# vibevoice-community/VibeVoice

Measured on AMD Instinct MI355X. Metric: audio-sec/wall-sec, higher is better.
Workload: dtype bf16

## Files before the change

### vibevoice_amd/csrc/engine.hip

```cpp
#include "engine_ctx.h"
#include "vv_w13.h"

thread_local char g_err[512] = "";
std::shared_mutex g_dev_mu;
std::mutex g_family_mu;

int fail(vv_ctx* ctx, const char* fmt, ...) {
    va_list ap; va_start(ap, fmt);
    char* dst = ctx ? ctx->err : g_err;
    vsnprintf(dst, 512, fmt, ap);
    va_end(ap);
    if (ctx) snprintf(g_err, 512, "%s", ctx->err);
    return -1;
}

int ring_acquire(vv_ctx* ctx) {
    const int slot = ctx->ring_i;
    ctx->ring_i = (ctx->ring_i + 1) % vv_ctx::RING;
    if (ctx->ring_used[slot]) hipEventSynchronize(ctx->ring_ev[slot]);
    ctx->ring_used[slot] = true;
    return slot;
}

void* dalloc(vv_ctx* ctx, size_t bytes, bool zero) {
// ... 102 lines not shown
                char prev[200]; snprintf(prev, sizeof(prev), "%s", ctx->err);
                return fail(ctx, "%s; the eager re-run failed as well (%s).  If another host thread called a device-wide synchronize "
                                 "(torch.cuda.synchronize()) during the capture, the stream is lost: synchronize streams or events instead", ctx->last_capture_issue, prev);
            }
            return 0;
        }
        if (ctx->graphs.size() >= ctx->graph_cap) {
            std::vector<std::pair<uint64_t, std::string>> order;
            for (auto& g : ctx->graphs) order.push_back({g.second.last_use, g.first});
            std::sort(order.begin(), order.end());
            std::unique_lock<std::shared_mutex> lk(g_dev_mu);
            HIPCHK(ctx, hipDeviceSynchronize());
            for (size_t i = 0; i < order.size() / 4 + 1; ++i) {
                auto v = ctx->graphs.find(order[i].second);
                hipGraphExecDestroy(v->second.exec);
                ctx->graphs.erase(v);
            }
        }
        it = ctx->graphs.emplace(key, ge).first;
    }
    it->second.last_use = ++ctx->graph_tick;
    VV_SHARED;
    HIPCHK(ctx, hipGraphLaunch(it->second.exec, st));
    return 0;
}

int drop_graphs(vv_ctx* ctx, std::initializer_list<const char*> prefixes) {
    auto hit = [&](const std::string& key) {
        for (const char* p : prefixes) if (key.rfind(p, 0) == 0) return true;
        return false;
    };
    bool any = false;
    for (auto& g : ctx->graphs) if (hit(g.first)) { any = true; break; }
    if (!any) return 0;
    HIPCHK(ctx, hipDeviceSynchronize());
    for (auto it = ctx->graphs.begin(); it != ctx->graphs.end();) {
        if (hit(it->first)) { hipGraphExecDestroy(it->second.exec); it = ctx->graphs.erase(it); } else ++it;
    }
    return 0;
}

extern "C" const char* vv_last_error(vv_ctx* ctx) { return ctx ? ctx->err : g_err; }

#ifndef VV_BUILD_ID
#define VV_BUILD_ID "unknown"
#endif
extern "C" const char* vv_build_id() { return "VVHIP_BUILD_ID=" VV_BUILD_ID; }

static int create_impl(const vv_config* cfg, vv_ctx* parent, vv_ctx** out) {
    VV_SHARED;
    vv_ctx* ctx = new vv_ctx();
    ctx->c = *cfg; ctx->err[0] = 0;
    ctx->parent = parent; ctx->creating = true;
    vv_config& c = ctx->c;
    if (c.max_rows < 1 || c.max_rows > 16384) { delete ctx; return fail(nullptr, "max_rows must be in [1,16384]"); }
    if (c.lm_head_dim != 64 && c.lm_head_dim != 128) { delete ctx; return fail(nullptr, "head_dim must be 64 or 128"); }
    if (c.lm_kv_heads < 1 || c.lm_heads % c.lm_kv_heads != 0 || c.lm_heads / c.lm_kv_heads > 16) {
        const int hq = c.lm_heads, hkv = c.lm_kv_heads;
        delete ctx;
        return fail(nullptr, "lm_heads=%d / lm_kv_heads=%d: the GQA group size must be an integer <= 16", hq, hkv);
    }
    if (c.xsplit < 1 || c.xsplit > 3) c.xsplit = 2;
    if (c.attn_splits < 1) c.attn_splits = 128;
    if (c.enc_frames < 1) c.enc_frames = 1;
    if (getenv("VVHIP_GRAPH_CAP")) ctx->graph_cap = (size_t)std::max(4, atoi(getenv("VVHIP_GRAPH_CAP")));
    c.max_ctx = (c.max_ctx + 127) & ~127;
    const int H = ctx->H = c.lm_hidden, D = ctx->D = c.lm_head_dim, Hq = ctx->Hq = c.lm_heads, Hkv = ctx->Hkv = c.lm_kv_heads;
    const int I = ctx->I = c.lm_inter;
    const int QKV = ctx->QKV = (Hq + 2 * Hkv) * D;
    const int R = c.max_rows;
    ctx->embed = walloc(ctx, (size_t)c.lm_vocab * H * 2);
    { int i = add_w(ctx, "lm.embed_tokens.weight", W_TABLE, (int64_t)c.lm_vocab * H); ctx->w[i].dev = ctx->embed; }
    { int i = add_w(ctx, "lm_head.weight", W_TABLE, (int64_t)c.lm_vocab * H, true); ctx->w[i].dev = nullptr; }
    ctx->inv_freq = add_vec(ctx, "lm.rope.inv_freq", D / 2);
    ctx->lm_norm = add_vec(ctx, "lm.norm.weight", H);
    if (c.tts_layers > 0) {
        if (c.tts_layers >= c.lm_layers) { delete ctx; return fail(nullptr, "tts_layers must be < lm_layers"); }
        ctx->tts_types = add_vec(ctx, "tts_input_types.weight", 2 * (int64_t)H);
        ctx->eos_w1 = alloc_packed(ctx, H, H); add_mat(ctx, "eos.fc1.weight", H, H, ctx->eos_w1, 0);
        ctx->eos_b1 = add_vec(ctx, "eos.fc1.bias", H);
        ctx->eos_w2 = alloc_packed(ctx, 1, H); add_mat(ctx, "eos.fc2.weight", 1, H, ctx->eos_w2, 0);
        ctx->eos_b2 = add_vec(ctx, "eos.fc2.bias", 1);
    }
    ctx->layers.resize(c.lm_layers);
    for (int l = 0; l < c.lm_layers; ++l) {
        auto& L = ctx->layers[l];
        char nm[128]; snprintf(nm, 128, "lm.layers.%d.", l);
        std::string p(nm);
        L.ln1 = add_vec(ctx, p + "input_layernorm.weight", H);
        L.ln2 = add_vec(ctx, p + "post_attention_layernorm.weight", H);
        L.wqkv = alloc_packed(ctx, QKV, H);
        L.bqkv = (float*)walloc(ctx, (size_t)QKV * 4);
        add_mat(ctx, p + "self_attn.q_proj.weight", Hq * D, H, L.wqkv, 0);
        add_mat(ctx, p + "self_attn.k_proj.weight", Hkv * D, H, L.wqkv, Hq * D / 16);
        add_mat(ctx, p + "self_attn.v_proj.weight", Hkv * D, H, L.wqkv, (Hq + Hkv) * D / 16);
        add_vec(ctx, p + "self_attn.q_proj.bias", Hq * D, L.bqkv);
        add_vec(ctx, p + "self_attn.k_proj.bias", Hkv * D, L.bqkv + Hq * D);
        add_vec(ctx, p + "self_attn.v_proj.bias", Hkv * D, L.bqkv + (Hq + Hkv) * D);
        L.wo = alloc_packed(ctx, H, Hq * D); add_mat(ctx, p + "self_attn.o_proj.weight", H, Hq * D, L.wo, 0);
        L.wg = alloc_packed(ctx, I, H); add_mat(ctx, p + "mlp.gate_proj.weight", I, H, L.wg, 0);
        L.wu = alloc_packed(ctx, I, H); add_mat(ctx, p + "mlp.up_proj.weight", I, H, L.wu, 0);
        L.wd = alloc_packed(ctx, H, I); add_mat(ctx, p + "mlp.down_proj.weight", H, I, L.wd, 0);
    }
    const int n_caches = 2 * c.n_slots;
    ctx->head_stride = (int64_t)c.max_ctx * D;
    ctx->layer_stride = ctx->head_stride * Hkv;
    ctx->cache_stride = ctx->layer_stride * c.lm_layers;
    ctx->kc = dalloc(ctx, (size_t)ctx->cache_stride * n_caches * 2);
    ctx->vc = dalloc(ctx, (size_t)ctx->cache_stride * n_caches * 2);
    ctx->rows_cap = std::max(2048, c.max_rows);
    ctx->rows_dev = (VVRow*)dalloc(ctx, sizeof(VVRow) * ctx->rows_cap);
    hipHostMalloc((void**)&ctx->rows_pin, sizeof(VVRow) * (size_t)ctx->rows_cap * vv_ctx::RING);
    for (int i = 0; i < vv_ctx::RING; ++i) hipEventCreateWithFlags(&ctx->ring_ev[i], hipEventDisableTiming);
    ctx->ids_cap = std::max(64, c.max_rows);
    ctx->ids_dev = (int*)dalloc(ctx, sizeof(int) * ctx->ids_cap);
    hipHostMalloc((void**)&ctx->ids_pin, sizeof(int) * (size_t)ctx->ids_cap * vv_ctx::RING);
    ctx->h = (float*)dalloc(ctx, (size_t)R * H * 4);
    ctx->h_parts = (float*)dalloc(ctx, (size_t)2 * R * H * 4);
    ctx->qkv = (float*)dalloc(ctx, (size_t)R * QKV * 4);
    ctx->qrot = (float*)dalloc(ctx, (size_t)R * Hq * D * 4);
    ctx->attn = (float*)dalloc(ctx, (size_t)R * Hq * D * 4);
    ctx->act = (float*)dalloc(ctx, (size_t)R * I * 4);
    if (R >= 64 && (H % 8) == 0 && ((Hq * D) % 8) == 0 && (I % 8) == 0) {
        ctx->xp = dalloc(ctx, (size_t)vv_packed_elems(R, std::max(H, Hq * D)) * 2);
        ctx->actp = dalloc(ctx, (size_t)vv_packed_elems(R, I) * 2);
        ctx->tile3_ok = c.xsplit == 1;
        if (ctx->tile3_ok) {
            ctx->gws.g3_bytes = (size_t)8 * std::min(R, 1024) * std::max(ctx->QKV, H) * 4;
            ctx->gws.g3_partials = (float*)dalloc(ctx, ctx->gws.g3_bytes, false);
            if (!ctx->gws.g3_partials) ctx->gws.g3_bytes = 0;
        }
        const char* no_ks = getenv("VVHIP_NO_KSPLIT");
        if (ctx->tile3_ok && R >= 1024 && !(no_ks && no_ks[0] == '1')) {
            ctx->gws.partials = (float*)dalloc(ctx, (size_t)256 * 32 * 512 * 16, false);
            ctx->gws.flags = (unsigned*)dalloc(ctx, 256 * sizeof(unsigned));
            if (hipHostMalloc((void**)&ctx->gws.err, sizeof(unsigned), hipHostMallocMapped) == hipSuccess && ctx->gws.err) *ctx->gws.err = 0u;
            else ctx->gws.err = nullptr;
        }
    }
    ctx->attn2_ok = c.xsplit == 1;
    if (c.xsplit == 1 && R > 4 && (H % 32) == 0 && ((Hq * D) % 32) == 0 && (I % 32) == 0) {
        const int kx = std::max(H, Hq * D), ka = std::max(I, c.head_ffn);
        ctx->p16_x = dalloc(ctx, (size_t)vv_packed_elems(16, kx) * 2);
        ctx->p16_act = dalloc(ctx, (size_t)vv_packed_elems(16, ka + 32) * 2);
        ctx->p16_y = dalloc(ctx, (size_t)vv_packed_elems(16, kx) * 2);
        ctx->ssq_a = (float*)dalloc(ctx, (size_t)(H / 16) * 16 * 4);
        ctx->ssq_b = (float*)dalloc(ctx, (size_t)(H / 16) * 16 * 4);
        ctx->p16_ok = ctx->p16_x && ctx->p16_act && ctx->p16_y && ctx->ssq_a && ctx->ssq_b;
    }
    ctx->rope_tab = dalloc(ctx, (size_t)c.max_ctx * (D / 2) * 8, false);
    ctx->ws_rows = std::min(R, 64);
    const size_t np = (size_t)ctx->ws_rows * Hkv * c.attn_splits * 16;
    ctx->pm = (float*)dalloc(ctx, np * 4); ctx->pl = (float*)dalloc(ctx, np * 4); ctx->po = (float*)dalloc(ctx, np * D * 4);
    const int L = c.latent_dim, HL = c.head_layers, HF = ctx->HF = c.head_ffn;
    const int MODW = ctx->MODW = HL * 3 * H + 2 * H;
    ctx->h_in = alloc_packed(ctx, H, L); add_mat(ctx, "head.noisy_images_proj.weight", H, L, ctx->h_in, 0);
    ctx->h_cond = alloc_packed(ctx, H, H); add_mat(ctx, "head.cond_proj.weight", H, H, ctx->h_cond, 0);
    ctx->h_t0 = alloc_packed(ctx, H, 256); add_mat(ctx, "head.t_embedder.mlp.0.weight", H, 256, ctx->h_t0, 0);
    ctx->h_t2 = alloc_packed(ctx, H, H); add_mat(ctx, "head.t_embedder.mlp.2.weight", H, H, ctx->h_t2, 0);
    ctx->h_ada = alloc_packed(ctx, MODW, H);
    ctx->hl.resize(HL);
    {
        const char* e = getenv("VVHIP_W13");
        ctx->w13_on = parent ? parent->w13_on : !(e && e[0] == '0') && c.xsplit == 1 && vv_w13_shape_ok(HF, H) && vv_w13_shape_ok(H, HF);
    }
    auto twin = [&](int N, int K) {
        if (ctx->w13_on) ctx->w.back().w13 = walloc(ctx, (size_t)vv_w13_bytes(N, K));
        return (int)ctx->w.size() - 1;
    };
    for (int l = 0; l < HL; ++l) {
        char nm[128]; snprintf(nm, 128, "head.layers.%d.", l);
        std::string p(nm);
        ctx->hl[l].norm = add_vec(ctx, p + "norm.weight", H);
        add_mat(ctx, p + "adaLN_modulation.1.weight", 3 * H, H, ctx->h_ada, l * 3 * H / 16);
        ctx->hl[l].wg = alloc_packed(ctx, HF, H); add_mat(ctx, p + "ffn.gate_proj.weight", HF, H, ctx->hl[l].wg, 0); ctx->hl[l].ig = twin(HF, H);
        ctx->hl[l].wu = alloc_packed(ctx, HF, H); add_mat(ctx, p + "ffn.up_proj.weight", HF, H, ctx->hl[l].wu, 0); ctx->hl[l].iu = twin(HF, H);
        ctx->hl[l].wd = alloc_packed(ctx, H, HF); add_mat(ctx, p + "ffn.down_proj.weight", H, HF, ctx->hl[l].wd, 0); ctx->hl[l].id = twin(H, HF);
    }
    add_mat(ctx, "head.final_layer.adaLN_modulation.1.weight", 2 * H, H, ctx->h_ada, HL * 3 * H / 16);
    ctx->h_out = alloc_packed(ctx, L, H); add_mat(ctx, "head.final_layer.linear.weight", L, H, ctx->h_out, 0);
    const int R2 = 16;
    ctx->cproj = (float*)dalloc(ctx, (size_t)R2 * H * 4);
    ctx->mod = (float*)dalloc(ctx, (size_t)R2 * MODW * 4);
    for (HeadGen& g : ctx->hg) {
        g.zz = (float*)dalloc(ctx, (size_t)R2 * L * 4);
        g.x0p = (float*)dalloc(ctx, (size_t)R2 * L * 4);
        g.xh = (float*)dalloc(ctx, (size_t)R2 * H * 4);
    }
    ctx->head_tail = c.xsplit == 1 && L == 64 && (H % 32) == 0 && vv_head_tail_init() == 0;
    if (const char* e = getenv("VVHIP_SOLVER_FUSE"); e && e[0] == '0') ctx->solver_fuse = false;
    if (const char* e = getenv("VVHIP_NAN_PROBE"); e && e[0] == '1') {
        ctx->probe_rec = (unsigned*)dalloc(ctx, PROBE_MAX * 16);
        ctx->probe_on = ctx->probe_rec != nullptr;
    }
    ctx->xh_parts = (float*)dalloc(ctx, (size_t)4 * R2 * H * 4);
    ctx->hact = (float*)dalloc(ctx, (size_t)R2 * HF * 4);
    ctx->eps = (float*)dalloc(ctx, (size_t)R2 * L * 4);
    ctx->tmp1 = (float*)dalloc(ctx, (size_t)64 * H * 4);
    ctx->tmp2 = (float*)dalloc(ctx, (size_t)64 * 256 * 4);
    auto mk_conn = [&](vv_ctx::Conn& cn, const std::string& p, int din) {
        cn.fc1 = alloc_packed(ctx, H, din); add_mat(ctx, p + "fc1.weight", H, din, cn.fc1, 0);
        cn.b1 = add_vec(ctx, p + "fc1.bias", H);
        cn.norm = add_vec(ctx, p + "norm.weight", H);
        cn.fc2 = alloc_packed(ctx, H, H); add_mat(ctx, p + "fc2.weight", H, H, cn.fc2, 0);
        cn.b2 = add_vec(ctx, p + "fc2.bias", H);
    };
    mk_conn(ctx->ac_conn, "ac_conn.", L);
    if (c.sem_dim > 0) mk_conn(ctx->sem_conn, "sem_conn.", c.sem_dim);
    ctx->ct1 = (float*)dalloc(ctx, (size_t)256 * H * 4);
    if (build_codec(ctx, ctx->dec, "dec.", true, L, 1, c.n_slots)) { *out = ctx; return -1; }
    if (c.sem_dim > 0 && build_codec(ctx, ctx->senc, "senc.", false, c.sem_dim, 1, c.n_slots)) { *out = ctx; return -1; }
    if (c.has_acoustic_encoder && build_codec(ctx, ctx->aenc, "aenc.", false, L, c.enc_frames, 1)) { *out = ctx; return -1; }
    if (hipDeviceSynchronize() != hipSuccess || ctx->err[0]) { *out = ctx; return fail(ctx, "vv_create: allocation failed: %s", ctx->err); }
    ctx->creating = false;
    if (parent) {
        if (ctx->wshare_i != parent->wallocs.size() || ctx->w.size() != parent->w.size()) {
            *out = ctx;
            return fail(ctx, "vv_create_shared: the child registered %zu weight buffers / %zu parameters, the parent %zu / %zu -- different model configuration",
                        ctx->wshare_i, ctx->w.size(), parent->wallocs.size(), parent->w.size());
        }
        for (size_t i = 0; i < ctx->w.size(); ++i) {
            if (ctx->w[i].name != parent->w[i].name || ctx->w[i].nelem != parent->w[i].nelem) { *out = ctx; return fail(ctx, "vv_create_shared: parameter table differs at '%s'", ctx->w[i].name.c_str()); }
            ctx->w[i].loaded = parent->w[i].loaded;
            ctx->w[i].w13_ok = parent->w[i].w13_ok;
            if (ctx->w[i].name == "lm_head.weight") ctx->w[i].dev = parent->w[i].dev;
        }
        ctx->lm_head = parent->lm_head; ctx->lm_head_loaded = parent->lm_head_loaded;
        ctx->scaling = parent->scaling; ctx->bias = parent->bias;
        { std::lock_guard<std::mutex> fl(g_family_mu); parent->n_children++; }
    }
    *out = ctx;
    return 0;
}

extern "C" int vv_create(const vv_config* cfg, vv_ctx** out) { return create_impl(cfg, nullptr, out); }

extern "C" int vv_create_shared(const vv_config* cfg, vv_ctx* parent, vv_ctx** out) {
    if (!parent) return fail(nullptr, "vv_create_shared: no parent context");
    if (parent->parent) return fail(nullptr, "vv_create_shared: the parent is itself a shared context; share from the owner of the weights");
    for (auto& w : parent->w)
        if (!w.loaded && !w.optional) return fail(nullptr, "vv_create_shared: parent parameter '%s' is not uploaded yet", w.name.c_str());
    vv_config a = *cfg, b = parent->c;
    a.n_slots = b.n_slots; a.max_ctx = b.max_ctx; a.max_rows = b.max_rows; a.attn_splits = b.attn_splits; a.use_graph = b.use_graph;
    if (a.xsplit < 1 || a.xsplit > 3) a.xsplit = 2;
    if (a.enc_frames < 1) a.enc_frames = 1;
    if (memcmp(&a, &b, sizeof(vv_config)) != 0) return fail(nullptr, "vv_create_shared: the model fields of the configuration differ from the parent's");
    int r = create_impl(cfg, parent, out);
    if (r != 0 && *out) { vv_ctx* c = *out; c->parent = nullptr; }
    return r;
}

static void destroy_impl(vv_ctx* ctx) {
    if (!ctx) return;
    hipDeviceSynchronize();
    {
        std::lock_guard<std::mutex> fl(g_family_mu);
        if (ctx->n_children > 0) { ctx->zombie = true; return; }
    }
    vv_ctx* par = ctx->parent;
    for (auto& g : ctx->graphs) hipGraphExecDestroy(g.second.exec);
    if (ctx->side_ready) {
        for (int j = 0; j < 8; ++j) { hipStreamDestroy(ctx->side[j]); hipEventDestroy(ctx->ev_join[j]); }
        hipEventDestroy(ctx->ev_fork);
    }
    for (void* p : ctx->allocs) hipFree(p);
    ctx->allocs.clear();
    if (ctx->stage) hipFree(ctx->stage);
    hipHostFree(ctx->rows_pin); hipHostFree(ctx->ids_pin);
    if (ctx->gws.err) hipHostFree(ctx->gws.err);
    for (int i = 0; i < vv_ctx::RING; ++i) if (ctx->ring_ev[i]) hipEventDestroy(ctx->ring_ev[i]);
    delete ctx;
    bool last_child = false;
    if (par) { std::lock_guard<std::mutex> fl(g_family_mu); last_child = (--par->n_children == 0 && par->zombie); }
    if (last_child) destroy_impl(par);
}
extern "C" void vv_destroy(vv_ctx* ctx) {
    VV_SHARED;
    destroy_impl(ctx);
}

extern "C" int vv_num_weights(vv_ctx* ctx) { return (int)ctx->w.size(); }
extern "C" int vv_weight_info(vv_ctx* ctx, int idx, char* name, int cap, int64_t* nelem, int* loaded) {
    if (idx < 0 || idx >= (int)ctx->w.size()) return fail(ctx, "weight index out of range");
    const Weight& w = ctx->w[idx];
    snprintf(name, cap, "%s", w.name.c_str());
    if (nelem) *nelem = w.nelem;
    if (loaded) *loaded = (w.loaded || w.optional) ? 1 : 0;
    return 0;
}

extern "C" int vv_upload(vv_ctx* ctx, const char* name, const void* src, int src_dtype, int64_t nelem) {
    VV_SHARED;
    auto it = ctx->widx.find(name);
    if (it == ctx->widx.end()) return fail(ctx, "unknown parameter '%s'", name);
    Weight& w = ctx->w[it->second];
    if (ctx->parent) return fail(ctx, "parameter '%s': this context shares its parent's weights -- upload through the parent", name);
    {
        std::lock_guard<std::mutex> fl(g_family_mu);
        if (ctx->n_children > 0)
            return fail(ctx, "parameter '%s': %d shared context(s) were created from this one and hold snapshots derived from its parameters -- "
                             "destroy them (model.close_lanes()), upload / merge, then fork again", name, ctx->n_children);
    }
    if (nelem != w.nelem) return fail(ctx, "parameter '%s': expected %lld elements, got %lld", name, (long long)w.nelem, (long long)nelem);
    const size_t esz = src_dtype ? 2 : 4;
    hipPointerAttribute_t attr;
    bool on_dev = (hipPointerGetAttributes(&attr, src) == hipSuccess) && (attr.type == hipMemoryTypeDevice);
    (void)hipGetLastError();
    const void* dsrc = src;
    if (!on_dev) {
        const size_t need = (size_t)nelem * esz;
        if (need > ctx->stage_bytes) {
            if (ctx->stage) hipFree(ctx->stage);
            ctx->stage = nullptr; ctx->stage_bytes = 0;
            HIPCHK(ctx, hipMalloc(&ctx->stage, need));
            ctx->stage_bytes = need;
        }
        HIPCHK(ctx, hipMemcpy(ctx->stage, src, need, hipMemcpyHostToDevice));
        dsrc = ctx->stage;
    }
    hipStream_t st = 0;
    if (w.kind == W_TABLE) {
        if (w.name == "lm_head.weight" && !ctx->lm_head_loaded) {
            ctx->lm_head = dalloc(ctx, (size_t)nelem * 2, false);
            if (!ctx->lm_head) return -1;
            ctx->lm_head_loaded = true; w.dev = ctx->lm_head;
        }
        if (src_dtype) HIPCHK(ctx, hipMemcpy(w.dev, dsrc, (size_t)nelem * 2, hipMemcpyDeviceToDevice));
        else VVCHK(vv_cvt_launch(dsrc, w.dev, nelem, 1, st));
    } else if (w.kind == W_MAT) {
        VVCHK(vv_pack_launch(dsrc, src_dtype, w.dev, w.N, w.K, w.pk, w.Cin, w.Cout, w.ksz, w.stride, st));
        VVTRY(lora_rebase(ctx, it->second, st));
        VVTRY(w13_repack(ctx, it->second, st));
    } else {
        const float* f32 = (const float*)dsrc;
        float* tmp = nullptr;
        if (src_dtype) {
            tmp = (float*)dalloc(ctx, (size_t)nelem * 4, false);
            if (!tmp) return -1;
            VVCHK(vv_cvt_launch(dsrc, tmp, nelem, 0, st));
            f32 = tmp;
        }
        if (w.kind == W_DW) {
            VVCHK(vv_dw_transpose_launch(f32, (float*)w.dev, (int)(nelem / 7), st));
        } else if (w.kind == W_BIAS_REP) {
            for (int r = 0; r < w.rep; ++r)
                HIPCHK(ctx, hipMemcpyAsync((float*)w.dev + (size_t)r * nelem, f32, (size_t)nelem * 4, hipMemcpyDeviceToDevice, st));
        } else {
            HIPCHK(ctx, hipMemcpyAsync(w.dev, f32, (size_t)nelem * 4, hipMemcpyDeviceToDevice, st));
        }
        HIPCHK(ctx, hipStreamSynchronize(st));
        dfree(ctx, tmp);
    }
    HIPCHK(ctx, hipStreamSynchronize(st));
    w.loaded = true;
    ctx->rope_ready = false;
    return 0;
}

int w13_repack(vv_ctx* ctx, int widx, hipStream_t st) {
    Weight& w = ctx->w[widx];
    if (!w.w13) return 0;
    VVCHK(vv_w13_pack_launch(w.dev, w.w13, w.N, w.K, st));
    HIPCHK(ctx, hipStreamSynchronize(st));
    unsigned ok = 0;
    HIPCHK(ctx, hipMemcpy(&ok, (const char*)w.w13 + vv_w13_plane_bytes(w.N, w.K) + (size_t)2 * (w.N / 16) * 4, 4, hipMemcpyDeviceToHost));
    const bool now = ok == 1;
    if (now == w.w13_ok) return 0;
    w.w13_ok = now;
    return drop_graphs(ctx, {"samp:", "sde:", "rows:", "gen:"});
}

extern "C" int vv_set_speech_factors(vv_ctx* ctx, float scaling, float bias) {
    VV_SHARED;
    ctx->scaling = scaling; ctx->bias = bias;
    return drop_graphs(ctx, {"dec:1:", "chain:1:"});
}

extern "C" int vv_set_valid_tokens(vv_ctx* ctx, const int* ids, int n) {
    VV_SHARED;
    if (n < 1 || n > 16) return fail(ctx, "n_valid must be in [1,16]");
    const int H = ctx->H;
    const void* table = ctx->lm_head_loaded ? ctx->lm_head : ctx->embed;
    void* rows = dalloc(ctx, (size_t)n * H * 2, false);
    if (!rows) return -1;
    for (int i = 0; i < n; ++i) {
        if (ids[i] < 0 || ids[i] >= ctx->c.lm_vocab) return fail(ctx, "token id %d out of range", ids[i]);
        HIPCHK(ctx, hipMemcpy((char*)rows + (size_t)i * H * 2, (const char*)table + (size_t)ids[i] * H * 2, (size_t)H * 2, hipMemcpyDeviceToDevice));
    }
    if (!ctx->valid_w) ctx->valid_w = alloc_packed(ctx, 16, H);
    VVCHK(vv_pack_launch(rows, 1, ctx->valid_w, n, H, 0, 0, 0, 0, 0, 0));
    HIPCHK(ctx, hipDeviceSynchronize());
    dfree(ctx, rows);
    ctx->n_valid = n;
    for (int i = 0; i < n; ++i) ctx->valid_ids[i] = ids[i];
    return 0;
}
extern "C" int vv_check(vv_ctx* ctx, void* stream) {
    if (!ctx) return -1;
    return ksplit_check(ctx, (hipStream_t)stream);
}
extern "C" int vv_audio_to_pcm16(vv_ctx* ctx, void* stream, int n, int samples, const float* audio_dev, int16_t* pcm_out_dev) {
    VV_SHARED;
    hipStream_t st = (hipStream_t)stream;
    if (n < 1 || samples < 1) return fail(ctx, "vv_audio_to_pcm16: n and samples must be positive");
    VVCHK(vv_pcm16_launch(audio_dev, (short*)pcm_out_dev, n, samples, st));
    return 0;
}
extern "C" int vv_connect(vv_ctx* ctx, void* stream, int n, const float* latent_dev, const float* sem_dev, float* out_dev) {
    VV_SHARED;
    hipStream_t st = (hipStream_t)stream;
    const int H = ctx->H, L = ctx->c.latent_dim;
    for (int i0 = 0; i0 < n; i0 += 16) {
        const int nn = std::min(16, n - i0);
        float* out = out_dev + (size_t)i0 * H;
        VVGemm a1 = mk_gemm(ctx->ac_conn.fc1, latent_dev + (size_t)i0 * L, ctx->ct1, nn, H, L, L, H);
        a1.epi = VV_EPI_BIAS; a1.bias = ctx->ac_conn.b1; GEMM(a1);
        VVGemm a2 = mk_gemm(ctx->ac_conn.fc2, ctx->ct1, out, nn, H, H, H, H);
        a2.pro = VV_PRO_RMS; a2.nw = ctx->ac_conn.norm; a2.eps = 1e-6f; a2.epi = VV_EPI_BIAS; a2.bias = ctx->ac_conn.b2; GEMM(a2);
        if (sem_dev) {
            const int S = ctx->c.sem_dim;
            VVGemm s1 = mk_gemm(ctx->sem_conn.fc1, sem_dev + (size_t)i0 * S, ctx->ct1, nn, H, S, S, H);
            s1.epi = VV_EPI_BIAS; s1.bias = ctx->sem_conn.b1; GEMM(s1);
            VVGemm s2 = mk_gemm(ctx->sem_conn.fc2, ctx->ct1, out, nn, H, H, H, H);
            s2.pro = VV_PRO_RMS; s2.nw = ctx->sem_conn.norm; s2.eps = 1e-6f; s2.epi = VV_EPI_RESID; s2.bias = ctx->sem_conn.b2; GEMM(s2);
        }
    }
    return 0;
}

extern "C" int64_t vv_packed_bytes(int N, int K) { return vv_packed_elems(N, K) * 2; }
extern "C" int vv_pack_matrix(void* stream, const float* src_dev, void* dst_dev, int N, int K) {
    return vv_pack_launch(src_dev, 0, dst_dev, N, K, 0, 0, 0, 0, 0, (hipStream_t)stream);
}
extern "C" int64_t vv_stat(vv_ctx* ctx, int what) {
    switch (what) {
        case 0: return ctx->launches;
        case 2: return ctx->prof_raw_ns;
        case 3: return ctx->prof_ev_over_ns;
        case 5: return ctx->foreign_nodes;
        case 4: return ctx->capture_fallbacks;
        case 6: return ctx->seam_launches;
        case 8: return ctx->solver_fused;
        case 7: return ctx->lora_base_bytes;
        case 9: {
            int64_t n = 0;
            for (const auto& l : ctx->hl) {
                if (ctx->w[l.ig].w13_ok && ctx->w[l.iu].w13_ok) n += 2;
                if (ctx->w[l.id].w13_ok) n += 1;
            }
            return n;
        }
        default: return (int64_t)ctx->graphs.size();
    }
}
```

### vibevoice_amd/csrc/engine_ctx.h

```cpp
#pragma once
#include <algorithm>
#include <cmath>
#include <cstdarg>
#include <cstdio>
#include <cstdlib>
#include <cstring>
#include <functional>
#include <initializer_list>
#include <map>
#include <mutex>
#include <set>
#include <shared_mutex>
#include <string>
#include <vector>
#include "../../include/vvhip.h"
#include "vv_common.h"
#include "vv_launch.h"

namespace vv_engine {
struct VVShiftH { float* buf; int T, hist, C; };
enum WKind { W_MAT = 0, W_VEC = 1, W_DW = 2, W_TABLE = 3, W_BIAS_REP = 4 };

struct Weight {
    std::string name;
    int kind = W_VEC;
    int64_t nelem = 0;
    void* dev = nullptr;
    int N = 0, K = 0, pk = 0, Cin = 0, Cout = 0, ksz = 0, stride = 0;
    int rep = 1;
    bool loaded = false;
    bool optional = false;
    void* w13 = nullptr;
    bool w13_ok = false;
};

struct Block {
    int C;
    float *norm_w, *ffn_norm_w, *gamma, *ffn_gamma, *dw_w, *dw_b, *b1, *b2;
    void *w1, *w2;
    float* nb;
    float* nst;
    int64_t nb_stride;
};

struct ConvG {
    void* w; float* bias;
    int K, N, ldx;
    int rows_per_frame;
};

struct Stage {
    int C, Tpf;
    int hist;
    float* xs;
    float* xs2;
    float* xfinal;
    bool fused;
    bool pp;
    int64_t sl_stride;
    std::vector<Block> blocks;
    ConvG in;
};

struct CodecNet {
    bool decoder = false;
    int Fmax = 1, in_dim = 1, out_dim = 1, in_hist = 6, in_Tpf = 1;
    std::vector<float*> in_buf;
    std::vector<std::vector<Stage>> st;
    ConvG head;
    std::vector<float*> u;
    std::map<std::pair<uint64_t, int>, std::pair<void*, int>> shift_tab;
    int maxC = 1;
    int kd = 0, ke = 1 << 30;
    bool head_batch = false;
    int64_t in_stride = 0, u_stride = 0;
};

struct GraphEntry { hipGraphExec_t exec; uint64_t last_use; };

struct HeadGen { float *xh = nullptr, *zz = nullptr, *x0p = nullptr, *m2 = nullptr; };

}
using namespace vv_engine;

constexpr int PROBE_MAX = 1024;

struct vv_ctx {
    vv_config c;
    char err[512];
    std::vector<Weight> w;
    std::map<std::string, int> widx;
    int H, D, Hq, Hkv, I, QKV;
    struct Layer { float *ln1, *ln2, *bqkv; void *wqkv, *wo, *wg, *wu, *wd; };
    std::vector<Layer> layers;
    float *lm_norm = nullptr, *inv_freq = nullptr;
    int ws_rows = 0;
    void* rope_tab = nullptr; bool rope_ready = false;
    float *tts_types = nullptr, *eos_b1 = nullptr, *eos_b2 = nullptr; void *eos_w1 = nullptr, *eos_w2 = nullptr;
    void *embed = nullptr, *lm_head = nullptr;
    bool lm_head_loaded = false;
    void* valid_w = nullptr; int n_valid = 0;
    int valid_ids[16] = {0};
    void *kc = nullptr, *vc = nullptr;
    int64_t cache_stride = 0, head_stride = 0, layer_stride = 0;
    VVRow* rows_dev = nullptr; VVRow* rows_pin = nullptr; int rows_cap = 2048;
    int* ids_dev = nullptr; int* ids_pin = nullptr; int ids_cap = 64;
    static constexpr int RING = 32;
    hipEvent_t ring_ev[RING] = {}; bool ring_used[RING] = {}; int ring_i = 0;
    float *h = nullptr, *qkv = nullptr, *qrot = nullptr, *attn = nullptr, *act = nullptr;
    float *h_parts = nullptr, *xh_parts = nullptr;
    void *xp = nullptr, *actp = nullptr;
    bool tile3_ok = false, attn2_ok = false;
    VVGemmWs gws = {nullptr, nullptr, nullptr, nullptr, 0};
    void *p16_x = nullptr, *p16_act = nullptr, *p16_y = nullptr, *p16_shift = nullptr; float *ssq_a = nullptr, *ssq_b = nullptr; bool p16_ok = false;
    size_t p16_shift_tile = 0;
    float *pm = nullptr, *pl = nullptr, *po = nullptr;
    int HF = 0, MODW = 0;
    struct HLayer { float* norm; void *wg, *wu, *wd; int ig, iu, id; };
    bool w13_on = false;
    std::vector<HLayer> hl;
    void *h_in = nullptr, *h_cond = nullptr, *h_t0 = nullptr, *h_t2 = nullptr, *h_ada = nullptr, *h_out = nullptr;
    int n_steps = 0;
    float *temb = nullptr, *coef = nullptr, *tvals = nullptr;
    bool sde_on = false;
    bool general_on = false;
    float* mod_all = nullptr; size_t mod_all_bytes = 0;
    float* ada_in = nullptr;
    void* ada_p = nullptr;
    float *cproj = nullptr, *mod = nullptr, *hact = nullptr, *eps = nullptr;
    HeadGen hg[2];
    bool head_tail = false;
    bool solver_fuse = true;
    float *tmp1 = nullptr, *tmp2 = nullptr;
    struct Conn { void *fc1, *fc2; float *b1, *b2, *norm; } ac_conn, sem_conn;
    float *ct1 = nullptr;
    CodecNet dec, aenc, senc;
    int enc_pass = 0;
    hipStream_t side[8] = {}; hipEvent_t ev_fork = nullptr, ev_join[8] = {}; bool side_ready = false;
    float scaling = 1.f, bias = 0.f;
    int hop = 3200;
    void* stage = nullptr; size_t stage_bytes = 0;
    std::map<std::string, GraphEntry> graphs;
    uint64_t graph_tick = 0; size_t graph_cap = 512;
    std::set<std::string> seen;
    std::set<void*> allocs;
    vv_ctx* parent = nullptr; int n_children = 0; bool zombie = false, creating = false;
    unsigned* probe_rec = nullptr; std::vector<std::string> probe_names; bool probe_on = false; int probe_calls = 0;
    int64_t foreign_nodes = 0;
    int64_t capture_fallbacks = 0; char last_capture_issue[256] = "";
    std::vector<std::pair<void*, size_t>> wallocs; size_t wshare_i = 0;
    struct LoraBase { void* snap; size_t bytes; bool merged; };
    std::map<int, LoraBase> lora_base;
    int64_t lora_base_bytes = 0;
    struct RowStage { int n_streams = 0; std::vector<int64_t> total; std::vector<char> flushed; };
    struct Resampler : RowStage { int L = 0, M = 0, T = 0; float* coef = nullptr; float* hist = nullptr; };
    static constexpr int N_RESAMPLERS = 4;
    Resampler rs[N_RESAMPLERS];
    struct Tempo : RowStage { float* window = nullptr; float* hist = nullptr; int* dstate = nullptr; std::vector<int> P, Q; };
    static constexpr int N_TEMPOS = 4;
    Tempo tp[N_TEMPOS];
    struct Level : RowStage { int A = 0, H = 0; float c = 0.f; float* hist = nullptr; std::vector<float> gain; };
    static constexpr int N_LEVELS = 4;
    Level lv[N_LEVELS];
    int64_t launches = 0;
    int64_t solver_fused = 0;
    int64_t seam_launches = 0;
    bool prof_on = false;
    std::vector<hipEvent_t> prof_ev;
    int prof_n = 0;
    double prof_bytes = 0.0;
    struct ProfRec { int T, N, K, pro, epi, dual; double bytes; int gemv; };
    std::vector<ProfRec> prof_rec;
    std::vector<VVGemm> prof_gemv;
    double prof_gemv_bytes = 0.0;
    struct ProfLaunch { int family; double bytes; std::function<int(hipStream_t)> fn; };
    std::vector<ProfLaunch> prof_other;
    int64_t prof_raw_ns = 0, prof_ev_over_ns = 0;
    hipStream_t prof_stream = nullptr;
#ifdef VV_GEMM_TIMING
    unsigned long long* tl_base = nullptr; int tl_idx = 0;
    struct TlRec { int T, N, K, pro, epi; };
    std::vector<TlRec> tl_rec;
#endif
};

extern thread_local char g_err[512];
extern std::shared_mutex g_dev_mu;
#define VV_SHARED std::shared_lock<std::shared_mutex> _vv_dev_lk(g_dev_mu)
extern std::mutex g_family_mu;
int fail(vv_ctx* ctx, const char* fmt, ...);
#define HIPCHK(ctx, e) do { hipError_t _e = (e); if (_e != hipSuccess) return fail(ctx, "%s:%d hip error %s", __FILE__, __LINE__, hipGetErrorString(_e)); } while (0)
#define VVCHK(e) do { int _r = (e); if (_r != 0) return _r < 0 ? fail(ctx, "%s:%d launch failed (%d): hip error %d (%s)", __FILE__, __LINE__, _r, g_vv_launch_err, hipGetErrorString((hipError_t)g_vv_launch_err)) : _r; } while (0)
#define VVTRY(e) do { if (int _r = (e)) return _r; } while (0)

void* dalloc(vv_ctx* ctx, size_t bytes, bool zero = true);
void dfree(vv_ctx* ctx, void* p);
void* walloc(vv_ctx* ctx, size_t bytes, bool zero = true);
void* alloc_packed(vv_ctx* ctx, int N, int K);
int add_w(vv_ctx* ctx, const std::string& name, int kind, int64_t nelem, bool optional = false);
void add_mat(vv_ctx* ctx, const std::string& name, int N, int K, void* base, int ntile_off, int pk = 0, int Cin = 0, int Cout = 0,
             int ksz = 0, int stride = 0, int64_t src_nelem = -1);
float* add_vec(vv_ctx* ctx, const std::string& name, int64_t n, float* dst = nullptr, int kind = W_VEC, int rep = 1);
// ... 27 lines not shown
```

### vibevoice_amd/csrc/engine_head.hip

```cpp
#include "engine_ctx.h"
#include "pass_plan.h"

static int set_schedule(vv_ctx* ctx, int n_steps, const float* t, const float* coef, int width, void* stream, bool stochastic = false) {
    VV_SHARED;
    hipStream_t st = (hipStream_t)stream;
    if (n_steps < 1 || n_steps > 64) return fail(ctx, "n_steps must be in [1,64]");
    const int H = ctx->H;
    if (!ctx->temb) {
        ctx->temb = (float*)dalloc(ctx, (size_t)64 * H * 4);
        ctx->coef = (float*)dalloc(ctx, 64 * 8 * 4);
        ctx->tvals = (float*)dalloc(ctx, 64 * 4);
    }
    const bool general = width == 8;
    if (general && !ctx->hg[0].m2) {
        for (HeadGen& g : ctx->hg) g.m2 = (float*)dalloc(ctx, (size_t)8 * ctx->c.latent_dim * 4);
        if (!ctx->hg[0].m2 || !ctx->hg[1].m2) return fail(ctx, "vv_set_schedule_general: out of device memory");
    }
    float rows[64 * 8] = {};
    for (int i = 0; i < n_steps; ++i)
        for (int j = 0; j < width; ++j) rows[i * 8 + j] = coef[i * width + j];
    ctx->sde_on = general ? stochastic : (width == 6);
    ctx->general_on = general;
    HIPCHK(ctx, hipStreamSynchronize(st));
    HIPCHK(ctx, hipMemcpy(ctx->coef, rows, (size_t)n_steps * 8 * 4, hipMemcpyHostToDevice));
    HIPCHK(ctx, hipMemcpy(ctx->tvals, t, (size_t)n_steps * 4, hipMemcpyHostToDevice));
    VVCHK(vv_tfreq_launch(ctx->tvals, ctx->tmp2, n_steps, st));
    for (int i0 = 0; i0 < n_steps; i0 += 16) {
        const int nn = std::min(16, n_steps - i0);
        VVGemm g = mk_gemm(ctx->h_t0, ctx->tmp2 + (size_t)i0 * 256, ctx->tmp1 + (size_t)i0 * H, nn, H, 256, 256, H);
        GEMM(g);
    }
    VVCHK(vv_silu_launch(ctx->tmp1, n_steps * H, st));
    for (int i0 = 0; i0 < n_steps; i0 += 16) {
        const int nn = std::min(16, n_steps - i0);
        VVGemm g = mk_gemm(ctx->h_t2, ctx->tmp1 + (size_t)i0 * H, ctx->temb + (size_t)i0 * H, nn, H, H, H, H);
        GEMM(g);
    }
    HIPCHK(ctx, hipStreamSynchronize(st));
    ctx->n_steps = n_steps;
    {
        const size_t need = (size_t)n_steps * 16 * ctx->MODW * 4;
        if (need > ctx->mod_all_bytes) {
            dfree(ctx, ctx->mod_all);
            dfree(ctx, ctx->ada_in);
            ctx->mod_all = (float*)dalloc(ctx, need, false);
            ctx->ada_in = (float*)dalloc(ctx, (size_t)n_steps * 16 * ctx->H * 4, false);
            dfree(ctx, ctx->ada_p);
            ctx->ada_p = (ctx->c.xsplit == 1 && (ctx->H & 7) == 0) ? dalloc(ctx, (size_t)vv_packed_elems(n_steps * 16, ctx->H) * 2, false) : nullptr;
            ctx->mod_all_bytes = (ctx->mod_all && ctx->ada_in) ? need : 0;
            dfree(ctx, ctx->p16_shift); ctx->p16_shift = nullptr;
            if (ctx->p16_ok) {
                ctx->p16_shift_tile = (size_t)vv_packed_elems(16, ctx->H) * 2;
                ctx->p16_shift = dalloc(ctx, (size_t)n_steps * (ctx->c.head_layers + 1) * ctx->p16_shift_tile);
            }
        }
    }
    return drop_graphs(ctx, {"samp:", "sde:", "rows:", "gen:"});
}
extern "C" int vv_set_schedule(vv_ctx* ctx, int n_steps, const float* t, const float* coef, void* stream) {
    return set_schedule(ctx, n_steps, t, coef, 5, stream);
}
extern "C" int vv_set_schedule_sde(vv_ctx* ctx, int n_steps, const float* t, const float* coef6, void* stream) {
    return set_schedule(ctx, n_steps, t, coef6, 6, stream);
}

extern "C" int vv_set_schedule_general(vv_ctx* ctx, int n_steps, const float* t, const float* coef, int stochastic, void* stream) {
    return set_schedule(ctx, n_steps, t, coef, 8, stream, stochastic != 0);
}

static VVHeadPlan head_plan(const vv_ctx* ctx, int rows, int n_steps, bool has_coef) {
    return vv_head_plan(rows, n_steps, ctx->HF, ctx->c.head_layers, ctx->MODW,
                        {ctx->p16_ok, ctx->p16_shift != nullptr, ctx->ada_p != nullptr, ctx->mod_all_bytes != 0, ctx->head_tail, ctx->w13_on}, has_coef,
                        has_coef && ctx->general_on);
}

struct StepEnd { const float* coef; float cfg; const float *cfg_rows, *noise; };
struct HeadStep {
    int step;
    const float *z, *temb, *mod;
    const unsigned char* sh_tiles;
    float* eps_out;
    const HeadGen &cur, &nxt;
    bool have_x;
    const StepEnd* end;
};

static int head_eval(vv_ctx* ctx, hipStream_t st, const VVHeadPlan& p, const HeadStep& s) {
    const vv_config& c = ctx->c;
    const int rows = p.rows, final_stage = vv_head_final(p, s.step);
    const int H = ctx->H, L = c.latent_dim, HL = c.head_layers, HF = ctx->HF, MODW = ctx->MODW;
    const float* mod = s.mod ? s.mod : ctx->mod;
    const StepEnd end = s.end ? *s.end : StepEnd{};
    auto put_end = [&](auto& a) { a.coef = end.coef; a.cfg = end.cfg; a.n_cfg = rows / 2; a.sde_noise = end.noise; a.cfg_rows = end.cfg_rows; };
    float* const xh = s.cur.xh;
    if (!s.mod) {
        VVGemm ga = mk_gemm(ctx->h_ada, ctx->cproj, ctx->mod, rows, MODW, H, H, MODW);
        ga.pro = VV_PRO_ADD_SILU; ga.addvec = s.temb; ga.nt = 1;
        GEMM(ga);
    }
    if (!s.have_x) {
        VVGemm gi = mk_gemm(ctx->h_in, s.z, xh, rows, H, L, L, H);
        GEMM(gi);
        nan_probe(ctx, st, "in-proj xh", xh, (size_t)rows * H);
    }
    int xp = 0;
    const int xps = 16 * H;
    for (int l = 0; l < HL; ++l) {
        const float* base = mod + (size_t)l * 3 * H;
        if (p.layers == VV_HEAD_P16) {
            ctx->launches += 3;
            VVCHK(vv_pack16_launch(xh, H, 2, ctx->hl[l].norm, c.head_eps, base + H, base, MODW, ctx->p16_x, rows, H, st));
            VVCHK(p16_gemv(ctx, st, ctx->hl[l].wg, ctx->hl[l].wu, ctx->p16_x, nullptr, ctx->p16_act, nullptr, nullptr, rows, HF, H, 0, 0, VV_EPI_SWIGLU));
            if (l + 1 == HL && final_stage == VV_FINAL_P16_CFG) {
                VVGemv16p ad = p16_args(ctx->hl[l].wd, nullptr, ctx->p16_act, xh, ctx->p16_x, rows, H, HF, H);
                ad.gate = base + 2 * H; ad.ld_gate = MODW; ad.ssq_out = ctx->ssq_a;
                ad.pk_nw = nullptr; ad.pk_sc = mod + (size_t)HL * 3 * H + H; ad.ld_pk = MODW;
                VVCHK(p16_go(ctx, st, ad, VV_EPI_GATED_RESID, 4));
            } else
            VVCHK(p16_gemv(ctx, st, ctx->hl[l].wd, nullptr, ctx->p16_act, xh, nullptr, nullptr, base + 2 * H, rows, H, HF, H, MODW, VV_EPI_GATED_RESID));
            continue;
        }
        VVGemm g1 = mk_gemm(ctx->hl[l].wg, xh, ctx->hact, rows, HF, H, H, HF);
        g1.W2 = (const u32x4*)ctx->hl[l].wu; g1.pro = VV_PRO_RMS_MOD; g1.nw = ctx->hl[l].norm; g1.eps = c.head_eps;
        g1.mod_shift = base; g1.mod_scale = base + H; g1.ld_mod = MODW; g1.epi = VV_EPI_SWIGLU; g1.nt = 1;
        float* cur = ctx->xh_parts + (size_t)(l & 1) * 2 * xps;
        float* nxt = ctx->xh_parts + (size_t)((l + 1) & 1) * 2 * xps;
        g1.xa = cur; g1.n_xa = xp; g1.part_stride = xps;
        const Weight &mg = ctx->w[ctx->hl[l].ig], &mu = ctx->w[ctx->hl[l].iu], &md = ctx->w[ctx->hl[l].id];
        if (p.w13 && mg.w13_ok && mu.w13_ok && vv_gemv_w13_form(&g1, c.xsplit) >= 0) { g1.w13 = mg.w13; g1.w13_2 = mu.w13; }
        GEMM(g1);
        VVGemm g2 = mk_gemm(ctx->hl[l].wd, ctx->hact, xh, rows, H, HF, HF, H);
        g2.epi = VV_EPI_GATED_RESID; g2.gate = base + 2 * H; g2.ld_gate = MODW; g2.nt = 1;
        g2.ya = cur; g2.n_ya = xp; g2.part_stride = xps;
        xp = ksplit_parts(ctx, g2, nxt, xps);
        if (p.w13 && md.w13_ok && vv_gemv_w13_form(&g2, c.xsplit) >= 0) g2.w13 = md.w13;
        if (ctx->probe_on) { char nm[64]; snprintf(nm, 64, "layer %d hact (parts in %d)", l, g1.n_xa); nan_probe(ctx, st, nm, ctx->hact, (size_t)rows * HF); }
        GEMM(g2);
        if (ctx->probe_on) {
            char nm[64]; snprintf(nm, 64, "layer %d xh", l); nan_probe(ctx, st, nm, xh, (size_t)rows * H);
            for (int q = 0; q < xp; ++q) { snprintf(nm, 64, "layer %d part %d", l, q); nan_probe(ctx, st, nm, nxt + (size_t)q * xps, (size_t)rows * H); }
        }
    }
    const float* fb = mod + (size_t)HL * 3 * H;
    if (final_stage == VV_FINAL_P16_CFG) {
        ctx->launches += 1;
        VVGemv16p af = p16_args(ctx->h_out, nullptr, ctx->p16_x, nullptr, nullptr, rows, L, H, L);
        af.ssq_in = ctx->ssq_a; af.ssq_tiles = H / 16; af.eps = c.head_eps;
        af.Xs = (const u32x4*)(s.sh_tiles + (size_t)HL * ctx->p16_shift_tile);
        af.z = s.cur.zz; af.x0p = s.cur.x0p; put_end(af);
        VVCHK(p16_go(ctx, st, af, VV_EPI_CFG_DPM, 3));
        return 0;
    }
    if (final_stage == VV_FINAL_SEAM) {
        VVTail t{};
        t.Wout = (const u32x4*)ctx->h_out; t.Win = (const u32x4*)ctx->h_in; t.bin = nullptr;
        t.X = xh; t.xa = ctx->xh_parts + (size_t)(HL & 1) * 2 * xps; t.n_xa = xp; t.part_stride = xps;
        t.sc = fb + H; t.sh = fb; t.ld_mod = MODW;
        t.Xout = s.nxt.xh;
        t.z_in = s.cur.zz; t.x0p_in = s.cur.x0p; t.z_out = s.nxt.zz; t.x0p_out = s.nxt.x0p; put_end(t);
        t.T = rows; t.H = H; t.L = L; t.eps = c.head_eps;
        if (vv_head_tail_ok(&t)) {
            ctx->launches++;
            ctx->seam_launches++;
            if (ctx->prof_on) {
                const VVTail tc = t;
                ctx->prof_other.push_back({3, (double)vv_packed_elems(L, H) * 2.0 + (double)vv_packed_elems(H, L) * 2.0 + (double)rows * H * 8.0,
                                           [=](hipStream_t s2) { return vv_head_tail_launch(&tc, s2); }});
            }
            VVCHK(vv_head_tail_launch(&t, st));
            return 1;
        }
    }
    VVGemm gf = mk_gemm(ctx->h_out, xh, s.eps_out, rows, L, H, H, L);
    gf.pro = VV_PRO_RMS_MOD; gf.nw = nullptr; gf.eps = c.head_eps; gf.mod_shift = fb; gf.mod_scale = fb + H; gf.ld_mod = MODW;
    gf.xa = ctx->xh_parts + (size_t)(HL & 1) * 2 * xps; gf.n_xa = xp; gf.part_stride = xps;
    if (final_stage != VV_FINAL_GEMM) {
        gf.epi = VV_EPI_CFG_DPM; gf.z = s.cur.zz; gf.x0p = s.cur.x0p; put_end(gf);
    }
    GEMM(gf);
    return 0;
}

struct SampleReq { int n; const float *cond, *noise, *step_noise; float cfg; const float* cfg_rows; float* out; };
struct StepDone { int rc; bool flipped; };

static StepDone step_shipped(vv_ctx* ctx, hipStream_t st, const VVHeadPlan& p, const SampleReq& r, HeadStep s) {
    const StepEnd end{ctx->coef + s.step * 8, r.cfg, r.cfg_rows,
                      r.step_noise ? r.step_noise + (size_t)s.step * r.n * ctx->c.latent_dim : nullptr};
    s.end = &end;
    const int hr = head_eval(ctx, st, p, s);
    return {hr, hr == 1};
}

static StepDone step_general(vv_ctx* ctx, hipStream_t st, const VVHeadPlan& p, const SampleReq& r, const HeadStep& s) {
    const int L = ctx->c.latent_dim;
    if (head_eval(ctx, st, p, s) < 0) return {-1, false};
    VVSolverStep v{};
    v.eps = s.eps_out; v.coef = ctx->coef + s.step * 8; v.cfg = r.cfg; v.cfg_rows = r.cfg_rows; v.n = r.n; v.L = L;
    v.noise = r.step_noise ? r.step_noise + (size_t)s.step * r.n * L : nullptr;
    v.z_in = s.cur.zz; v.m1_in = s.cur.x0p; v.m2_in = s.cur.m2;
    v.z_out = s.nxt.zz; v.m1_out = s.nxt.x0p; v.m2_out = s.nxt.m2;
    if (s.step + 1 < p.n_steps && ctx->solver_fuse) { v.Win = (const u32x4*)ctx->h_in; v.Xout = s.nxt.xh; v.H = ctx->H; v.xs = ctx->c.xsplit; }
    ctx->launches++;
    const int sr = vv_solver_step_launch(&v, st);
    if (sr == VV_RC_NO_FORM) return {fail(ctx, "vv_diffusion_sample_general: solver.hip has no form for n = %d, latent_dim = %d", r.n, L), false};
    if (sr < 0) return {fail(ctx, "%s:%d launch failed (%d): hip error %d (%s)", __FILE__, __LINE__, sr, g_vv_launch_err, hipGetErrorString((hipError_t)g_vv_launch_err)), false};
    if (sr == 1) ctx->solver_fused++;
    return {sr == 1, true};
}

static int sample_body(vv_ctx* ctx, hipStream_t st, const SampleReq& r) {
    const int H = ctx->H, L = ctx->c.latent_dim, HL = ctx->c.head_layers;
    const int n = r.n, rows = 2 * n;
    ctx->seam_launches = ctx->solver_fused = 0;
    ctx->probe_names.clear();
    nan_probe(ctx, st, "cond (input)", r.cond, (size_t)rows * H);
    nan_probe(ctx, st, "noise (input)", r.noise, (size_t)n * L);
    VVCHK(vv_sampler_init_launch(r.noise, ctx->hg[0].zz, ctx->hg[0].x0p, n * L, st));
    VVGemm gc = mk_gemm(ctx->h_cond, r.cond, ctx->cproj, rows, H, H, H, H);
    gc.nt = 1;
    GEMM(gc);
    const int MODW = ctx->MODW;
    const VVHeadPlan p = head_plan(ctx, rows, ctx->n_steps, true);
    const bool batch_ada = p.ada != VV_ADA_PER_STEP;
    if (batch_ada) {
        const int total = rows * ctx->n_steps;
        if (p.ada == VV_ADA_TILE) {
            ctx->launches += 2;
            VVCHK(vv_ada_pack_launch(ctx->cproj, ctx->temb, ctx->ada_p, rows, ctx->n_steps, H, st));
            VVCHK(vv_gemm3_launch(ctx->h_ada, nullptr, ctx->ada_p, ctx->mod_all, nullptr, nullptr, total, MODW, H, MODW, VV_EPI_STORE, nullptr, st));
        } else {
        VVCHK(vv_ada_in_launch(ctx->cproj, ctx->temb, ctx->ada_in, rows, ctx->n_steps, H, st));
        ctx->launches++;
        for (int t0 = 0; t0 < total; t0 += 16) {
            const int T = std::min(16, total - t0);
            VVGemm ga = mk_gemm(ctx->h_ada, ctx->ada_in + (size_t)t0 * H, ctx->mod_all + (size_t)t0 * MODW, T, MODW, H, H, MODW);
            GEMM(ga);
        }
        }
    }
    nan_probe(ctx, st, "cproj", ctx->cproj, (size_t)rows * H);
    if (batch_ada) nan_probe(ctx, st, "mod_all", ctx->mod_all, (size_t)rows * ctx->n_steps * MODW);
    if (p.sh_tiles) {
        ctx->launches++;
        VVCHK(vv_pack16_tiles_launch(ctx->mod_all, MODW, (int64_t)rows * MODW, HL + 1, (int64_t)3 * H, ctx->p16_shift,
                                     (int64_t)ctx->p16_shift_tile, rows, H, ctx->n_steps * (HL + 1), st));
    }
    int gen = 0; bool have_x = false;
    for (int i = 0; i < ctx->n_steps; ++i) {
        const HeadGen& cur = ctx->hg[gen];
        const HeadStep s{.step = i, .z = cur.zz, .temb = ctx->temb + (size_t)i * H,
                         .mod = batch_ada ? ctx->mod_all + (size_t)i * rows * MODW : nullptr,
                         .sh_tiles = p.sh_tiles ? (const unsigned char*)ctx->p16_shift + (size_t)i * (HL + 1) * ctx->p16_shift_tile : nullptr,
                         .eps_out = ctx->eps, .cur = cur, .nxt = ctx->hg[gen ^ 1], .have_x = have_x, .end = nullptr};
        const StepDone d = p.solver_step ? step_general(ctx, st, p, r, s) : step_shipped(ctx, st, p, r, s);
        if (d.rc < 0) return -1;
        have_x = d.rc == 1;
        gen ^= d.flipped;
        if (ctx->probe_on) {
            const HeadGen& now = ctx->hg[gen];
            char nm[64];
            snprintf(nm, 64, "step %d z%s", i, p.solver_step ? " (general)" : have_x ? " (seam, next gen)" : ""); nan_probe(ctx, st, nm, now.zz, (size_t)rows * L);
            if (!p.solver_step) { snprintf(nm, 64, "step %d x0p", i); nan_probe(ctx, st, nm, now.x0p, (size_t)n * L); }
            if (!p.solver_step && have_x) { snprintf(nm, 64, "step %d next xh", i); nan_probe(ctx, st, nm, now.xh, (size_t)rows * H); }
        }
    }
    VVCHK(vv_copy_launch(r.out, ctx->hg[gen].zz, (size_t)n * L * 4, st));
    return 0;
}

static int run_sampler(vv_ctx* ctx, hipStream_t st, const char* key, const SampleReq& r) {
    ctx->launches = 0;
    const int rc = graphed(ctx, key, st, [&]() { return sample_body(ctx, st, r); });
    nan_probe_report(ctx, st, key);
    return rc;
}

extern "C" int vv_diffusion_sample(vv_ctx* ctx, void* stream, int n, const float* cond_dev, const float* noise_dev, float cfg_scale, float* latent_out_dev) {
    if (ctx->n_steps < 1) return fail(ctx, "vv_set_schedule has not been called");
    if (n < 1 || n > 8) return fail(ctx, "vv_diffusion_sample: n must be in [1,8]");
    if (ctx->general_on) return fail(ctx, "the installed table is a general one (vv_set_schedule_general): sample with vv_diffusion_sample_general");
    if (ctx->sde_on) return fail(ctx, "the schedule is stochastic (vv_set_schedule_sde): sample with vv_diffusion_sample_sde and its per-step noise");
    char key[128]; snprintf(key, 128, "samp:%d:%p:%p:%p:%a", n, (const void*)cond_dev, (const void*)noise_dev, (void*)latent_out_dev, cfg_scale);
    return run_sampler(ctx, (hipStream_t)stream, key, {n, cond_dev, noise_dev, nullptr, cfg_scale, nullptr, latent_out_dev});
}

extern "C" int vv_diffusion_sample_sde(vv_ctx* ctx, void* stream, int n, const float* cond_dev, const float* noise_dev,
                                       const float* step_noise_dev, float cfg_scale, float* latent_out_dev) {
    if (ctx->n_steps < 1) return fail(ctx, "vv_set_schedule_sde has not been called");
    if (n < 1 || n > 8) return fail(ctx, "vv_diffusion_sample_sde: n must be in [1,8]");
    if (ctx->general_on) return fail(ctx, "the installed table is a general one (vv_set_schedule_general): sample with vv_diffusion_sample_general");
    if (!ctx->sde_on) return fail(ctx, "the schedule is deterministic (vv_set_schedule): sample with vv_diffusion_sample");
    if (!step_noise_dev) return fail(ctx, "vv_diffusion_sample_sde: step_noise is null");
    char key[160]; snprintf(key, 160, "sde:%d:%p:%p:%p:%p:%a", n, (const void*)cond_dev, (const void*)noise_dev, (const void*)step_noise_dev,
                            (void*)latent_out_dev, cfg_scale);
    return run_sampler(ctx, (hipStream_t)stream, key, {n, cond_dev, noise_dev, step_noise_dev, cfg_scale, nullptr, latent_out_dev});
}

extern "C" int vv_diffusion_sample_rows(vv_ctx* ctx, void* stream, int n, const float* cond_dev, const float* noise_dev,
                                        const float* step_noise_dev, const float* cfg_rows_dev, float* latent_out_dev) {
    if (ctx->n_steps < 1) return fail(ctx, "vv_set_schedule / vv_set_schedule_sde has not been called");
    if (n < 1 || n > 8) return fail(ctx, "vv_diffusion_sample_rows: n must be in [1,8]");
    if (ctx->general_on) return fail(ctx, "the installed table is a general one (vv_set_schedule_general): sample with vv_diffusion_sample_general");
    if (!cfg_rows_dev) return fail(ctx, "vv_diffusion_sample_rows: cfg_rows is null");
    if (ctx->sde_on && !step_noise_dev) return fail(ctx, "the schedule is stochastic (vv_set_schedule_sde): vv_diffusion_sample_rows needs its per-step noise");
    if (!ctx->sde_on && step_noise_dev) return fail(ctx, "the schedule is deterministic (vv_set_schedule): vv_diffusion_sample_rows takes no step noise");
    char key[192]; snprintf(key, 192, "rows:%d:%p:%p:%p:%p:%p", n, (const void*)cond_dev, (const void*)noise_dev, (const void*)step_noise_dev,
                            (const void*)cfg_rows_dev, (void*)latent_out_dev);
    return run_sampler(ctx, (hipStream_t)stream, key, {n, cond_dev, noise_dev, step_noise_dev, 0.f, cfg_rows_dev, latent_out_dev});
}

extern "C" int vv_diffusion_sample_general(vv_ctx* ctx, void* stream, int n, const float* cond_dev, const float* noise_dev,
                                           const float* step_noise_dev, float cfg_scale, const float* cfg_rows_dev, float* latent_out_dev) {
    if (ctx->n_steps < 1) return fail(ctx, "vv_set_schedule_general has not been called");
    if (n < 1 || n > 8) return fail(ctx, "vv_diffusion_sample_general: n must be in [1,8]");
    if (!ctx->general_on) return fail(ctx, "the installed table is a shipped one (vv_set_schedule / vv_set_schedule_sde): sample with vv_diffusion_sample, _sde or _rows");
    if (ctx->sde_on && !step_noise_dev) return fail(ctx, "the general table is stochastic: vv_diffusion_sample_general needs its per-step noise");
    if (!ctx->sde_on && step_noise_dev) return fail(ctx, "the general table is deterministic: vv_diffusion_sample_general takes no step noise");
    char key[224]; snprintf(key, 224, "gen:%d:%p:%p:%p:%p:%p:%a", n, (const void*)cond_dev, (const void*)noise_dev, (const void*)step_noise_dev,
                            (const void*)cfg_rows_dev, (void*)latent_out_dev, cfg_rows_dev ? 0.f : cfg_scale);
    return run_sampler(ctx, (hipStream_t)stream, key, {n, cond_dev, noise_dev, step_noise_dev, cfg_scale, cfg_rows_dev, latent_out_dev});
}

extern "C" int vv_head_forward(vv_ctx* ctx, void* stream, int n, const float* noisy_dev, const float* t_host, const float* cond_dev, float* out_dev) {
    VV_SHARED;
    hipStream_t st = (hipStream_t)stream;
    if (n < 1 || n > 16) return fail(ctx, "vv_head_forward: n must be in [1,16]");
    const int H = ctx->H;
    for (int i = 1; i < n; ++i) if (t_host[i] != t_host[0]) return fail(ctx, "vv_head_forward: all rows must share one timestep");
    float* tdev = ctx->tmp2 + 63 * 256;
    HIPCHK(ctx, hipStreamSynchronize(st));
    HIPCHK(ctx, hipMemcpy(tdev + 128, t_host, 4, hipMemcpyHostToDevice));
    VVCHK(vv_tfreq_launch(tdev + 128, ctx->tmp2, 1, st));
    VVGemm g = mk_gemm(ctx->h_t0, ctx->tmp2, ctx->tmp1, 1, H, 256, 256, H); GEMM(g);
    VVCHK(vv_silu_launch(ctx->tmp1, H, st));
    VVGemm g2 = mk_gemm(ctx->h_t2, ctx->tmp1, ctx->tmp1 + H, 1, H, H, H, H); GEMM(g2);
    VVGemm gc = mk_gemm(ctx->h_cond, cond_dev, ctx->cproj, n, H, H, H, H); GEMM(gc);
    const HeadStep s{.step = 0, .z = noisy_dev, .temb = ctx->tmp1 + H, .mod = nullptr, .sh_tiles = nullptr, .eps_out = out_dev,
                     .cur = ctx->hg[0], .nxt = ctx->hg[1], .have_x = false, .end = nullptr};
    if (head_eval(ctx, st, head_plan(ctx, n, 1, false), s)) return -1;
    HIPCHK(ctx, hipStreamSynchronize(st));
    return 0;
}
```

### vibevoice_amd/csrc/engine_lm.hip

```cpp
#include "engine_ctx.h"
#include "pass_plan.h"

int p16_gemv(vv_ctx* ctx, hipStream_t st, const void* W, const void* W2, const void* Xp, float* Y, void* Yp, const float* bias,
                    const float* gate, int T, int N, int K, int ldy, int ld_gate, int epi) {
    if (ctx->prof_on) {
        const double by = (double)vv_packed_elems(N, K) * 2.0 * (W2 ? 2.0 : 1.0) + (double)vv_packed_elems(16, K) * 2.0 +
                          (Yp ? (double)T * N * 2.0 : (double)T * N * 4.0 * (epi == VV_EPI_RESID || epi == VV_EPI_GATED_RESID ? 2.0 : 1.0));
        ctx->prof_other.push_back({1, by, [=](hipStream_t s) { return vv_gemv16p_launch(W, W2, Xp, Y, Yp, bias, gate, T, N, K, ldy, ld_gate, epi, s); }});
    }
    return vv_gemv16p_launch(W, W2, Xp, Y, Yp, bias, gate, T, N, K, ldy, ld_gate, epi, st);
}

int p16_go(vv_ctx* ctx, hipStream_t st, const VVGemv16p& a, int epi, int flags) {
    if (ctx->prof_on) {
        const double by = (double)vv_packed_elems(a.N, a.K) * 2.0 * (a.W2 ? 2.0 : 1.0) + (double)vv_packed_elems(16, a.K) * 2.0 * ((flags & 2) ? 2.0 : 1.0) +
                          ((epi == VV_EPI_SWIGLU) ? (double)a.T * a.N * 2.0 : (double)a.T * a.N * 4.0 * (epi == VV_EPI_RESID || epi == VV_EPI_GATED_RESID ? 2.0 : 1.0)) +
                          ((flags & 4) ? (double)a.T * a.N * 2.0 : 0.0);
        const VVGemv16p ac = a;
        ctx->prof_other.push_back({1, by, [=](hipStream_t s) { return vv_gemv16p_launch2(&ac, epi, flags, s); }});
    }
    return vv_gemv16p_launch2(&a, epi, flags, st);
}
VVGemv16p p16_args(const void* W, const void* W2, const void* Xp, float* Y, void* Yp, int T, int N, int K, int ldy) {
    VVGemv16p a{};
// ... 21 lines not shown
    const vv_config& c = ctx->c;
    const int H = ctx->H, D = ctx->D, Hq = ctx->Hq, Hkv = ctx->Hkv, I = ctx->I, QKV = ctx->QKV;
    for (int l = l0; l < l1; ++l) {
        auto& L = ctx->layers[l];
        char *kl = lm_kc(ctx, l), *vl = lm_vc(ctx, l);
        ctx->launches += 9;
        VVCHK(vv_pack_rows_launch(ctx->h, H, L.ln1, c.lm_eps, ctx->xp, R, H, st));
        const int fq = vv_gemm_qkv_rope_launch(L.wqkv, ctx->xp, L.bqkv, R, H, D, Hq, Hkv, ctx->rows_dev, ctx->rope_tab, ctx->qrot, kl, vl,
                                               ctx->cache_stride, ctx->head_stride, &ctx->gws, st);
        if (fq < 0) return fail(ctx, "vv_gemm_qkv_rope_launch failed (%d)", fq);
        if (fq == 0) {
            VVCHK(vv_gemm3_launch(L.wqkv, nullptr, ctx->xp, ctx->qkv, nullptr, L.bqkv, R, QKV, H, QKV, VV_EPI_BIAS, &ctx->gws, st));
            VVCHK(vv_rope_append_launch(D, ctx->qkv, ctx->rows_dev, ctx->inv_freq, ctx->qrot, kl, vl,
                                        R, Hq, Hkv, ctx->cache_stride, ctx->head_stride, st));
        }
        const bool apk = ((Hq * D) & 31) == 0;
        VVCHK(vv_attn_prefill4_launch(D, ctx->qrot, ctx->rows_dev, kl, vl, R, Hq, Hkv, ctx->cache_stride, ctx->head_stride, ctx->attn,
                                      apk ? ctx->xp : nullptr, st));
        if (!apk) VVCHK(vv_pack_rows_launch(ctx->attn, Hq * D, nullptr, 0.f, ctx->xp, R, Hq * D, st));
        VVCHK(vv_gemm3_launch(L.wo, nullptr, ctx->xp, ctx->h, nullptr, nullptr, R, H, Hq * D, H, VV_EPI_RESID, &ctx->gws, st));
        VVCHK(vv_pack_rows_launch(ctx->h, H, L.ln2, c.lm_eps, ctx->xp, R, H, st));
        VVCHK(vv_gemm3_launch(L.wg, L.wu, ctx->xp, nullptr, ctx->actp, nullptr, R, I, H, 0, VV_EPI_SWIGLU, &ctx->gws, st));
        VVCHK(vv_gemm3_launch(L.wd, nullptr, ctx->actp, ctx->h, nullptr, nullptr, R, H, I, H, VV_EPI_RESID, &ctx->gws, st));
    }
    return lm_finish(ctx, st, R, hidden_out, final_norm);
}

static int lm_decode_attn(vv_ctx* ctx, hipStream_t st, int R, int l, const VVLmPlan& p, void* out_packed) {
    const vv_config& c = ctx->c;
    const int D = ctx->D, Hq = ctx->Hq, Hkv = ctx->Hkv;
    char *kl = lm_kc(ctx, l), *vl = lm_vc(ctx, l);
    const int attn_S = p.attn_S;
    ctx->launches += (attn_S > 1) ? 2 : 1;
    if (ctx->prof_on) {
        const double by = (double)p.kv_positions * Hkv * D * 2.0 * 2.0 + (double)R * (ctx->QKV + Hq * D) * 4.0;
        const int xs = c.xsplit; vv_ctx* cx = ctx;
        ctx->prof_other.push_back({2, by, [=](hipStream_t s) {
            return vv_attn_fused_launch(D, xs, cx->qkv, cx->rows_dev, cx->rope_tab, kl, vl, R, Hq, Hkv, cx->cache_stride,
                                        cx->head_stride, attn_S, cx->pm, cx->pl, cx->po, cx->attn, out_packed, s); }});
    }
    VVCHK(vv_attn_fused_launch(D, c.xsplit, ctx->qkv, ctx->rows_dev, ctx->rope_tab, kl, vl, R, Hq, Hkv, ctx->cache_stride,
                               ctx->head_stride, attn_S, ctx->pm, ctx->pl, ctx->po, ctx->attn, out_packed, st));
    return 0;
}

static int lm_p16_layer(vv_ctx* ctx, hipStream_t st, int R, int l, int l0, int l1, const VVLmPlan& p) {
    const vv_config& c = ctx->c;
    const int H = ctx->H, Hq = ctx->Hq, D = ctx->D, I = ctx->I, QKV = ctx->QKV;
    auto& L = ctx->layers[l];
    if (l > l0) {
        ctx->launches += 1;
        VVGemv16p a = p16_args(L.wqkv, nullptr, ctx->p16_x, ctx->qkv, nullptr, R, QKV, H, QKV);
        a.bias = L.bqkv; a.ssq_in = ctx->ssq_b; a.ssq_tiles = H / 16; a.eps = c.lm_eps;
        VVCHK(p16_go(ctx, st, a, VV_EPI_BIAS, 1));
    } else {
        ctx->launches += 2;
        VVCHK(vv_pack16_launch(ctx->h, H, 1, L.ln1, c.lm_eps, nullptr, nullptr, 0, ctx->p16_x, R, H, st));
        VVCHK(p16_gemv(ctx, st, L.wqkv, nullptr, ctx->p16_x, ctx->qkv, nullptr, L.bqkv, nullptr, R, QKV, H, QKV, 0, VV_EPI_BIAS));
    }
    VVTRY(lm_decode_attn(ctx, st, R, l, p, ctx->p16_y));
    ctx->launches += 3;
    VVGemv16p ao = p16_args(L.wo, nullptr, ctx->p16_y, ctx->h, ctx->p16_x, R, H, Hq * D, H);
    ao.pk_nw = L.ln2; ao.ssq_out = ctx->ssq_a;
    VVCHK(p16_go(ctx, st, ao, VV_EPI_RESID, 4));
    VVGemv16p ag = p16_args(L.wg, L.wu, ctx->p16_x, nullptr, ctx->p16_act, R, I, H, 0);
    ag.ssq_in = ctx->ssq_a; ag.ssq_tiles = H / 16; ag.eps = c.lm_eps;
    VVCHK(p16_go(ctx, st, ag, VV_EPI_SWIGLU, 1));
    VVGemv16p ad = p16_args(L.wd, nullptr, ctx->p16_act, ctx->h, nullptr, R, H, I, H);
    if (l + 1 < l1) {
        ad.Yp = (unsigned char*)ctx->p16_x; ad.pk_nw = ctx->layers[l + 1].ln1; ad.ssq_out = ctx->ssq_b;
        VVCHK(p16_go(ctx, st, ad, VV_EPI_RESID, 4));
    } else VVCHK(p16_go(ctx, st, ad, VV_EPI_RESID, 0));
    return 0;
}

static int lm_gemv_layer(vv_ctx* ctx, hipStream_t st, int R, int l, int l1, const VVLmPlan& p, int& hp) {
    const vv_config& c = ctx->c;
    const int H = ctx->H, D = ctx->D, Hq = ctx->Hq, Hkv = ctx->Hkv, I = ctx->I, QKV = ctx->QKV;
    const int hps = ctx->c.max_rows * H;
    auto& L = ctx->layers[l];
    VVGemm g = mk_gemm(L.wqkv, ctx->h, ctx->qkv, R, QKV, H, H, QKV);
    g.pro = VV_PRO_RMS; g.nw = L.ln1; g.eps = c.lm_eps; g.epi = VV_EPI_BIAS; g.bias = L.bqkv; g.nt = 1;
    g.xa = ctx->h_parts; g.n_xa = hp; g.part_stride = hps;
    GEMM(g);
    if (p.attn == VV_ATTN_FUSED) {
        VVTRY(lm_decode_attn(ctx, st, R, l, p, nullptr));
    } else {
        char *kl = lm_kc(ctx, l), *vl = lm_vc(ctx, l);
        ctx->launches += 3;
        VVCHK(vv_rope_append_launch(D, ctx->qkv, ctx->rows_dev, ctx->inv_freq, ctx->qrot, kl, vl,
                                    R, Hq, Hkv, ctx->cache_stride, ctx->head_stride, st));
        if (p.attn == VV_ATTN_PREFILL4)
            VVCHK(vv_attn_prefill4_launch(D, ctx->qrot, ctx->rows_dev, kl, vl, R, Hq, Hkv, ctx->cache_stride, ctx->head_stride, ctx->attn, nullptr, st));
        else {
            for (int k = 0; k < p.attn_groups; ++k) {
                const int g0 = k * ctx->ws_rows, ng = std::min(ctx->ws_rows, R - g0);
                if (g0) ctx->launches += 2;
                VVCHK(vv_attn_launch(D, c.xsplit, ctx->qrot + (size_t)g0 * Hq * D, ctx->rows_dev + g0, kl, vl, ng, Hq, Hkv, ctx->cache_stride,
                                     ctx->head_stride, p.attn_S, ctx->pm, ctx->pl, ctx->po, ctx->attn + (size_t)g0 * Hq * D, st));
            }
        }
    }
    VVGemm go = mk_gemm(L.wo, ctx->attn, ctx->h, R, H, Hq * D, Hq * D, H);
    go.epi = VV_EPI_RESID; go.nt = 1;
    go.ya = ctx->h_parts; go.n_ya = hp; go.part_stride = hps;
    GEMM(go);
    hp = 0;
    VVGemm gm = mk_gemm(L.wg, ctx->h, ctx->act, R, I, H, H, I);
    gm.W2 = (const u32x4*)L.wu; gm.pro = VV_PRO_RMS; gm.nw = L.ln2; gm.eps = c.lm_eps; gm.epi = VV_EPI_SWIGLU; gm.nt = 1;
    GEMM(gm);
    VVGemm gd = mk_gemm(L.wd, ctx->act, ctx->h, R, H, I, I, H);
    gd.epi = VV_EPI_RESID; gd.nt = 1;
    if (l + 1 < l1) hp = ksplit_parts(ctx, gd, ctx->h_parts, hps);
    GEMM(gd);
    return 0;
}

static int lm_body(vv_ctx* ctx, hipStream_t st, int R, const float* x_in, float* hidden_out, int l0, int l1, int final_norm, const VVLmPlan& p) {
    VVCHK(vv_copy_launch(ctx->h, x_in, (size_t)R * ctx->H * 4, st));
    if (p.zero_v_tail) VVTRY(lm_zero_v_tail(ctx, st, R, l0, l1));
    if (p.route == VV_LM_PREFILL) return lm_prefill_layers(ctx, st, R, hidden_out, l0, l1, final_norm);
    int hp = 0;
    for (int l = l0; l < l1; ++l)
        VVTRY(p.route == VV_LM_P16 ? lm_p16_layer(ctx, st, R, l, l0, l1, p) : lm_gemv_layer(ctx, st, R, l, l1, p, hp));
    return lm_finish(ctx, st, R, hidden_out, final_norm);
}

int ksplit_check(vv_ctx* ctx, hipStream_t st) {
    if (!(ctx->gws.err && *ctx->gws.err)) return 0;
    {
        VV_SHARED;
        hipStreamSynchronize(st);
        if (ctx->gws.flags) { hipMemsetAsync(ctx->gws.flags, 0, 256 * sizeof(unsigned), st); hipStreamSynchronize(st); }
    }
    *ctx->gws.err = 0u;
    return fail(ctx, "prefill GEMM: a K-split hand-off timed out (lost producer workgroup); the prompt pass that was in flight is invalid -- "
                     "the arrival words were re-armed, retry the pass (VVHIP_NO_KSPLIT=1 disables the split)");
}
extern "C" int vv_lm_forward(vv_ctx* ctx, void* stream, int n_rows, const vv_row* rows, const float* x_in_dev, float* hidden_out_dev) {
    return vv_lm_forward_range(ctx, stream, n_rows, rows, x_in_dev, hidden_out_dev, 0, ctx->c.lm_layers, 1);
}
extern "C" int vv_lm_forward_range(vv_ctx* ctx, void* stream, int n_rows, const vv_row* rows, const float* x_in_dev,
                                   float* hidden_out_dev, int l0, int l1, int final_norm) {
    hipStream_t st = (hipStream_t)stream;
    if (l0 < 0 || l1 > ctx->c.lm_layers || l0 >= l1) return fail(ctx, "layer range [%d,%d) invalid", l0, l1);
    if (n_rows < 1 || n_rows > ctx->c.max_rows) return fail(ctx, "n_rows %d out of range [1,%d]", n_rows, ctx->c.max_rows);
    if (ksplit_check(ctx, st)) return -1;
    (void)hipGetLastError();
    for (int i = 0; i < n_rows; ++i) {
        if (rows[i].cache < 0 || rows[i].cache >= 2 * ctx->c.n_slots) return fail(ctx, "row %d: cache id %d out of range", i, rows[i].cache);
        if (rows[i].pos < 0 || rows[i].pos >= ctx->c.max_ctx) return fail(ctx, "row %d: position %d exceeds max_ctx %d", i, rows[i].pos, ctx->c.max_ctx);
    }
    const int slot = ring_acquire(ctx);
    VVRow* pin = ctx->rows_pin + (size_t)slot * ctx->rows_cap;
    for (int i = 0; i < n_rows; ++i) { pin[i].cache = rows[i].cache; pin[i].pos = rows[i].pos; }
    HIPCHK(ctx, hipMemcpyAsync(ctx->rows_dev, pin, sizeof(VVRow) * n_rows, hipMemcpyHostToDevice, st));
    HIPCHK(ctx, hipEventRecord(ctx->ring_ev[slot], st));
    ctx->launches = 0;
    if (!ctx->rope_ready) {
        VVCHK(vv_rope_table_launch(ctx->inv_freq, ctx->rope_tab, ctx->c.max_ctx, ctx->D / 2, st));
        ctx->rope_ready = true;
    }
    VVLmPlan plan;
    if (vv_lm_pass_plan(pin, n_rows, {ctx->ws_rows, ctx->c.attn_splits, ctx->Hkv, ctx->tile3_ok, ctx->attn2_ok, ctx->p16_ok}, &plan))
        return fail(ctx, "a launch of %d rows must be consecutive positions of one cache (decode / ragged launches take <= %d rows)", n_rows, ctx->ws_rows);
    char key[160]; snprintf(key, 160, "lm:%d:%p:%p:%d:%d:%d:%d:%d", n_rows, (const void*)x_in_dev, (void*)hidden_out_dev, l0, l1, final_norm,
                            plan.key_mode, plan.key_split);
    return graphed(ctx, key, st, [&]() { return lm_body(ctx, st, n_rows, x_in_dev, hidden_out_dev, l0, l1, final_norm, plan); });
}

extern "C" int vv_kv_import_at(vv_ctx* ctx, void* stream, int cache, int layer, int pos0, int n_pos, const void* k_dev, const void* v_dev, int src_dtype) {
    VV_SHARED;
    hipStream_t st = (hipStream_t)stream;
    if (cache < 0 || cache >= 2 * ctx->c.n_slots) return fail(ctx, "cache id %d out of range", cache);
    if (layer < 0 || layer >= ctx->c.lm_layers) return fail(ctx, "layer %d out of range", layer);
    if (pos0 < 0 || n_pos < 0 || (int64_t)pos0 + n_pos > ctx->c.max_ctx) return fail(ctx, "positions [%d, %d) exceed max_ctx %d", pos0, pos0 + n_pos, ctx->c.max_ctx);
    if (n_pos == 0) return 0;
    const size_t off = ((size_t)cache * ctx->cache_stride + (size_t)layer * ctx->layer_stride) * 2;
    VVCHK(vv_kv_import_launch(k_dev, v_dev, src_dtype, (char*)ctx->kc + off, (char*)ctx->vc + off, n_pos, ctx->Hkv, ctx->D, ctx->head_stride, pos0, st));
    return 0;
}
extern "C" int vv_kv_move(vv_ctx* ctx, void* stream, int cache, int src_pos, int dst_pos) {
    VV_SHARED;
    hipStream_t st = (hipStream_t)stream;
    if (cache < 0 || cache >= 2 * ctx->c.n_slots) return fail(ctx, "cache id %d out of range", cache);
    if (src_pos < 0 || dst_pos < 0 || src_pos >= ctx->c.max_ctx || dst_pos >= ctx->c.max_ctx)
        return fail(ctx, "vv_kv_move: positions %d -> %d outside [0, %d)", src_pos, dst_pos, ctx->c.max_ctx);
    if (src_pos == dst_pos) return 0;
    const size_t off = (size_t)cache * ctx->cache_stride * 2;
    ctx->launches++;
    VVCHK(vv_kv_move_launch((char*)ctx->kc + off, (char*)ctx->vc + off, ctx->c.lm_layers, ctx->Hkv, ctx->D, ctx->layer_stride, ctx->head_stride,
                            src_pos, dst_pos, st));
    return 0;
}
extern "C" int vv_kv_import(vv_ctx* ctx, void* stream, int cache, int layer, int n_pos, const void* k_dev, const void* v_dev, int src_dtype) {
    return vv_kv_import_at(ctx, stream, cache, layer, 0, n_pos, k_dev, v_dev, src_dtype);
}
extern "C" int vv_kv_export(vv_ctx* ctx, void* stream, int cache, int layer, int pos0, int n_pos, void* k_out_dev, void* v_out_dev, int dst_dtype) {
    VV_SHARED;
    hipStream_t st = (hipStream_t)stream;
    if (cache < 0 || cache >= 2 * ctx->c.n_slots) return fail(ctx, "cache id %d out of range", cache);
    if (layer < 0 || layer >= ctx->c.lm_layers) return fail(ctx, "layer %d out of range", layer);
    if (pos0 < 0 || n_pos < 0 || (int64_t)pos0 + n_pos > ctx->c.max_ctx)
        return fail(ctx, "vv_kv_export: positions [%d, %lld) exceed max_ctx %d", pos0, (long long)pos0 + n_pos, ctx->c.max_ctx);
    if (dst_dtype != 0 && dst_dtype != 1) return fail(ctx, "vv_kv_export: dst_dtype %d (0 = fp32, 1 = bf16)", dst_dtype);
    if (n_pos == 0) return 0;
    if (!k_out_dev || !v_out_dev) return fail(ctx, "vv_kv_export: null output");
    if (((uintptr_t)k_out_dev | (uintptr_t)v_out_dev) & 15) return fail(ctx, "vv_kv_export: outputs must be 16-byte aligned");
    const size_t off = ((size_t)cache * ctx->cache_stride + (size_t)layer * ctx->layer_stride) * 2;
    VVCHK(vv_kv_export_launch((char*)ctx->kc + off, (char*)ctx->vc + off, k_out_dev, v_out_dev, dst_dtype, n_pos, ctx->Hkv, ctx->D, ctx->head_stride, pos0, st));
    return 0;
}
extern "C" int64_t vv_kv_snapshot_bytes(vv_ctx* ctx, int n_pos) {
    if (n_pos < 0 || n_pos > ctx->c.max_ctx) return fail(ctx, "vv_kv_snapshot_bytes: %d positions outside [0, max_ctx %d]", n_pos, ctx->c.max_ctx);
    return (int64_t)ctx->c.lm_layers * ctx->Hkv * ((n_pos + 31) & ~31) * ctx->D * 2;
}
static int kv_span_copy(vv_ctx* ctx, void* stream, const char* who, int cache, int n_pos, void* k_dev, void* v_dev, int to_cache) {
    VV_SHARED;
    hipStream_t st = (hipStream_t)stream;
    if (cache < 0 || cache >= 2 * ctx->c.n_slots) return fail(ctx, "%s: cache id %d out of range", who, cache);
    if (n_pos < 0 || n_pos > ctx->c.max_ctx) return fail(ctx, "%s: %d positions outside [0, max_ctx %d]", who, n_pos, ctx->c.max_ctx);
    if (n_pos == 0) return 0;
    if (!k_dev || !v_dev) return fail(ctx, "%s: null snapshot buffer", who);
    if (((uintptr_t)k_dev | (uintptr_t)v_dev) & 15) return fail(ctx, "%s: snapshot buffers must be 16-byte aligned", who);
    const size_t off = (size_t)cache * ctx->cache_stride * 2;
    VVCHK(vv_kv_span_copy_launch((char*)ctx->kc + off, (char*)ctx->vc + off, k_dev, v_dev, to_cache, ctx->c.lm_layers, ctx->Hkv, ctx->D,
                                 ctx->layer_stride, ctx->head_stride, n_pos, st));
    return 0;
}
extern "C" int vv_kv_snapshot(vv_ctx* ctx, void* stream, int cache, int n_pos, void* k_out_dev, void* v_out_dev) {
    return kv_span_copy(ctx, stream, "vv_kv_snapshot", cache, n_pos, k_out_dev, v_out_dev, 0);
}
extern "C" int vv_kv_restore(vv_ctx* ctx, void* stream, int cache, int n_pos, const void* k_dev, const void* v_dev) {
    return kv_span_copy(ctx, stream, "vv_kv_restore", cache, n_pos, (void*)k_dev, (void*)v_dev, 1);
}
extern "C" int vv_add_type_embedding(vv_ctx* ctx, void* stream, int n, const float* x_dev, int type, float* out_dev) {
    VV_SHARED;
    hipStream_t st = (hipStream_t)stream;
    if (!ctx->tts_types) return fail(ctx, "engine was not configured with tts_layers");
    if (type < 0 || type > 1) return fail(ctx, "type must be 0 (speech) or 1 (text)");
    VVCHK(vv_add_rows_launch(x_dev, ctx->tts_types + (size_t)type * ctx->H, out_dev, n, ctx->H, st));
    return 0;
}

extern "C" int vv_eos_logit(vv_ctx* ctx, void* stream, int n, const float* hidden_dev, float* out_dev) {
    VV_SHARED;
    hipStream_t st = (hipStream_t)stream;
// ... 78 lines not shown
```

### vibevoice_amd/csrc/gemv.hip

```cpp
#include <array>
#include <utility>
#include "vv_common.h"
#include "vv_device.h"
#include "vv_launch.h"
#include "vv_w13.h"

#ifdef VV_GEMM_TIMING
#define VV_STAMP(i) do { if (a.dbg && blockIdx.x == 0 && threadIdx.x == 0) a.dbg[i] = __builtin_amdgcn_s_memtime(); } while (0)
#define VV_BSTAMP(i) do { if (a.dbg && threadIdx.x == 0 && blockIdx.y * gridDim.x + blockIdx.x < 3200) a.dbg[16 + 2 * (blockIdx.y * gridDim.x + blockIdx.x) + (i)] = __builtin_amdgcn_s_memrealtime(); } while (0)
#else
#define VV_BSTAMP(i) do { } while (0)
#define VV_STAMP(i) do { } while (0)
#endif

namespace {

constexpr int U = 8;


template <int XS, int PRO, int EPI, int MR, int WPB, int PARTS = 0, int SL = 0, int WF = 0>
__global__ __launch_bounds__(WPB * 64) void vv_gemv_kernel(const u32x4* __restrict__ pW, const u32x4* __restrict__ pW2,
                                                           const float* __restrict__ pX, float* __restrict__ pY,
                                                           const float* __restrict__ pnw, int pT, int pN, int pK, int pldx,
                                                           int pldy, const VVGemm a) {
    constexpr bool DUAL = (EPI == VV_EPI_SWIGLU);
    constexpr int NM = DUAL ? 2 : 1;
    constexpr bool FOLD = (PRO == VV_PRO_RMS_MOD) && MR <= 4;
    constexpr int NOP = (PRO == VV_PRO_RMS_MOD && !FOLD) ? 2 : 1;
    constexpr int MRS = FOLD ? 2 * MR : MR;
    static_assert(WF == 0 || (XS == 1 && NOP == 1 && MR <= 4 && PARTS == 0 && SL == 0), "W13 forms: bf16 mode, decode rows, one operand");
    constexpr int GSB = MRS * 16 + (MR == 16 ? 16 : 0);
    __shared__ __attribute__((aligned(16))) unsigned char stg_all[WPB * NOP * XS * U * 4 * GSB];
    __shared__ f32x4 red[WPB][NM * NOP][64];
    __shared__ float ssq_sh[WPB][MR];
    __shared__ float ssq1_sh[PRO == VV_PRO_NORMDW ? WPB : 1];
    asm volatile("" ::"s"(a.mod_scale), "s"(a.mod_shift), "s"(a.addvec), "s"(a.bias), "s"(a.nscale), "s"(a.gate));
    asm volatile("" ::"s"(a.ld_mod), "s"(a.ld_gate), "s"(a.x_row_mod), "s"(a.add_rows_per_vec),
                 "s"(a.eps), "s"(a.z), "s"(a.x0p), "s"(a.coef), "s"(a.cfg), "s"(a.n_cfg));
    asm volatile("" ::"s"(a.yparts), "s"(a.xa), "s"(a.ya), "s"(a.n_xa), "s"(a.n_ya), "s"(a.part_stride));
    if constexpr (EPI == VV_EPI_CFG_DPM) asm volatile("" ::"s"(a.sde_noise), "s"(a.cfg_rows));
    VV_STAMP(0);
    VV_BSTAMP(0);
    const int lane = threadIdx.x & 63;
    const int wave = __builtin_amdgcn_readfirstlane((int)(threadIdx.x >> 6));
    const int t_base = (MR == 16) ? (int)blockIdx.y * 16 : 0;
    const int T = min(MR, pT - t_base);
    const unsigned tile = blockIdx.x;
    const unsigned k_tiles = (unsigned)(pK + 31) >> 5;
    const unsigned KSB = (MR <= 4) ? gridDim.y : 1u;
    const unsigned ksb = (MR <= 4) ? blockIdx.y : 0u;
    const unsigned kchunk = (k_tiles + KSB - 1) / KSB;
    const unsigned kb0 = min(k_tiles, ksb * kchunk), kb1 = min(k_tiles, kb0 + kchunk);
    const unsigned kper = (kb1 - kb0 + WPB - 1) / WPB;
    const unsigned kt0 = kb0 + wave * kper;
    const unsigned kt1 = min(kb1, kt0 + kper);
    const bool has_k = kt0 < kt1;
    const int frow = lane & 15, fq = lane >> 4;
    unsigned char* stg = stg_all + (size_t)wave * (NOP * XS * U * 4 * GSB);
    const unsigned kk = lane * 4;
    const unsigned st_off = ((kk >> 5) * 4 + ((kk & 31) >> 3)) * GSB + (kk & 7) * 2;

    const u32x4* wbase = pW + (size_t)tile * k_tiles * 64 + lane;
    const u32x4* wbase2 = DUAL ? pW2 + (size_t)tile * k_tiles * 64 + lane : nullptr;
    const unsigned char* gbase = reinterpret_cast<const unsigned char*>(pW) + (size_t)tile * (k_tiles >> 2) * VV_W13_GROUP;
    const unsigned char* gbase2 = reinterpret_cast<const unsigned char*>(pW2) + (size_t)tile * (k_tiles >> 2) * VV_W13_GROUP;
    constexpr int RG = WF ? (DUAL ? 2 : 3) : 1;
    const unsigned g_lo = kt0 >> 2, g_hi = (kt1 + 3) >> 2, ph = kt0 & 3;
    VVW13Raw raw[RG][NM];
    auto g_load = [&](unsigned g, VVW13Raw (&dst)[NM]) {
        g = min(g, g_hi - 1);
        dst[0] = vv_w13_load(gbase + g * VV_W13_GROUP, lane);
        if constexpr (DUAL) dst[1] = vv_w13_load(gbase2 + g * VV_W13_GROUP, lane);
    };

    unsigned xoff_sl[SL ? MR : 1];
    if constexpr (SL) {
#pragma unroll
        for (int r = 0; r < MR; ++r) {
            const int rg = t_base + r;
            const int j = rg / a.sl_T, tt = rg - j * a.sl_T;
            xoff_sl[r] = (r < T) ? (a.sl_x ? (unsigned)(vv_slot_id(a.sl_id, j) * a.sl_x + tt * pldx) : (unsigned)(rg * pldx)) : 0u;
        }
    }
    constexpr int MODR = (PRO == VV_PRO_RMS_MOD) ? MR : 1;
    constexpr int ADDR = (PRO == VV_PRO_ADD_SILU) ? MR : 1;
    constexpr int PR = (PARTS == 1) ? MR : 1;
    constexpr int DWH = (PRO == VV_PRO_NORMDW) ? 6 : 1, DWT = (PRO == VV_PRO_NORMDW) ? 7 : 1;
    struct XR { float4 x[MR]; float4 p0[PR]; float4 p1[PR]; float4 sc[MODR]; float4 sh[MODR]; float4 addv[ADDR]; float4 nwv;
                float4 dh[DWH]; float4 dt[DWT]; float4 db, dg, dn; };
    auto x_load = [&](unsigned ktb, XR& R) {
        unsigned k = ktb * 32 + kk;
        const bool kin = k < min(kt1 * 32, (unsigned)pK);
        if (!kin) k = 0;
        R.nwv = pnw ? *reinterpret_cast<const float4*>(pnw + k) : float4{1.f, 1.f, 1.f, 1.f};
        if constexpr (PRO == VV_PRO_NORMDW) {
#pragma unroll
            for (int j = 0; j < 6; ++j) R.dh[j] = *reinterpret_cast<const float4*>(a.dw_hist + (unsigned)(j * pK) + k);
#pragma unroll
            for (int j = 0; j < 7; ++j) R.dt[j] = *reinterpret_cast<const float4*>(a.dw_w + (unsigned)(j * pK) + k);
            R.db = *reinterpret_cast<const float4*>(a.dw_b + k);
            R.dg = *reinterpret_cast<const float4*>(a.dw_gamma + k);
            R.dn = *reinterpret_cast<const float4*>(a.dw_nw + k);
        }
#pragma unroll
        for (int r = 0; r < MR; ++r) {
            if (r < T) {
                const int rg = t_base + r;
                const int xr_idx = a.x_row_mod > 0 ? rg % a.x_row_mod : rg;
                if constexpr (SL) R.x[r] = *reinterpret_cast<const float4*>(pX + xoff_sl[r] + k);
                else R.x[r] = *reinterpret_cast<const float4*>(pX + (unsigned)(xr_idx * pldx) + k);
                if constexpr (PARTS == 1) {
                    R.p0[r] = *reinterpret_cast<const float4*>(a.xa + (unsigned)(xr_idx * pldx) + k);
                    R.p1[r] = *reinterpret_cast<const float4*>(a.xa + (unsigned)(a.part_stride + xr_idx * pldx) + k);
                }
                if constexpr (PRO == VV_PRO_ADD_SILU) {
                    const int av = a.add_rows_per_vec > 0 ? rg / a.add_rows_per_vec : 0;
                    R.addv[r] = *reinterpret_cast<const float4*>(a.addvec + (unsigned)(av * pK) + k);
                }
                if constexpr (PRO == VV_PRO_RMS_MOD) {
                    R.sc[r] = *reinterpret_cast<const float4*>(a.mod_scale + (unsigned)(rg * a.ld_mod) + k);
                    R.sh[r] = *reinterpret_cast<const float4*>(a.mod_shift + (unsigned)(rg * a.ld_mod) + k);
                }
            }
        }
    };
    auto w_load = [&](unsigned ktb, u32x4 (&dst)[U][NM]) {
#pragma unroll
        for (int u = 0; u < U; ++u) {
            const unsigned kt = min(ktb + u, kt1 - 1);
            dst[u][0] = __builtin_nontemporal_load(wbase + kt * 64);
            if constexpr (DUAL) dst[u][1] = __builtin_nontemporal_load(wbase2 + kt * 64);
        }
    };
    XR R;
    u32x4 wA[WF ? 1 : U][NM], wB[WF ? 1 : U][NM];
    if constexpr (WF) {
        if (has_k) {
            x_load(kt0, R);
#pragma unroll
            for (int q = 0; q < RG; ++q) g_load(g_lo + q, raw[q]);
        }
    } else
    if (has_k) { x_load(kt0, R); w_load(kt0, wA); }
    __builtin_amdgcn_sched_barrier(0);
    VV_STAMP(1);
    float rs1 = 1.0f;
    if constexpr (PRO == VV_PRO_NORMDW) {
        float s1 = 0.f;
        for (unsigned ktb = kt0; ktb < kt1; ktb += U) {
            const unsigned k = ktb * 32 + kk;
            if (k < min(kt1 * 32, (unsigned)pK)) {
                const float4 v = *reinterpret_cast<const float4*>(pX + k);
                s1 += v.x * v.x + v.y * v.y + v.z * v.z + v.w * v.w;
            }
        }
        s1 = vv_wave_sum_dpp(s1);
        if (lane == 0) ssq1_sh[wave] = s1;
        __syncthreads();
        float tot = 0.f;
#pragma unroll
        for (int w = 0; w < WPB; ++w) tot += ssq1_sh[w];
        rs1 = rsqrtf(tot / (float)pK + a.eps);
    }

    const int n0 = tile * 16 + fq * 4;
    const bool epi_lane = (wave == 0) && frow < T && n0 < pN;
    float4 pre_y = {0.f, 0.f, 0.f, 0.f}, pre_b = {0.f, 0.f, 0.f, 0.f}, pre_g = {1.f, 1.f, 1.f, 1.f};
    float4 pre_y0 = {0.f, 0.f, 0.f, 0.f}, pre_y1 = {0.f, 0.f, 0.f, 0.f};
    unsigned yrow_off = (unsigned)((t_base + frow) * pldy);
    if constexpr (SL) {
        const int rg = min(t_base + frow, pT - 1);
        const int j = rg / a.sl_T, tt = rg - j * a.sl_T;
        yrow_off = a.sl_y ? (unsigned)(vv_slot_id(a.sl_id, j) * a.sl_y + tt * pldy) : (unsigned)(rg * pldy);
    }
    if (epi_lane) {
        if constexpr (EPI == VV_EPI_BIAS || EPI == VV_EPI_BIAS_GELU || EPI == VV_EPI_RESID) {
            if (a.bias) pre_b = *reinterpret_cast<const float4*>(a.bias + n0);
        }
        if constexpr (EPI == VV_EPI_RESID || EPI == VV_EPI_GATED_RESID) {
            pre_y = *reinterpret_cast<const float4*>(pY + (yrow_off + (unsigned)n0));
            if constexpr (PARTS == 2) {
                const float* yp0 = a.ya + (unsigned)((t_base + frow) * pldy + n0);
                pre_y0 = *reinterpret_cast<const float4*>(yp0);
                pre_y1 = *reinterpret_cast<const float4*>(yp0 + a.part_stride);
            }
            if constexpr (EPI == VV_EPI_GATED_RESID) pre_g = *reinterpret_cast<const float4*>(a.gate + (unsigned)((t_base + frow) * a.ld_gate + n0));
            else if (a.nscale) pre_g = *reinterpret_cast<const float4*>(a.nscale + n0);
        }
    }

    f32x4 acc[NM * NOP];
#pragma unroll
    for (int i = 0; i < NM * NOP; ++i) acc[i] = f32x4{0.f, 0.f, 0.f, 0.f};
    float ssq[MR];
#pragma unroll
    for (int r = 0; r < MR; ++r) ssq[r] = 0.f;

    auto x_stage = [&](unsigned ktb, const XR& R) {
        const unsigned k = ktb * 32 + kk;
        const float msk = (k < min(kt1 * 32, (unsigned)pK)) ? 1.f : 0.f;
#pragma unroll
        for (int r = 0; r < MR; ++r) {
            if (r < T) {
                float v[4] = {R.x[r].x, R.x[r].y, R.x[r].z, R.x[r].w};
                if constexpr (PARTS == 1) {
                    v[0] = (v[0] + R.p0[r].x) + R.p1[r].x; v[1] = (v[1] + R.p0[r].y) + R.p1[r].y;
                    v[2] = (v[2] + R.p0[r].z) + R.p1[r].z; v[3] = (v[3] + R.p0[r].w) + R.p1[r].w;
                }
                v[0] *= msk; v[1] *= msk; v[2] *= msk; v[3] *= msk;
                if constexpr (PRO == VV_PRO_RMS) {
                    ssq[r] += v[0] * v[0] + v[1] * v[1] + v[2] * v[2] + v[3] * v[3];
                    v[0] *= R.nwv.x; v[1] *= R.nwv.y; v[2] *= R.nwv.z; v[3] *= R.nwv.w;
                } else if constexpr (PRO == VV_PRO_NORMDW) {
                    if (r == 0) {
                        const float xn[4] = {R.dn.x, R.dn.y, R.dn.z, R.dn.w}, bb[4] = {R.db.x, R.db.y, R.db.z, R.db.w};
                        const float gg[4] = {R.dg.x, R.dg.y, R.dg.z, R.dg.w}, n2[4] = {R.nwv.x, R.nwv.y, R.nwv.z, R.nwv.w};
                        float hn[4], xo[4];
#pragma unroll
                        for (int e = 0; e < 4; ++e) {
                            hn[e] = v[e] * rs1 * xn[e];
                            float acc = bb[e];
#pragma unroll
                            for (int j = 0; j < 6; ++j) acc += reinterpret_cast<const float*>(&R.dt[j])[e] * reinterpret_cast<const float*>(&R.dh[j])[e];
                            acc += reinterpret_cast<const float*>(&R.dt[6])[e] * hn[e];
                            xo[e] = (v[e] + gg[e] * acc) * msk;
                        }
                        if (tile == 0 && msk != 0.f) {
                            *reinterpret_cast<float4*>(a.dw_xout + k) = float4{xo[0], xo[1], xo[2], xo[3]};
                            *reinterpret_cast<float4*>(a.dw_hnew + k) = float4{hn[0], hn[1], hn[2], hn[3]};
                        }
                        ssq[r] += xo[0] * xo[0] + xo[1] * xo[1] + xo[2] * xo[2] + xo[3] * xo[3];
#pragma unroll
                        for (int e = 0; e < 4; ++e) v[e] = xo[e] * n2[e];
                    }
                } else if constexpr (PRO == VV_PRO_RMS_MOD) {
                    ssq[r] += v[0] * v[0] + v[1] * v[1] + v[2] * v[2] + v[3] * v[3];
                    v[0] = (v[0] * R.nwv.x) * (1.f + R.sc[r].x); v[1] = (v[1] * R.nwv.y) * (1.f + R.sc[r].y);
                    v[2] = (v[2] * R.nwv.z) * (1.f + R.sc[r].z); v[3] = (v[3] * R.nwv.w) * (1.f + R.sc[r].w);
                    float sh4[4] = {R.sh[r].x * msk, R.sh[r].y * msk, R.sh[r].z * msk, R.sh[r].w * msk};
                    uint2 sparts[XS];
                    vv_split_bf16<XS>(sh4, sparts);
#pragma unroll
                    for (int p = 0; p < XS; ++p) {
                        if constexpr (FOLD) *reinterpret_cast<uint2*>(stg + p * (U * 4 * GSB) + st_off + (MR + r) * 16) = sparts[p];
                        else *reinterpret_cast<uint2*>(stg + (XS + p) * (U * 4 * GSB) + st_off + r * 16) = sparts[p];
                    }
                } else if constexpr (PRO == VV_PRO_ADD_SILU) {
                    v[0] = vv_silu(v[0] + R.addv[r].x) * msk; v[1] = vv_silu(v[1] + R.addv[r].y) * msk;
                    v[2] = vv_silu(v[2] + R.addv[r].z) * msk; v[3] = vv_silu(v[3] + R.addv[r].w) * msk;
                }
                uint2 parts[XS];
                vv_split_bf16<XS>(v, parts);
#pragma unroll
                for (int p = 0; p < XS; ++p)
                    *reinterpret_cast<uint2*>(stg + p * (U * 4 * GSB) + st_off + r * 16) = parts[p];
            }
        }
    };
    auto mma = [&](unsigned ktb, const u32x4 (&wb)[U][NM]) {
#pragma unroll
        for (int u = 0; u < U; ++u) {
            if (ktb + u < kt1) {
#pragma unroll
                for (int p = 0; p < XS; ++p) {
                    u32x4 f = u32x4{0u, 0u, 0u, 0u};
                    if (frow < MRS) f = *reinterpret_cast<const u32x4*>(stg + (size_t)((p * U + u) * 4 + fq) * GSB + frow * 16);
                    const bf16x8 xb = __builtin_bit_cast(bf16x8, f);
#pragma unroll
                    for (int i = 0; i < NM; ++i)
                        acc[i] = __builtin_amdgcn_mfma_f32_16x16x32_bf16(__builtin_bit_cast(bf16x8, wb[u][i]), xb, acc[i], 0, 0, 0);
                    if constexpr (NOP == 2) {
                        u32x4 f2 = u32x4{0u, 0u, 0u, 0u};
                        if (frow < MR) f2 = *reinterpret_cast<const u32x4*>(stg + (size_t)(((XS + p) * U + u) * 4 + fq) * GSB + frow * 16);
                        const bf16x8 sb = __builtin_bit_cast(bf16x8, f2);
#pragma unroll
                        for (int i = 0; i < NM; ++i)
                            acc[NM + i] = __builtin_amdgcn_mfma_f32_16x16x32_bf16(__builtin_bit_cast(bf16x8, wb[u][i]), sb, acc[NM + i], 0, 0, 0);
                    }
                }
            }
        }
    };

    if constexpr (WF) {
        float wscale[NM];
        {
            const size_t tail = (size_t)gridDim.x * (k_tiles >> 2) * VV_W13_GROUP;
            wscale[0] = vv_w13_scale(reinterpret_cast<const unsigned*>(reinterpret_cast<const unsigned char*>(pW) + tail)[tile]);
            if constexpr (DUAL) wscale[1] = vv_w13_scale(reinterpret_cast<const unsigned*>(reinterpret_cast<const unsigned char*>(pW2) + tail)[tile]);
        }
        if (has_k) {
            x_stage(kt0, R);
            VV_STAMP(2);
            const unsigned klen = kt1 - kt0;
            auto mma1 = [&](const u32x4 (&f)[NM][4], int t, unsigned slot) {
                u32x4 xf = u32x4{0u, 0u, 0u, 0u};
                if (frow < MRS) xf = *reinterpret_cast<const u32x4*>(stg + (size_t)(slot * 4 + fq) * GSB + frow * 16);
                const bf16x8 xb = __builtin_bit_cast(bf16x8, xf);
#pragma unroll
                for (int i = 0; i < NM; ++i)
                    acc[i] = __builtin_amdgcn_mfma_f32_16x16x32_bf16(__builtin_bit_cast(bf16x8, f[i][t]), xb, acc[i], 0, 0, 0);
            };
            auto wstep = [&](unsigned i, auto s0c, auto s1c) {
                constexpr int sl[2] = {decltype(s0c)::value, decltype(s1c)::value};
#pragma unroll
                for (int gi = 0; gi < 2; ++gi) {
                    u32x4 f[NM][4];
                    if (gi == 0) {
                        if (ph > 0 && i > 0) {
#pragma unroll
                            for (int m = 0; m < NM; ++m) vv_w13_unpack(raw[sl[0]][m], wscale[m], f[m]);
#pragma unroll
                            for (int t = 0; t < 3; ++t)
                                if ((unsigned)t < ph && 8 * i + t - ph < klen) mma1(f, t, 8 + t - ph);
                        }
                        if (i > 0 && 8 * i < klen) x_stage(kt0 + 8 * i, R);
                        if (8 * (i + 1) < klen) x_load(kt0 + 8 * (i + 1), R);
                    }
#pragma unroll
                    for (int m = 0; m < NM; ++m) vv_w13_unpack(raw[sl[gi]][m], wscale[m], f[m]);
                    const unsigned gn = g_lo + 2 * i + gi + RG;
                    if (gn < g_hi) g_load(gn, raw[sl[gi]]);
#pragma unroll
                    for (int t = 0; t < 4; ++t)
                        if ((unsigned)t >= (gi == 0 ? ph : 0u) && 8 * i + 4 * gi + t - ph < klen) mma1(f, t, 4 * gi + t - ph);
                }
            };
            const unsigned n_wb = (ph + klen + 7) >> 3;
            using S0 = std::integral_constant<int, 0>; using S1 = std::integral_constant<int, 1>; using S2 = std::integral_constant<int, 2>;
            if constexpr (RG == 2) {
#pragma unroll 1
                for (unsigned i = 0; i < n_wb; ++i) wstep(i, S0{}, S1{});
            } else {
#pragma unroll 1
                for (unsigned i = 0; i < n_wb; i += 3) {
                    wstep(i, S0{}, S1{});
                    if (i + 1 < n_wb) wstep(i + 1, S2{}, S0{});
                    if (i + 2 < n_wb) wstep(i + 2, S1{}, S2{});
                }
            }
        }
    } else
    if (has_k) {
        x_stage(kt0, R);
        VV_STAMP(2);
        if constexpr (DUAL) {
#pragma unroll 1
            for (unsigned ktb = kt0; ktb < kt1; ktb += U) {
                const bool n1 = ktb + U < kt1;
                if (n1) x_load(ktb + U, R);
                mma(ktb, wA);
                if (n1) { w_load(ktb + U, wA); x_stage(ktb + U, R); }
            }
        } else
#pragma unroll 1
        for (unsigned ktb = kt0; ktb < kt1; ktb += 2 * U) {
            const bool n1 = ktb + U < kt1, n2 = ktb + 2 * U < kt1;
            if (n1) { x_load(ktb + U, R); w_load(ktb + U, wB); }
            mma(ktb, wA);
            if (n1) x_stage(ktb + U, R);
            if (n2) { x_load(ktb + 2 * U, R); w_load(ktb + 2 * U, wA); }
            if (n1) mma(ktb + U, wB);
            if (n2) x_stage(ktb + 2 * U, R);
        }
    }

    VV_STAMP(3);
#pragma unroll
    for (int i = 0; i < NM * NOP; ++i) red[wave][i][lane] = acc[i];
    if constexpr (PRO == VV_PRO_RMS || PRO == VV_PRO_RMS_MOD || PRO == VV_PRO_NORMDW) {
#pragma unroll
        for (int r = 0; r < MR; ++r) {
            const float s = (r < T) ? vv_wave_sum_dpp(ssq[r]) : 0.f;
            if (lane == 0) ssq_sh[wave][r] = s;
        }
    }
    VV_STAMP(4);
    __syncthreads();
    VV_STAMP(5);
    if (wave != 0) return;
#pragma unroll
    for (int w = 1; w < WPB; ++w)
#pragma unroll
        for (int i = 0; i < NM * NOP; ++i) acc[i] += red[w][i][lane];
    f32x4 shf[FOLD ? NM : 1];
    if constexpr (FOLD) {
#pragma unroll
        for (int i = 0; i < NM; ++i)
#pragma unroll
            for (int r = 0; r < 4; ++r) {
                const float av = acc[i][r];
                const int sv = __builtin_amdgcn_update_dpp(0, __builtin_bit_cast(int, av), 0x100 + MR, 0xF, 0xF, true);
                shf[i][r] = __builtin_bit_cast(float, sv);
            }
    }
    if (!epi_lane) return;
    float rs = 1.0f;
    if constexpr (PRO == VV_PRO_RMS || PRO == VV_PRO_RMS_MOD || PRO == VV_PRO_NORMDW) {
        float s = 0.f;
#pragma unroll
        for (int w = 0; w < WPB; ++w) s += ssq_sh[w][frow];
        rs = rsqrtf(s / (float)pK + a.eps);
    }
    float o[4] = {acc[0][0] * rs, acc[0][1] * rs, acc[0][2] * rs, acc[0][3] * rs};
    float up[4] = {0.f, 0.f, 0.f, 0.f};
    if constexpr (DUAL) { up[0] = acc[1][0] * rs; up[1] = acc[1][1] * rs; up[2] = acc[1][2] * rs; up[3] = acc[1][3] * rs; }
    if constexpr (NOP == 2) {
#pragma unroll
        for (int r = 0; r < 4; ++r) { o[r] += acc[NM][r]; if constexpr (DUAL) up[r] += acc[NM + 1][r]; }
    }
    if constexpr (FOLD) {
#pragma unroll
        for (int r = 0; r < 4; ++r) { o[r] += shf[0][r]; if constexpr (DUAL) up[r] += shf[1][r]; }
    }
    const float pb[4] = {pre_b.x, pre_b.y, pre_b.z, pre_b.w};
    const float py[4] = {(pre_y.x + pre_y0.x) + pre_y1.x, (pre_y.y + pre_y0.y) + pre_y1.y, (pre_y.z + pre_y0.z) + pre_y1.z, (pre_y.w + pre_y0.w) + pre_y1.w};
    const float pg[4] = {pre_g.x, pre_g.y, pre_g.z, pre_g.w};
    if constexpr (EPI == VV_EPI_BIAS) {
#pragma unroll
        for (int r = 0; r < 4; ++r) o[r] += pb[r];
    } else if constexpr (EPI == VV_EPI_BIAS_GELU) {
#pragma unroll
        for (int r = 0; r < 4; ++r) o[r] = vv_gelu_erf(o[r] + pb[r]);
    } else if constexpr (EPI == VV_EPI_SWIGLU) {
#pragma unroll
        for (int r = 0; r < 4; ++r) o[r] = vv_silu(o[r]) * up[r];
    } else if constexpr (EPI == VV_EPI_RESID) {
#pragma unroll
        for (int r = 0; r < 4; ++r) o[r] = (ksb == 0) ? py[r] + pg[r] * (o[r] + pb[r]) : pg[r] * o[r];
    } else if constexpr (EPI == VV_EPI_GATED_RESID) {
#pragma unroll
        for (int r = 0; r < 4; ++r) o[r] = (ksb == 0) ? py[r] + pg[r] * o[r] : pg[r] * o[r];
    }
    if constexpr (EPI == VV_EPI_CFG_DPM) {
        const int nc = a.n_cfg;
        const VVSolverCoef cf = vv_solver_coef(a.coef, a.sde_noise != nullptr);
        float cfg = a.cfg;
        if (a.cfg_rows && frow < nc) cfg = a.cfg_rows[frow];
#pragma unroll
        for (int r = 0; r < 4; ++r) {
            const float vu = __shfl(o[r], lane + nc);
            const int n = n0 + r;
            if (frow < nc && n < pN) {
                const unsigned zi = (unsigned)(frow * pN + n);
                float x0, zn;
                vv_cfg_dpm_update(o[r], vu, cfg, a.z[zi], a.x0p[zi], cf, a.sde_noise != nullptr, [&] { return a.sde_noise[zi]; }, x0, zn);
                a.x0p[zi] = x0;
                a.z[zi] = zn;
                a.z[zi + (unsigned)(nc * pN)] = zn;
            }
        }
        return;
    }
    float* yp = (ksb == 0 ? pY : a.yparts + (unsigned)((ksb - 1) * a.part_stride)) + (yrow_off + (unsigned)n0);
    *reinterpret_cast<float4*>(yp) = float4{o[0], o[1], o[2], o[3]};
    VV_STAMP(6);
    VV_BSTAMP(1);
}

}

extern "C" int vv_gemv_ok(const VVGemm* a) { return vv_gemv_eligible(a); }

using GemvKernel = void (*)(const u32x4*, const u32x4*, const float*, float*, const float*, int, int, int, int, int, const VVGemm);
template <int F, int I, int XS>
static constexpr GemvKernel gemv_kernel_at() {
    constexpr const VVGemvFamily& f = vv_gemv_families[F];
    if constexpr (I < f.n && XS <= f.xs_max) return vv_gemv_kernel<XS, f.pair[I].pro, f.pair[I].epi, f.mr, f.wpb, f.parts, f.sl>;
    else return nullptr;
}
template <size_t... J>
static constexpr std::array<GemvKernel, sizeof...(J)> gemv_kernel_table(std::index_sequence<J...>) {
    return {gemv_kernel_at<J / (VV_GEMV_MAX_PAIRS * VV_GEMV_MAX_XS), J / VV_GEMV_MAX_XS % VV_GEMV_MAX_PAIRS, J % VV_GEMV_MAX_XS + 1>()...};
}
static const auto gemv_kernels = gemv_kernel_table(std::make_index_sequence<VV_GF_COUNT * VV_GEMV_MAX_PAIRS * VV_GEMV_MAX_XS>{});

template <size_t... J>
static constexpr std::array<std::array<GemvKernel, 2>, sizeof...(J)> gemv_w13_table(std::index_sequence<J...>) {
    return {{{vv_gemv_kernel<1, vv_gemv_w13_forms[J].pro, vv_gemv_w13_forms[J].epi, vv_gemv_w13_forms[J].mr, vv_gemv_w13_forms[J].wpb, 0, 0, 0>,
              vv_gemv_kernel<1, vv_gemv_w13_forms[J].pro, vv_gemv_w13_forms[J].epi, vv_gemv_w13_forms[J].mr, vv_gemv_w13_forms[J].wpb, 0, 0, 1>}...}};
}
static const auto gemv_w13_kernels = gemv_w13_table(std::make_index_sequence<VV_GEMV_W13_FORMS>{});

static GemvKernel gemv_kernel(const VVGemvForm& form, int pro, int epi) {
    for (int f = 0; f < VV_GF_COUNT; ++f) {
        const VVGemvFamily& fam = vv_gemv_families[f];
        if (fam.mr != form.mr || fam.wpb != form.wpb || fam.parts != form.parts || fam.sl != form.sl || form.xs > fam.xs_max) continue;
        for (int i = 0; i < fam.n; ++i)
            if (fam.pair[i].pro == pro && fam.pair[i].epi == epi) return gemv_kernels[(f * VV_GEMV_MAX_PAIRS + i) * VV_GEMV_MAX_XS + form.xs - 1];
    }
    return nullptr;
}

extern "C" int vv_gemv_launch(VVGemm a, int xs, hipStream_t s, int* form) {
    if (a.epi == VV_EPI_SWIGLU && !a.W2) return -1;
    VVGemvPlan p;
    if (!vv_gemv_plan(&a, xs, &p)) return VV_RC_NO_FORM;
    GemvKernel k = gemv_kernel(p.form, a.pro, a.epi);
    if (a.w13) {
        const int wi = vv_gemv_w13_form(&a, xs);
        if (wi < 0 || (a.epi == VV_EPI_SWIGLU && !a.w13_2)) return VV_RC_NO_FORM;
        k = gemv_w13_kernels[wi][1];
        a.W = (const u32x4*)a.w13; a.W2 = (const u32x4*)a.w13_2;
    }
    if (form) { form[0] = p.form.xs; form[1] = p.form.mr; form[2] = p.form.wpb; form[3] = p.form.parts; form[4] = p.form.sl; }
    hipLaunchKernelGGL(k, p.grid, dim3(p.form.wpb * 64), 0, s, a.W, a.W2, a.X, a.Y, a.nw, a.T, a.N, a.K, a.ldx, a.ldy, a);
    return vv_launch_rc(0);
}

extern "C" int vv_gemv_w13_form_launch(VVGemm a, int mr, int wpb, hipStream_t s) {
    if (a.epi == VV_EPI_SWIGLU && (!a.W2 || (a.w13 && !a.w13_2))) return -1;
    const int wi = vv_gemv_w13_find(a.pro, a.epi, mr, wpb);
    if (wi < 0 || !vv_gemv_eligible(&a) || !vv_gemv_w13_shape(&a, 1) || a.T > mr) return VV_RC_NO_FORM;
    const GemvKernel k = gemv_w13_kernels[wi][a.w13 ? 1 : 0];
    if (a.w13) { a.W = (const u32x4*)a.w13; a.W2 = (const u32x4*)a.w13_2; }
    hipLaunchKernelGGL(k, dim3(a.N / 16, 1), dim3(wpb * 64), 0, s, a.W, a.W2, a.X, a.Y, a.nw, a.T, a.N, a.K, a.ldx, a.ldy, a);
    return vv_launch_rc(0);
}
```

### vibevoice_amd/csrc/gemv_plan.h

```cpp
#pragma once
#include "vv_common.h"

struct VVGemvForm { int xs, mr, wpb, parts, sl; };
struct VVGemvPlan { VVGemvForm form; dim3 grid; };

struct VVGemvPair { int pro, epi; };
struct VVGemvFamily {
    int mr, wpb, parts, sl, xs_max, n;
    const VVGemvPair* pair;
    template <int N>
    constexpr VVGemvFamily(int mr_, int wpb_, int parts_, int sl_, int xs_max_, const VVGemvPair (&p)[N])
        : mr(mr_), wpb(wpb_), parts(parts_), sl(sl_), xs_max(xs_max_), n(N), pair(p) {}
    constexpr bool has(int pro, int epi) const {
        for (int i = 0; i < n; ++i) if (pair[i].pro == pro && pair[i].epi == epi) return true;
        return false;
    }
};
inline constexpr VVGemvPair vv_gemv_pairs[] = {
    {VV_PRO_NONE, VV_EPI_STORE}, {VV_PRO_NONE, VV_EPI_BIAS}, {VV_PRO_NONE, VV_EPI_RESID}, {VV_PRO_NONE, VV_EPI_GATED_RESID},
    {VV_PRO_RMS, VV_EPI_BIAS}, {VV_PRO_RMS, VV_EPI_BIAS_GELU}, {VV_PRO_RMS, VV_EPI_SWIGLU}, {VV_PRO_RMS, VV_EPI_RESID}, {VV_PRO_RMS, VV_EPI_STORE},
    {VV_PRO_RMS_MOD, VV_EPI_SWIGLU}, {VV_PRO_RMS_MOD, VV_EPI_CFG_DPM}, {VV_PRO_RMS_MOD, VV_EPI_STORE},
    {VV_PRO_ADD_SILU, VV_EPI_STORE}, {VV_PRO_NORMDW, VV_EPI_BIAS_GELU}};
inline constexpr VVGemvPair vv_gemv_pairs_w4[] = {
    {VV_PRO_RMS, VV_EPI_SWIGLU}, {VV_PRO_RMS_MOD, VV_EPI_SWIGLU}, {VV_PRO_RMS, VV_EPI_BIAS_GELU}, {VV_PRO_RMS, VV_EPI_BIAS},
// ... 23 lines not shown
    {4, 16, 0, 0, 1, vv_gemv_pairs_w16},
    {16, 8, 0, 0, 2, vv_gemv_pairs_wide},
    {16, 4, 0, 0, 1, vv_gemv_pairs_wide4},
    {16, 4, 0, 0, 1, vv_gemv_pairs_wide_mod},
    {4, 8, 1, 0, 3, vv_gemv_pairs_parts_x},
    {2, 4, 1, 0, 1, vv_gemv_pairs_parts_x_wide},
    {4, 4, 1, 0, 1, vv_gemv_pairs_parts_x_wide},
    {4, 8, 2, 0, 3, vv_gemv_pairs_parts_y},
    {16, 8, 0, 1, 2, vv_gemv_pairs_slots},
    {16, 4, 0, 1, 1, vv_gemv_pairs_slots}};

inline bool vv_gemv_eligible(const VVGemm* a) {
    const VVGemvFamily* const fam = vv_gemv_families;
    if (a->T < 1) return false;
    if (a->T > 4 || a->sl_n > 0) { if (!fam[VV_GF_WIDE].has(a->pro, a->epi) && !fam[VV_GF_WIDE_MOD].has(a->pro, a->epi)) return false; }
    else if (!fam[VV_GF_DEFAULT].has(a->pro, a->epi)) return false;
    if (a->sl_n > 0) {
        if (a->sl_n > 8 || a->sl_T < 1 || a->T != a->sl_n * a->sl_T || a->sl_x < 0 || a->sl_y < 0 || (a->sl_x & 3) || (a->sl_y & 3)) return false;
        if (a->kgrid > 1 || a->n_xa || a->n_ya || a->x_row_mod > 0 || a->add_rows_per_vec > 0) return false;
        if (!fam[VV_GF_SLOTS].has(a->pro, a->epi)) return false;
        for (int j = 0; j < a->sl_n; ++j)
            if (a->sl_id[j] < 0 || (int64_t)a->sl_id[j] * a->sl_x + (int64_t)a->sl_T * a->ldx >= (1LL << 30) ||
                (int64_t)a->sl_id[j] * a->sl_y + (int64_t)a->sl_T * a->ldy >= (1LL << 30)) return false;
    }
    if ((a->x_row_mod > 0 || a->add_rows_per_vec > 0) && a->pro != VV_PRO_ADD_SILU) return false;
    if (a->epi == VV_EPI_CFG_DPM && (a->n_cfg < 1 || a->T != 2 * a->n_cfg || a->T > 16 || !a->z || !a->x0p || !a->coef)) return false;
    if (a->pro == VV_PRO_NORMDW) {
        if (a->T != 1 || a->sl_n > 0 || a->kgrid > 1 || a->n_xa || a->n_ya || !a->dw_hist || !a->dw_w || !a->dw_b || !a->dw_gamma ||
            !a->dw_nw || !a->dw_xout || !a->dw_hnew || a->dw_xout == a->X) return false;
        if ((((uintptr_t)a->dw_hist) | ((uintptr_t)a->dw_w) | ((uintptr_t)a->dw_b) | ((uintptr_t)a->dw_gamma) | ((uintptr_t)a->dw_nw) |
             ((uintptr_t)a->dw_xout) | ((uintptr_t)a->dw_hnew)) & 15) return false;
        if ((int64_t)7 * a->K >= (1LL << 30)) return false;
    }
    if ((a->K & 3) || (a->ldx & 3) || (((uintptr_t)a->X) & 15)) return false;
    if (a->pro == VV_PRO_RMS_MOD && (a->ld_mod & 3)) return false;
    if (a->nw && (((uintptr_t)a->nw) & 15)) return false;
    if (a->K < 32) return false;
    if ((int64_t)a->T * a->ldy >= (1LL << 30) || (int64_t)a->T * a->ldx >= (1LL << 30)) return false;
    if ((a->N & 3) || (a->ldy & 3)) return false;
    if ((((uintptr_t)a->Y) & 15) || (a->bias && (((uintptr_t)a->bias) & 15))) return false;
    if (a->nscale && (((uintptr_t)a->nscale) & 15)) return false;
    if (a->epi == VV_EPI_GATED_RESID && ((a->ld_gate & 3) || (((uintptr_t)a->gate) & 15))) return false;
    if (a->pro == VV_PRO_RMS_MOD && ((((uintptr_t)a->mod_scale) & 15) || (((uintptr_t)a->mod_shift) & 15))) return false;
    if (a->pro == VV_PRO_ADD_SILU && (((uintptr_t)a->addvec) & 15)) return false;
    if (a->kgrid > 1 && (a->T > 4 || a->kgrid != 3 || a->pro != VV_PRO_NONE || !a->yparts || (a->part_stride & 3) ||
                         (a->epi != VV_EPI_RESID && a->epi != VV_EPI_GATED_RESID) || (((uintptr_t)a->yparts) & 15))) return false;
    if ((a->n_xa > 0 && (!a->xa || (((uintptr_t)a->xa) & 15))) || (a->n_ya > 0 && (!a->ya || (((uintptr_t)a->ya) & 15)))) return false;
    if ((a->n_xa != 0 && a->n_xa != 2) || (a->n_ya != 0 && a->n_ya != 2) || (a->n_xa && a->n_ya)) return false;
    if ((a->n_xa || a->n_ya) && ((a->part_stride & 3) || a->T > 4 || !fam[a->n_xa > 0 ? VV_GF_PARTS_X : VV_GF_PARTS_Y].has(a->pro, a->epi))) return false;
    return true;
}

constexpr int VV_GEMV_WIDE_TILES = 256;
constexpr int VV_GEMV_W16_MAX_TILES = 128, VV_GEMV_W16_MIN_KTILES = 96;
constexpr int VV_GEMV_WIDE4_WGS = 128;

inline bool vv_gemv_plan(const VVGemm* a, int xs, VVGemvPlan* out) {
    if (!vv_gemv_eligible(a)) return false;
    const VVGemvFamily* const fam = vv_gemv_families;
    const int n_tiles = (a->N + 15) / 16, k_tiles = (a->K + 31) / 32;
    const bool rows16 = a->T > 4 || a->sl_n > 0;
    const int grid_y = rows16 ? (a->T + 15) / 16 : a->kgrid > 1 ? a->kgrid : 1;
    const auto fits = [&](int f) { return xs >= 1 && xs <= fam[f].xs_max && fam[f].has(a->pro, a->epi); };
    const bool wide = n_tiles > VV_GEMV_WIDE_TILES, wide4 = (int64_t)n_tiles * grid_y > VV_GEMV_WIDE4_WGS;
    int f = VV_GF_DEFAULT;
    if (a->sl_n > 0) f = wide4 && fits(VV_GF_SLOTS4) ? VV_GF_SLOTS4 : VV_GF_SLOTS;
    else if (rows16 && wide4 && fits(VV_GF_WIDE4)) f = VV_GF_WIDE4;
    else if (rows16) f = fits(VV_GF_WIDE) ? VV_GF_WIDE : VV_GF_WIDE_MOD;
    else if (a->n_xa > 0 && wide && a->T <= 2 && fits(VV_GF_PARTS_X_ROWS2_W4)) f = VV_GF_PARTS_X_ROWS2_W4;
    else if (a->n_xa > 0) f = wide && fits(VV_GF_PARTS_X_W4) ? VV_GF_PARTS_X_W4 : VV_GF_PARTS_X;
    else if (a->n_ya > 0) f = VV_GF_PARTS_Y;
    else if (a->kgrid > 1) f = VV_GF_DEFAULT;
    else if (wide && a->T <= 2 && fits(VV_GF_ROWS2_W4)) f = VV_GF_ROWS2_W4;
    else if (wide && fits(VV_GF_ROWS4_W4)) f = VV_GF_ROWS4_W4;
    else if (n_tiles <= VV_GEMV_W16_MAX_TILES && k_tiles >= VV_GEMV_W16_MIN_KTILES && fits(VV_GF_W16)) f = VV_GF_W16;
    if (!fits(f)) return false;
    out->form = {xs, fam[f].mr, fam[f].wpb, fam[f].parts, fam[f].sl};
    out->grid = dim3(n_tiles, grid_y);
    return true;
}

struct VVGemvW13Form { int pro, epi, mr, wpb; };
inline constexpr VVGemvW13Form vv_gemv_w13_forms[] = {
    {VV_PRO_RMS_MOD, VV_EPI_SWIGLU, 2, 4}, {VV_PRO_RMS_MOD, VV_EPI_SWIGLU, 4, 8}, {VV_PRO_NONE, VV_EPI_GATED_RESID, 4, 8}};
constexpr int VV_GEMV_W13_FORMS = sizeof(vv_gemv_w13_forms) / sizeof(vv_gemv_w13_forms[0]);
inline int vv_gemv_w13_find(int pro, int epi, int mr, int wpb) {
    for (int i = 0; i < VV_GEMV_W13_FORMS; ++i) {
        const VVGemvW13Form& f = vv_gemv_w13_forms[i];
        if (f.pro == pro && f.epi == epi && f.mr == mr && f.wpb == wpb) return i;
    }
    return -1;
}
inline bool vv_gemv_w13_shape(const VVGemm* a, int xs) {
    return xs == 1 && (a->K & 127) == 0 && (a->N & 15) == 0 && a->T <= 4 && a->kgrid <= 1 && a->n_xa == 0 && a->n_ya == 0 && a->sl_n == 0;
}
inline int vv_gemv_w13_form(const VVGemm* a, int xs) {
    VVGemvPlan p;
    if (!vv_gemv_w13_shape(a, xs) || !vv_gemv_plan(a, xs, &p) || p.form.parts || p.form.sl) return -1;
    return vv_gemv_w13_find(a->pro, a->epi, p.form.mr, p.form.wpb);
}

constexpr int VV_TILE_BM = 64;
#define VV_TILE_COMBOS(X)                                                                      \
    X(VV_PRO_NONE, VV_EPI_STORE) X(VV_PRO_NONE, VV_EPI_BIAS) X(VV_PRO_NONE, VV_EPI_RESID)      \
    X(VV_PRO_RMS, VV_EPI_BIAS) X(VV_PRO_RMS, VV_EPI_BIAS_GELU) X(VV_PRO_RMS, VV_EPI_SWIGLU)    \
    X(VV_PRO_RMS, VV_EPI_STORE)

inline bool vv_tile_eligible(const VVGemm* a, int xs) {
    if (a->T < 32 || xs > 2) return false;
    {
        const int per_wg = 4 * (a->epi == VV_EPI_SWIGLU ? 1 : 2);
        const int64_t wgs = (int64_t)(((a->N + 15) / 16 + per_wg - 1) / per_wg) * ((a->T + VV_TILE_BM - 1) / VV_TILE_BM);
        const int min_wgs = a->sl_n > 0 ? 40 : 48;
        if (wgs < min_wgs) return false;
    }
    if (a->sl_n > 0) {
        if (a->sl_n > 8 || a->sl_T < 1 || a->T != a->sl_n * a->sl_T || a->sl_x < 0 || a->sl_y < 0 || (a->sl_x & 3) || (a->sl_y & 3)) return false;
    }
    if ((a->K & 3) || (a->ldx & 3) || (a->N & 3) || (a->ldy & 3)) return false;
    if ((((uintptr_t)a->X) | ((uintptr_t)a->Y)) & 15) return false;
    if ((a->nw && (((uintptr_t)a->nw) & 15)) || (a->bias && (((uintptr_t)a->bias) & 15)) || (a->nscale && (((uintptr_t)a->nscale) & 15))) return false;
    if (a->x_row_mod > 0 || a->add_rows_per_vec > 0 || a->kgrid > 1 || a->n_xa > 0 || a->n_ya > 0 || a->ksplit > 0) return false;
    if (a->K < 32) return false;
    if (a->epi == VV_EPI_SWIGLU && !a->W2) return false;
#define X(P, E) if (a->pro == P && a->epi == E) return true;
    VV_TILE_COMBOS(X)
#undef X
    return false;
}

enum { VV_ROUTE_TILE, VV_ROUTE_GEMV, VV_ROUTE_GENERAL, VV_ROUTE_NONE };
inline int vv_gemm_route(const VVGemm* a, int xs) {
    VVGemvPlan p;
    if (vv_tile_eligible(a, xs)) return VV_ROUTE_TILE;
    if (a->sl_n > 0) return xs <= 2 && vv_gemv_plan(a, xs, &p) ? VV_ROUTE_GEMV : VV_ROUTE_NONE;
    if (a->ksplit <= 0 && vv_gemv_plan(a, xs, &p)) return VV_ROUTE_GEMV;
    if (a->kgrid > 1 || a->n_xa > 0 || a->n_ya > 0) return VV_ROUTE_NONE;
    return VV_ROUTE_GENERAL;
}

struct VVGemmGeneralPlan {
    bool vec, dual;
    int wpb, maxr, nt;
    int ks, t_pad;
    dim3 grid;
    size_t lds;
};
constexpr int VV_GG_NT2_TILE_PAIRS = 4096;
constexpr int VV_GG_WAVES = 2048, VV_GG_MIN_KSTEPS = 8;
constexpr int VV_GG_FEW_TILES = 512;
inline int vv_pow2_floor(int v) { int p = 1; while (p * 2 <= v) p *= 2; return p; }

inline int vv_gemm_general_plan(const VVGemm* a, int xs, VVGemmGeneralPlan* p) {
    const int n_tiles = (a->N + 15) / 16, k_tiles = (a->K + 31) / 32, t_tiles = (a->T + 15) / 16;
    p->dual = a->epi == VV_EPI_SWIGLU;
    if (p->dual && !a->W2) return -1;
    p->vec = ((a->K & 3) == 0) && ((a->ldx & 3) == 0) && ((((uintptr_t)a->X) & 15) == 0) && (a->pro != VV_PRO_RMS_MOD || (a->ld_mod & 3) == 0);
    if (!p->vec && p->dual) return VV_RC_NO_FORM;
    p->t_pad = a->T < 16 ? a->T : 16;
    p->wpb = (p->t_pad <= 4 && p->vec) ? 8 : 4;
    p->maxr = p->wpb == 8 ? 4 : 16;
    p->nt = (!p->dual && p->vec && (long)n_tiles * t_tiles >= VV_GG_NT2_TILE_PAIRS) ? 2 : 1;
    const long work = ((long)n_tiles + p->nt - 1) / p->nt * t_tiles;
    int ks = 1;
    if (a->ksplit > 0) ks = a->ksplit;
    else {
        const int want = (int)((VV_GG_WAVES + work - 1) / work);
// ... 15 lines not shown
```

### vibevoice_amd/csrc/pass_plan.h

```cpp
#pragma once
#include "vv_common.h"

constexpr int VV_P16_MIN_ROWS = 5, VV_P16_MAX_ROWS = 16;
inline bool vv_p16_rows(int rows) { return rows >= VV_P16_MIN_ROWS && rows <= VV_P16_MAX_ROWS; }

constexpr int VV_ATTN_SPLIT_POS = 1024;
constexpr int VV_ATTN_TARGET_WGS = 256;
constexpr int VV_CHUNK_MIN_ROWS = 8;
constexpr int VV_PREFILL_MIN_ROWS = 64;

enum { VV_LM_PREFILL, VV_LM_P16, VV_LM_GEMV };
enum { VV_ATTN_FUSED, VV_ATTN_PREFILL4, VV_ATTN_SPLIT_MERGE };

struct VVLmCaps { int ws_rows, attn_splits, Hkv; bool tile3_ok, attn2_ok, p16_ok; };

struct VVLmPlan {
    bool fused;
    bool contiguous;
    int route, attn;
    int attn_S;
    int attn_groups;
    bool zero_v_tail;
    int key_mode, key_split;
    int64_t kv_positions;
};

inline int vv_lm_pass_plan(const VVRow* rows, int n_rows, const VVLmCaps& c, VVLmPlan* p) {
    bool fused = true;
    for (int i = 0; i < n_rows && fused; ++i)
        for (int j = 0; j < i; ++j) if (rows[i].cache == rows[j].cache) { fused = false; break; }
    bool contiguous = !fused && n_rows >= VV_CHUNK_MIN_ROWS;
    for (int i = 1; i < n_rows && contiguous; ++i)
        if (rows[i].cache != rows[0].cache || rows[i].pos != rows[0].pos + i) contiguous = false;
    p->fused = fused; p->contiguous = contiguous;
    if (!contiguous && n_rows > c.ws_rows) return -1;
    int max_len = 1, n_long = 0;
    int64_t kv_positions = 0;
    for (int i = 0; i < n_rows; ++i) {
        const int len = rows[i].pos + 1;
        if (len > max_len) max_len = len;
        if (len > VV_ATTN_SPLIT_POS) ++n_long;
        kv_positions += len;
    }
    const int long_wgs = (n_long > 1 ? n_long : 1) * c.Hkv;
    int S = (VV_ATTN_TARGET_WGS + long_wgs - 1) / long_wgs;
    if (S < 1) S = 1;
    if (S > c.attn_splits) S = c.attn_splits;
    const int by_len = (max_len + VV_ATTN_SPLIT_POS - 1) / VV_ATTN_SPLIT_POS;
    if (S > by_len) S = by_len;
    p->attn_S = S;
    p->kv_positions = kv_positions;
    const bool chunk_attn = contiguous && c.attn2_ok;
    if (contiguous && c.tile3_ok && n_rows >= VV_PREFILL_MIN_ROWS) { p->route = VV_LM_PREFILL; p->attn = VV_ATTN_PREFILL4; }
    else {
        p->route = vv_p16_rows(n_rows) && c.p16_ok && fused ? VV_LM_P16 : VV_LM_GEMV;
        p->attn = fused ? VV_ATTN_FUSED : chunk_attn ? VV_ATTN_PREFILL4 : VV_ATTN_SPLIT_MERGE;
    }
    p->attn_groups = p->attn == VV_ATTN_SPLIT_MERGE ? (n_rows + c.ws_rows - 1) / c.ws_rows : 0;
    p->zero_v_tail = p->route == VV_LM_PREFILL || chunk_attn;
    p->key_mode = fused ? 1 : (contiguous ? 2 : 0);
    p->key_split = chunk_attn ? 0 : S;
    return 0;
}

constexpr int VV_ADA_TILE_ABOVE_ROWS = 32;

enum { VV_ADA_PER_STEP, VV_ADA_TILE, VV_ADA_ROWS16 };
enum { VV_HEAD_P16, VV_HEAD_GEMV };
enum { VV_FINAL_P16_CFG,
       VV_FINAL_SEAM,
       VV_FINAL_GEMM_CFG,
       VV_FINAL_GEMM };

struct VVHeadCaps { bool p16_ok, p16_shift, ada_p, mod_all, head_tail, w13; };

struct VVHeadPlan {
    int rows, n_steps;
    int ada;
    bool sh_tiles;
    int layers;
    bool seam;
    int final_stage;
    bool solver_step;
    bool w13;
};

inline VVHeadPlan vv_head_plan(int rows, int n_steps, int HF, int HL, int MODW, const VVHeadCaps& c, bool has_coef, bool solver_step = false) {
    VVHeadPlan p;
    p.rows = rows; p.n_steps = n_steps;
    const bool batch_ada = has_coef && c.mod_all;
    p.ada = !batch_ada ? VV_ADA_PER_STEP : (c.ada_p && rows * n_steps > VV_ADA_TILE_ABOVE_ROWS && (MODW & 3) == 0) ? VV_ADA_TILE : VV_ADA_ROWS16;
    p.sh_tiles = batch_ada && vv_p16_rows(rows) && c.p16_shift;
    p.layers = vv_p16_rows(rows) && c.p16_ok && (HF % 32) == 0 ? VV_HEAD_P16 : VV_HEAD_GEMV;
    p.seam = has_coef && rows == 2 && c.head_tail;
    p.w13 = c.w13 && p.layers == VV_HEAD_GEMV && rows <= 2;
    p.final_stage = p.layers == VV_HEAD_P16 && p.sh_tiles && has_coef && HL > 0 ? VV_FINAL_P16_CFG : has_coef ? VV_FINAL_GEMM_CFG : VV_FINAL_GEMM;
    p.solver_step = solver_step;
    if (solver_step) { p.sh_tiles = false; p.seam = false; p.final_stage = VV_FINAL_GEMM; }
    return p;
}
inline int vv_head_final(const VVHeadPlan& p, int step) { return p.seam && step + 1 < p.n_steps ? VV_FINAL_SEAM : p.final_stage; }
```

### vibevoice_amd/csrc/vv_common.h

```cpp
#pragma once
#include <hip/hip_runtime.h>
#include <stdint.h>

typedef __attribute__((ext_vector_type(8))) __bf16 bf16x8;
typedef __attribute__((ext_vector_type(4))) __bf16 bf16x4;
typedef __attribute__((ext_vector_type(2))) __bf16 bf16x2;
typedef __attribute__((ext_vector_type(4))) float f32x4;
typedef __attribute__((ext_vector_type(2))) float f32x2;
typedef __attribute__((ext_vector_type(4))) unsigned int u32x4;

#define VV_WAVE 64

static inline __host__ __device__ int64_t vv_packed_elems(int N, int K) {
    return (int64_t)((N + 15) / 16) * ((K + 31) / 32) * 512;
}

struct VVRow {
    int cache;
    int pos;
};

struct VVGemmWs {
    float* partials;
    unsigned* flags;
    unsigned* err;
    float* g3_partials;
    size_t g3_bytes;
};

enum { VV_PRO_NONE = 0, VV_PRO_RMS = 1, VV_PRO_RMS_MOD = 2, VV_PRO_ADD_SILU = 3,
       VV_PRO_NORMDW = 4 };
enum { VV_EPI_STORE = 0, VV_EPI_BIAS = 1, VV_EPI_BIAS_GELU = 2, VV_EPI_SWIGLU = 3,
       VV_EPI_RESID = 4, VV_EPI_GATED_RESID = 5, VV_EPI_CFG_DPM = 6,
       VV_EPI_QKV_ROPE = 7 };

struct VVGemm {
    const u32x4* W;
    const u32x4* W2;
    const float* X;
    float* Y;
    const float* nw;
    const float* mod_scale;
    const float* mod_shift;
    const float* addvec;
    const float* bias;
    const float* nscale;
    const float* gate;
    int T, N, K;
    int ldx, ldy, ld_mod, ld_gate;
    int pro, epi;
    int ksplit;
    int nt;
    int t_pad;
    float* z;
    float* x0p;
    const float* coef;
    float cfg;
    int n_cfg;
    const float* cfg_rows;
    const float* sde_noise;
    unsigned long long* dbg;
    int x_row_mod, add_rows_per_vec;
    float eps;
    int kgrid;
    float* yparts;
    const float* xa;
    const float* ya;
    int n_xa, n_ya;
    int part_stride;
    int sl_n, sl_T, sl_x, sl_y;
    int sl_id[8];
    const float* dw_hist;
    const float* dw_w;
    const float* dw_b;
    const float* dw_gamma;
    const float* dw_nw;
    float* dw_xout;
    float* dw_hnew;
    const void* w13;
    const void* w13_2;
};

struct VVGemv16p {
    const u32x4* W;
    const u32x4* W2;
    const u32x4* Xp;
    float* Y;
    unsigned char* Yp;
    const float* bias;
    const float* gate;
    int T, N, K, ldy, ld_gate;
    const float* ssq_in;
    int ssq_tiles;
    float eps;
    const u32x4* Xs;
    const float* pk_nw;
    const float* pk_sc;
    int ld_pk;
    float* ssq_out;
    float* z; float* x0p; const float* coef; float cfg; int n_cfg; const float* sde_noise;
    const float* cfg_rows;
};

struct VVTail {
    const u32x4* Wout;
    const u32x4* Win;
    const float* bin;
    const float* X;
    const float* xa; int n_xa, part_stride;
    const float* sc; const float* sh; int ld_mod;
    float* Xout;
    const float* z_in; const float* x0p_in;
    float* z_out; float* x0p_out;
    const float* coef; float cfg; int n_cfg; const float* sde_noise;
    const float* cfg_rows;
    int T, H, L; float eps;
};

struct VVSlotIds { int n; int id[8]; };
static inline VVSlotIds vv_slot_ids(const int* ids, int n) {
    VVSlotIds sl; sl.n = ids ? n : 0;
    for (int i = 0; i < 8; ++i) sl.id[i] = (ids && i < n) ? ids[i] : 0;
    return sl;
}
__device__ __forceinline__ int vv_slot_id(const int (&id)[8], int j) {
    int r = id[0];
#pragma unroll
    for (int i = 1; i < 8; ++i) r = (j == i) ? id[i] : r;
    return r;
}

struct VVRsRow { int stream, n_in, n_out, p0, b0; };
struct VVRsRows { VVRsRow r[16]; };
constexpr int VV_RS_MAX_OUT = 8192;

struct VVTpRow { long long k0, base; int stream, n_in, nblk, n_out, P, Q; };
struct VVTpRows { VVTpRow r[16]; };
constexpr int VV_TP_HS = 240, VV_TP_N = 480, VV_TP_DELTA = 160;
constexpr int VV_TP_HIST = 1280;
constexpr int VV_TP_MAX_IN = 7680;
constexpr int VV_TP_PAD = 896;
constexpr int VV_TP_BUF = VV_TP_HIST + VV_TP_MAX_IN + VV_TP_PAD;
constexpr int VV_TP_MAX_BLOCKS = 96;

struct VVLvRow { int stream, n_in, n_out, b0; float gain; };
struct VVLvRows { VVLvRow r[16]; };
constexpr int VV_LV_BUF = 8128;
constexpr int VV_LV_MAX_A = 2047;

template <class... K>
static inline hipError_t vv_raise_lds_limit(int bytes, K*... kernels) {
    hipError_t rc = hipSuccess;
    for (const void* k : {reinterpret_cast<const void*>(kernels)...}) {
        const hipError_t e = hipFuncSetAttribute(k, hipFuncAttributeMaxDynamicSharedMemorySize, bytes);
        if (rc == hipSuccess) rc = e;
    }
    return rc;
}

enum { VV_RC_NO_FORM = -3, VV_RC_NO_KERNEL = -4 };

inline thread_local int g_vv_launch_err = 0;
static inline int vv_launch_rc(int rc_ok) {
// ... 7 lines not shown
```

### vibevoice_amd/csrc/vv_launch.h

```cpp
#pragma once
#include "vv_common.h"
#include "gemv_plan.h"

struct VVSolverStep {
    const float* eps;
    const float* z_in; const float* m1_in; const float* m2_in;
    float* z_out; float* m1_out; float* m2_out;
    const float* coef;
    float cfg; const float* cfg_rows;
    const float* noise;
    int n, L;
    const u32x4* Win;
    float* Xout;
    int H, xs;
};
extern "C" {
int vv_gemm_launch(VVGemm a, int xs, hipStream_t s);
int vv_pack_launch(const void* src, int src_is_bf16, void* dst, int N, int K, int kind, int Cin, int Cout, int ksz, int stride, hipStream_t s);
int vv_rope_append_launch(int D, const float* qkv, const VVRow* rows, const float* inv_freq, float* q_out, void* kc, void* vc, int R, int Hq, int Hkv,
                          int64_t cache_stride, int64_t head_stride, hipStream_t s);
int vv_rope_table_launch(const float* inv_freq, void* tab, int n_pos, int half, hipStream_t s);
int vv_attn_fused_launch(int D, int xs, const float* qkv, const VVRow* rows, const void* rope_tab, void* kc, void* vc, int R, int Hq, int Hkv,
                         int64_t cache_stride, int64_t head_stride, int S, float* pm, float* pl, float* po, float* out, void* out_packed,
                         hipStream_t s);
int vv_attn_launch(int D, int xs, const float* q, const VVRow* rows, const void* kc, const void* vc, int R, int Hq, int Hkv, int64_t cache_stride,
                   int64_t head_stride, int S, float* pm, float* pl, float* po, float* out, hipStream_t s);
int vv_embed_launch(const void* table, const int* ids, float* out, int n, int H, hipStream_t s);
int vv_logits_full_launch(const void* table, const float* hidden, float* out, int n, int V, int H, hipStream_t s);
int vv_warp_valid_launch(const float* logits, const unsigned char* seen, float* out, int* survivors, int n, int V, const int* ids, int n_valid,
                         float pen, float temp, int do_sample, int top_k, float top_p, float min_p, hipStream_t s);
int vv_noise_rows_launch(float* out, int n, const uint32_t* keys, uint32_t stream0, int n_streams, int n_t, int width, hipStream_t s);
int vv_rmsnorm_rows_launch(const float* x, int ldx, float* y, int ldy, const float* w, int T, int C, float eps, hipStream_t s);
int vv_dwconv_res_launch(const float* nb, const float* x, float* xo, const float* w, const float* b, const float* gamma, int T, int C, hipStream_t s);
int vv_normdw_sliced_ok(int T, int C);
int vv_normdw_sliced_slots_launch(const float* xin, float* xout, float* nb, const float* nw, const float* w, const float* b, const float* gamma,
                                  int T, int C, float eps, const int* ids, int n, int64_t sx, int64_t snb, hipStream_t s);
int vv_normdw_rows_slots_launch(const float* xin, float* xout, float* nb, const float* nw, const float* w, const float* b, const float* gamma, int T,
                                int C, float eps, const int* ids, int n, int64_t sx, int64_t snb, hipStream_t s);
int vv_stem_conv_slots_launch(const float* in, const void* wp, const float* bias, float* out, int T, int N, const int* ids, int n, int64_t s_in,
                              int64_t s_out, hipStream_t s);
int vv_head_conv1_slots_launch(const float* x, const void* wp, const float* bias, float* out, int T, int Cin, const int* ids, int n, int64_t s_in,
                               int64_t s_out, hipStream_t s);
int vv_block1d_slots_launch(int C, int xs, const float* xin, float* xout, float* nst, const float* norm_w, const float* ffn_norm_w,
                            const float* gamma, const float* ffn_gamma, const float* dw_w, const float* dw_b, const float* b1, const float* b2,
                            const void* w1, const void* w2, int T, float eps, const int* ids, int n, int64_t sx, int64_t snst, hipStream_t s);
int vv_affine_slots_launch(const float* x, float* y, float mul, float add, int L, const int* ids, int n, int64_t stride, hipStream_t s);
int vv_normdw_launch(float* x, float* nb, const float* nw, const float* w, const float* b, const float* gamma, int T, int C, float eps,
                     hipStream_t s);
int vv_normdw_rows_ok(int T, int C);
int vv_shift_rows_launch(const void* tab, int n_entries, int maxC, hipStream_t s);
int vv_zero_hist_launch(const void* tab, int n_entries, hipStream_t s);
int vv_affine_launch(const float* x, float* y, float mul, float add, int n, hipStream_t s);
int vv_copy_launch(void* dst, const void* src, size_t bytes, hipStream_t s);
int vv_zero_launch(void* dst, size_t bytes, hipStream_t s);
int vv_sampler_init_launch(const float* noise, float* z, float* x0p, int nL, hipStream_t s);
int vv_tfreq_launch(const float* t, float* out, int n, hipStream_t s);
int vv_silu_launch(float* x, int n, hipStream_t s);
int vv_ada_in_launch(const float* cproj, const float* temb, float* out, int rows, int n_steps, int H, hipStream_t s);
int vv_add_rows_launch(const float* x, const float* v, float* y, int n, int C, hipStream_t s);
int vv_relu_launch(float* x, int n, hipStream_t s);
int vv_kv_import_launch(const void* k, const void* v, int src_bf16, void* kc, void* vc, int L, int Hkv, int D, int64_t head_stride, int pos0,
                        hipStream_t s);
int vv_kv_move_launch(void* kc, void* vc, int layers, int Hkv, int D, int64_t layer_stride, int64_t head_stride, int src, int dst, hipStream_t s);
int vv_kv_zero_v_tail_launch(void* vc, const VVRow* rows, int R, int layers, int Hkv, int D, int64_t cache_stride, int64_t layer_stride,
                             int64_t head_stride, int max_ctx, hipStream_t s);
int vv_kv_span_copy_launch(void* kc, void* vc, void* ks, void* vs, int to_cache, int layers, int Hkv, int D, int64_t layer_stride,
                           int64_t head_stride, int n_pos, hipStream_t s);
int vv_kv_export_launch(const void* kc, const void* vc, void* k, void* v, int dst_bf16, int L, int Hkv, int D, int64_t head_stride, int pos0,
                        hipStream_t s);
int vv_pcm16_launch(const float* x, short* out, int n, int samples, hipStream_t s);
int vv_cvt_launch(const void* src, void* dst, int64_t n, int to_bf16, hipStream_t s);
int vv_dw_transpose_launch(const float* src, float* dst, int C, hipStream_t s);
int vv_pack_rows_launch(const float* x, int ldx, const float* nw, float eps, void* xp, int T, int K, hipStream_t s);
int vv_unpack_rows_launch(const void* xp, float* x, int T, int K, hipStream_t s);
int vv_pack16_launch(const float* x, int ldx, int mode, const float* nw, float eps, const float* sc, const float* sh, int ld_mod, void* xp, int T,
                     int K, hipStream_t s);
int vv_gemv16p_launch(const void* W, const void* W2, const void* Xp, float* Y, void* Yp, const float* bias, const float* gate, int T, int N, int K,
                      int ldy, int ld_gate, int epi, hipStream_t s);
int vv_gemv16p_launch2(const VVGemv16p* a, int epi, int flags, hipStream_t s);
int vv_head_tail_ok(const VVTail* a);
int vv_head_tail_init();
int vv_head_tail_launch(const VVTail* a, hipStream_t s);
int vv_solver_step_ok(const VVSolverStep* a);
int vv_solver_step_fused_ok(const VVSolverStep* a);
int vv_solver_step_launch(const VVSolverStep* a, hipStream_t s);
int vv_pack16_tiles_launch(const float* x, int ldx, int64_t stride_outer, int n_inner, int64_t stride_inner, void* xp, int64_t tile_bytes, int T,
                           int K, int n_tiles, hipStream_t s);
int vv_ada_pack_launch(const float* cproj, const float* temb, void* xp, int rows, int n_steps, int H, hipStream_t s);
int vv_gemm3_launch(const void* W, const void* W2, const void* Xp, float* Y, void* Yp, const float* bias, int T, int N, int K, int ldy, int epi,
                    const VVGemmWs* ws, hipStream_t s);
int vv_gemm_qkv_rope_launch(const void* W, const void* Xp, const float* bias, int T, int K, int D, int Hq, int Hkv, const VVRow* rows_dev,
                            const void* rope_tab, float* q_out, void* kc, void* vc, int64_t cache_stride, int64_t head_stride, const VVGemmWs* ws,
                            hipStream_t s);
int vv_attn_prefill4_launch(int D, const float* q, const VVRow* rows, const void* kc, const void* vc, int R, int Hq, int Hkv, int64_t cache_stride,
                            int64_t head_stride, float* out, void* out_packed, hipStream_t s);
int vv_block1d_supported(int C);
int vv_gemv_ok(const VVGemm* a);
int vv_gemv_launch(VVGemm a, int xs, hipStream_t s, int* form);
int vv_gemv_w13_form_launch(VVGemm a, int mr, int wpb, hipStream_t s);
int vv_w13_pack_launch(const void* packed, void* twin, int N, int K, hipStream_t s);
int vv_w13_unpack_launch(const void* twin, void* packed, int N, int K, hipStream_t s);
int vv_tile_ok(const VVGemm* a, int xs);
int vv_tile_launch(VVGemm a, int xs, hipStream_t s);
int vv_lora_merge_launch(const void* base, void* dst, int N, int K, const float* a, const float* b, int r, float scale, int delta_bf16,
                         hipStream_t s);
int vv_unpack_launch(const void* packed, float* dst, int N, int K, hipStream_t s);
int vv_resample_lds_bytes(int L, int T, int n_in);
int vv_resample_rows_launch(const VVRsRows* rows, int n, int L, int M, int T, const float* coef, float* hist, int n_streams, const float* x,
                            int ld_in, void* out, int ld_out, int pcm16, hipStream_t s);
int vv_resample_once_launch(int L, int M, int T, const float* coef, int n, int n_in, const float* x, int ld_in, float* out, int ld_out, hipStream_t s);
int vv_resample_reset_launch(float* hist, int T, int n_streams, const int* ids, int n, hipStream_t s);
int vv_tempo_rows_launch(const VVTpRows* rows, int n, const float* window, float* hist, int* dstate, int n_streams, const float* x, int ld_in,
                         void* out, int ld_out, int pcm16, int* offsets, int ld_off, hipStream_t s);
int vv_tempo_once_launch(const float* window, int P, int Q, int n, int n_in, const float* x, int ld_in, float* out, int ld_out, int* offsets,
                         int ld_off, hipStream_t s);
int vv_tempo_reset_launch(float* hist, int* dstate, int n_streams, const int* ids, int n, hipStream_t s);
int vv_level_rows_launch(const VVLvRows* rows, int n, int A, int H, float c, float* hist, int n_streams, const float* x, int ld_in, void* out,
                         int ld_out, int pcm16, hipStream_t s);
int vv_level_once_launch(int A, int H, float g, float c, int n, int n_in, const float* x, int ld_in, float* out, int ld_out, hipStream_t s);
int vv_level_reset_launch(float* hist, int nh, int n_streams, const int* ids, int n, hipStream_t s);
}
```

### vibevoice_amd/csrc/w13.hip

```cpp
#include "vv_common.h"
#include "vv_w13.h"
#include "vv_launch.h"

namespace {

constexpr int PACK_WAVES = 4;

__global__ __launch_bounds__(PACK_WAVES * 64) void vv_w13_pack_kernel(const u32x4* __restrict__ W, unsigned char* __restrict__ out, int n_tiles, int k_tiles) {
    __shared__ unsigned red[PACK_WAVES];
    const int lane = threadIdx.x & 63, wave = threadIdx.x >> 6;
    const unsigned tile = blockIdx.x;
    const int groups = k_tiles >> 2;
    const u32x4* src = W + (size_t)tile * k_tiles * 64;
    unsigned emax = 0;
    for (int i = threadIdx.x; i < k_tiles * 64; i += PACK_WAVES * 64) {
        const u32x4 v = src[i];
#pragma unroll
        for (int d = 0; d < 4; ++d) emax = max(emax, max((v[d] >> 7) & 0xffu, (v[d] >> 23) & 0xffu));
    }
#pragma unroll
    for (int o = 32; o > 0; o >>= 1) emax = max(emax, (unsigned)__shfl_xor((int)emax, o));
    if (lane == 0) red[wave] = emax;
    __syncthreads();
    emax = red[0];
#pragma unroll
    for (int w = 1; w < PACK_WAVES; ++w) emax = max(emax, red[w]);
    __syncthreads();
    const float scale = vv_w13_scale(emax);
    unsigned char* planes = out + (size_t)tile * groups * VV_W13_GROUP;
    unsigned ok = 1;
    for (int g = wave; g < groups; g += PACK_WAVES) {
        u32x4 f[4];
#pragma unroll
        for (int t = 0; t < 4; ++t) f[t] = src[(g * 4 + t) * 64 + lane];
        unsigned hi[8] = {0, 0, 0, 0, 0, 0, 0, 0}, lo[5] = {0, 0, 0, 0, 0};
#pragma unroll
        for (int j = 0; j < 16; ++j) {
            const unsigned pair = f[j >> 2][j & 3];
            unsigned x = 0;
#pragma unroll
            for (int h = 0; h < 2; ++h) {
                const unsigned b = (pair >> (16 * h)) & 0xffffu, s = b >> 15, E = (b >> 7) & 0xffu, m = b & 0x7fu;
                const bool zero = (b & 0x7fffu) == 0;
                const bool rep = zero || (E >= 1 && E + 29 >= emax && emax <= 254);
                const unsigned c = (rep && !zero) ? E + 30 - emax : 0u;
                const unsigned hb = (s << 7) | (c << 2) | ((rep && !zero) ? m >> 5 : 0u);
                const unsigned l5 = (rep && !zero) ? m & 31u : 0u;
                hi[j >> 1] |= hb << (8 * (2 * (j & 1) + h));
                x |= l5 << (5 * h);
            }
            const int d = (10 * j) >> 5, s10 = (10 * j) & 31;
            lo[d] |= x << s10;
            if (s10 + 10 > 32) lo[d + 1] |= x >> (32 - s10);
        }
        VVW13Raw r;
        r.h0 = u32x4{hi[0], hi[1], hi[2], hi[3]}; r.h1 = u32x4{hi[4], hi[5], hi[6], hi[7]};
        r.lo = u32x4{lo[0], lo[1], lo[2], lo[3]}; r.l4 = lo[4];
        vv_w13_store(planes + (size_t)g * VV_W13_GROUP, lane, r);
        u32x4 back[4];
        vv_w13_unpack(r, scale, back);
#pragma unroll
        for (int t = 0; t < 4; ++t)
#pragma unroll
            for (int d = 0; d < 4; ++d) if (back[t][d] != f[t][d]) ok = 0;
    }
    ok = __all((int)ok) ? 1u : 0u;
    if (lane == 0) red[wave] = ok;
    __syncthreads();
    if (threadIdx.x == 0) {
        unsigned all = 1;
#pragma unroll
        for (int w = 0; w < PACK_WAVES; ++w) all &= red[w];
        unsigned* tail = reinterpret_cast<unsigned*>(out + (size_t)n_tiles * groups * VV_W13_GROUP);
        tail[tile] = emax;
        tail[n_tiles + tile] = all;
    }
}

__global__ __launch_bounds__(256) void vv_w13_fold_kernel(unsigned* __restrict__ tail, int n_tiles) {
    __shared__ unsigned red[4];
    unsigned ok = 1;
    for (int i = threadIdx.x; i < n_tiles; i += 256) ok &= tail[n_tiles + i];
    ok = __all((int)ok) ? 1u : 0u;
    if ((threadIdx.x & 63) == 0) red[threadIdx.x >> 6] = ok;
    __syncthreads();
    if (threadIdx.x == 0) tail[2 * n_tiles] = red[0] & red[1] & red[2] & red[3];
}

__global__ __launch_bounds__(PACK_WAVES * 64) void vv_w13_unpack_kernel(const unsigned char* __restrict__ in, u32x4* __restrict__ W, int n_tiles, int k_tiles) {
    const int lane = threadIdx.x & 63, wave = threadIdx.x >> 6;
    const unsigned tile = blockIdx.x;
    const int groups = k_tiles >> 2;
    const unsigned* tail = reinterpret_cast<const unsigned*>(in + (size_t)n_tiles * groups * VV_W13_GROUP);
    const float scale = vv_w13_scale(tail[tile]);
    const unsigned char* planes = in + (size_t)tile * groups * VV_W13_GROUP;
    u32x4* dst = W + (size_t)tile * k_tiles * 64;
    for (int g = wave; g < groups; g += PACK_WAVES) {
        const VVW13Raw r = vv_w13_load(planes + (size_t)g * VV_W13_GROUP, lane);
        u32x4 f[4];
        vv_w13_unpack(r, scale, f);
#pragma unroll
        for (int t = 0; t < 4; ++t) dst[(g * 4 + t) * 64 + lane] = f[t];
    }
}

}

extern "C" int vv_w13_pack_launch(const void* packed, void* twin, int N, int K, hipStream_t s) {
    if (!vv_w13_shape_ok(N, K)) return VV_RC_NO_FORM;
    const int n_tiles = N / 16, k_tiles = K / 32;
    hipLaunchKernelGGL(vv_w13_pack_kernel, dim3(n_tiles), dim3(PACK_WAVES * 64), 0, s, (const u32x4*)packed, (unsigned char*)twin, n_tiles, k_tiles);
    hipLaunchKernelGGL(vv_w13_fold_kernel, dim3(1), dim3(256), 0, s, reinterpret_cast<unsigned*>((unsigned char*)twin + vv_w13_plane_bytes(N, K)), n_tiles);
    return vv_launch_rc(0);
}
extern "C" int vv_w13_unpack_launch(const void* twin, void* packed, int N, int K, hipStream_t s) {
    if (!vv_w13_shape_ok(N, K)) return VV_RC_NO_FORM;
    const int n_tiles = N / 16, k_tiles = K / 32;
    hipLaunchKernelGGL(vv_w13_unpack_kernel, dim3(n_tiles), dim3(PACK_WAVES * 64), 0, s, (const unsigned char*)twin, (u32x4*)packed, n_tiles, k_tiles);
    return vv_launch_rc(0);
}
```

Measured before the change: 17.28.

## Extend compressed W13 weight twins to LM decode GEMVs with per-tile exactness fallback

Builds compressed W13 twins for the LM layer weights (qkv, o, gate/up, down) alongside the existing diffusion-head twins, and adds W13 GEMV forms for the LM decode prologue/epilogue combos. The GEMV kernel gains a third variant that checks per-tile exactness and falls back to loading the bf16 weights for tiles that did not round-trip losslessly, so non-exact matrices can still use the compressed path. The aim is to cut weight-memory traffic in small-row LM decode, which is bandwidth-bound. Exactness resolution becomes lazy, done at head-sample time, in exchange for extra device memory for the twins and more kernel variants.

```diff
diff --git a/vibevoice_amd/csrc/engine.hip b/vibevoice_amd/csrc/engine.hip
--- a/vibevoice_amd/csrc/engine.hip
+++ b/vibevoice_amd/csrc/engine.hip
@@ -208,6 +208,18 @@
         ctx->eos_w2 = alloc_packed(ctx, 1, H); add_mat(ctx, "eos.fc2.weight", 1, H, ctx->eos_w2, 0);
         ctx->eos_b2 = add_vec(ctx, "eos.fc2.bias", 1);
     }
+    {
+        const char* e = getenv("VVHIP_W13");
+        const bool on = !(e && e[0] == '0') && c.xsplit == 1;
+        ctx->w13_on = parent ? parent->w13_on : on && vv_w13_shape_ok(c.head_ffn, H) && vv_w13_shape_ok(H, c.head_ffn);
+        ctx->w13_lm = parent ? parent->w13_lm : on && !(e && !strcmp(e, "head"));
+    }
+    auto twin = [&](bool want, bool lm, const void* src, int N, int K, int n_par = 1) -> void* {
+        if (!want || !vv_w13_shape_ok(N, K)) return nullptr;
+        ctx->twins.push_back({walloc(ctx, (size_t)vv_w13_bytes(N, K)), src, N, K, lm});
+        for (int j = 0; j < n_par; ++j) ctx->w[ctx->w.size() - 1 - j].twin = (int)ctx->twins.size() - 1;
+        return ctx->twins.back().planes;
+    };
     ctx->layers.resize(c.lm_layers);
     for (int l = 0; l < c.lm_layers; ++l) {
         auto& L = ctx->layers[l];
@@ -220,13 +232,14 @@
         add_mat(ctx, p + "self_attn.q_proj.weight", Hq * D, H, L.wqkv, 0);
         add_mat(ctx, p + "self_attn.k_proj.weight", Hkv * D, H, L.wqkv, Hq * D / 16);
         add_mat(ctx, p + "self_attn.v_proj.weight", Hkv * D, H, L.wqkv, (Hq + Hkv) * D / 16);
+        L.tqkv = twin(ctx->w13_lm, true, L.wqkv, QKV, H, 3);
         add_vec(ctx, p + "self_attn.q_proj.bias", Hq * D, L.bqkv);
         add_vec(ctx, p + "self_attn.k_proj.bias", Hkv * D, L.bqkv + Hq * D);
         add_vec(ctx, p + "self_attn.v_proj.bias", Hkv * D, L.bqkv + (Hq + Hkv) * D);
-        L.wo = alloc_packed(ctx, H, Hq * D); add_mat(ctx, p + "self_attn.o_proj.weight", H, Hq * D, L.wo, 0);
-        L.wg = alloc_packed(ctx, I, H); add_mat(ctx, p + "mlp.gate_proj.weight", I, H, L.wg, 0);
-        L.wu = alloc_packed(ctx, I, H); add_mat(ctx, p + "mlp.up_proj.weight", I, H, L.wu, 0);
-        L.wd = alloc_packed(ctx, H, I); add_mat(ctx, p + "mlp.down_proj.weight", H, I, L.wd, 0);
+        L.wo = alloc_packed(ctx, H, Hq * D); add_mat(ctx, p + "self_attn.o_proj.weight", H, Hq * D, L.wo, 0); L.to = twin(ctx->w13_lm, true, L.wo, H, Hq * D);
+        L.wg = alloc_packed(ctx, I, H); add_mat(ctx, p + "mlp.gate_proj.weight", I, H, L.wg, 0); L.tg = twin(ctx->w13_lm, true, L.wg, I, H);
+        L.wu = alloc_packed(ctx, I, H); add_mat(ctx, p + "mlp.up_proj.weight", I, H, L.wu, 0); L.tu = twin(ctx->w13_lm, true, L.wu, I, H);
+        L.wd = alloc_packed(ctx, H, I); add_mat(ctx, p + "mlp.down_proj.weight", H, I, L.wd, 0); L.td = twin(ctx->w13_lm, true, L.wd, H, I);
     }
     const int n_caches = 2 * c.n_slots;
     ctx->head_stride = (int64_t)c.max_ctx * D;
@@ -286,12 +299,8 @@
     ctx->h_t2 = alloc_packed(ctx, H, H); add_mat(ctx, "head.t_embedder.mlp.2.weight", H, H, ctx->h_t2, 0);
     ctx->h_ada = alloc_packed(ctx, MODW, H);
     ctx->hl.resize(HL);
-    {
-        const char* e = getenv("VVHIP_W13");
-        ctx->w13_on = parent ? parent->w13_on : !(e && e[0] == '0') && c.xsplit == 1 && vv_w13_shape_ok(HF, H) && vv_w13_shape_ok(H, HF);
-    }
-    auto twin = [&](int N, int K) {
-        if (ctx->w13_on) ctx->w.back().w13 = walloc(ctx, (size_t)vv_w13_bytes(N, K));
+    auto htwin = [&](const void* src, int N, int K) {
+        twin(ctx->w13_on, false, src, N, K);
         return (int)ctx->w.size() - 1;
     };
     for (int l = 0; l < HL; ++l) {
@@ -299,9 +308,9 @@
         std::string p(nm);
         ctx->hl[l].norm = add_vec(ctx, p + "norm.weight", H);
         add_mat(ctx, p + "adaLN_modulation.1.weight", 3 * H, H, ctx->h_ada, l * 3 * H / 16);
-        ctx->hl[l].wg = alloc_packed(ctx, HF, H); add_mat(ctx, p + "ffn.gate_proj.weight", HF, H, ctx->hl[l].wg, 0); ctx->hl[l].ig = twin(HF, H);
-        ctx->hl[l].wu = alloc_packed(ctx, HF, H); add_mat(ctx, p + "ffn.up_proj.weight", HF, H, ctx->hl[l].wu, 0); ctx->hl[l].iu = twin(HF, H);
-        ctx->hl[l].wd = alloc_packed(ctx, H, HF); add_mat(ctx, p + "ffn.down_proj.weight", H, HF, ctx->hl[l].wd, 0); ctx->hl[l].id = twin(H, HF);
+        ctx->hl[l].wg = alloc_packed(ctx, HF, H); add_mat(ctx, p + "ffn.gate_proj.weight", HF, H, ctx->hl[l].wg, 0); ctx->hl[l].ig = htwin(ctx->hl[l].wg, HF, H);
+        ctx->hl[l].wu = alloc_packed(ctx, HF, H); add_mat(ctx, p + "ffn.up_proj.weight", HF, H, ctx->hl[l].wu, 0); ctx->hl[l].iu = htwin(ctx->hl[l].wu, HF, H);
+        ctx->hl[l].wd = alloc_packed(ctx, H, HF); add_mat(ctx, p + "ffn.down_proj.weight", H, HF, ctx->hl[l].wd, 0); ctx->hl[l].id = htwin(ctx->hl[l].wd, H, HF);
     }
     add_mat(ctx, "head.final_layer.adaLN_modulation.1.weight", 2 * H, H, ctx->h_ada, HL * 3 * H / 16);
     ctx->h_out = alloc_packed(ctx, L, H); add_mat(ctx, "head.final_layer.linear.weight", L, H, ctx->h_out, 0);
@@ -348,7 +357,6 @@
         for (size_t i = 0; i < ctx->w.size(); ++i) {
             if (ctx->w[i].name != parent->w[i].name || ctx->w[i].nelem != parent->w[i].nelem) { *out = ctx; return fail(ctx, "vv_create_shared: parameter table differs at '%s'", ctx->w[i].name.c_str()); }
             ctx->w[i].loaded = parent->w[i].loaded;
-            ctx->w[i].w13_ok = parent->w[i].w13_ok;
             if (ctx->w[i].name == "lm_head.weight") ctx->w[i].dev = parent->w[i].dev;
         }
         ctx->lm_head = parent->lm_head; ctx->lm_head_loaded = parent->lm_head_loaded;
@@ -484,16 +492,20 @@
 }
 
 int w13_repack(vv_ctx* ctx, int widx, hipStream_t st) {
-    Weight& w = ctx->w[widx];
-    if (!w.w13) return 0;
-    VVCHK(vv_w13_pack_launch(w.dev, w.w13, w.N, w.K, st));
-    HIPCHK(ctx, hipStreamSynchronize(st));
-    unsigned ok = 0;
-    HIPCHK(ctx, hipMemcpy(&ok, (const char*)w.w13 + vv_w13_plane_bytes(w.N, w.K) + (size_t)2 * (w.N / 16) * 4, 4, hipMemcpyDeviceToHost));
-    const bool now = ok == 1;
-    if (now == w.w13_ok) return 0;
-    w.w13_ok = now;
-    return drop_graphs(ctx, {"samp:", "sde:", "rows:", "gen:"});
+    const Weight& w = ctx->w[widx];
+    if (w.twin < 0) return 0;
+    W13Twin& t = ctx->twins[w.twin];
+    const int tile0 = (int)(((const char*)w.dev - (const char*)t.src) / ((int64_t)(t.K / 32) * 1024));
+    VVCHK(vv_w13_pack_rows_launch(t.src, t.planes, t.N, t.K, tile0, w.N / 16, st));
+    t.exact = -1;
+    return 0;
+}
+
+static bool w13_ok_words(const W13Twin& t, std::vector<unsigned>& ok, bool folded) {
+    const int n_tiles = t.N / 16;
+    ok.resize(folded ? 1 : n_tiles);
+    return hipMemcpy(ok.data(), (const char*)t.planes + vv_w13_plane_bytes(t.N, t.K) + (size_t)(folded ? 2 * n_tiles : n_tiles) * 4, ok.size() * 4,
+                     hipMemcpyDeviceToHost) == hipSuccess;
 }
 
 extern "C" int vv_set_speech_factors(vv_ctx* ctx, float scaling, float bias) {
@@ -568,14 +580,34 @@
         case 6: return ctx->seam_launches;
         case 8: return ctx->solver_fused;
         case 7: return ctx->lora_base_bytes;
-        case 9: {
+        case 9: case 11: {
+            VV_SHARED;
+            if (hipDeviceSynchronize() != hipSuccess) return -1;
+            std::vector<unsigned> tail;
+            if (what == 11) {
+                int64_t n = 0;
+                for (const W13Twin& t : ctx->twins) {
+                    if (!w13_ok_words(t, tail, false)) return -1;
+                    for (unsigned v : tail) n += v == 0;
+                }
+                return n;
+            }
+            auto exact = [&](int widx) {
+                const int ti = ctx->w[widx].twin;
+                return ti >= 0 && w13_ok_words(ctx->twins[ti], tail, true) && tail[0] == 1;
+            };
             int64_t n = 0;
             for (const auto& l : ctx->hl) {
-                if (ctx->w[l.ig].w13_ok && ctx->w[l.iu].w13_ok) n += 2;
-                if (ctx->w[l.id].w13_ok) n += 1;
+                if (exact(l.ig) && exact(l.iu)) n += 2;
+                if (exact(l.id)) n += 1;
             }
             return n;
         }
+        case 10: {
+            int64_t n = 0;
+            for (const W13Twin& t : ctx->twins) n += t.lm;
+            return n;
+        }
         default: return (int64_t)ctx->graphs.size();
     }
 }
diff --git a/vibevoice_amd/csrc/engine_ctx.h b/vibevoice_amd/csrc/engine_ctx.h
--- a/vibevoice_amd/csrc/engine_ctx.h
+++ b/vibevoice_amd/csrc/engine_ctx.h
@@ -30,9 +30,10 @@
     int rep = 1;
     bool loaded = false;
     bool optional = false;
-    void* w13 = nullptr;
-    bool w13_ok = false;
-};
+    int twin = -1;
+};
+
+struct W13Twin { void* planes; const void* src; int N, K; bool lm; int exact = -1, used = -1; };
 
 struct Block {
     int C;
@@ -91,7 +92,7 @@
     std::vector<Weight> w;
     std::map<std::string, int> widx;
     int H, D, Hq, Hkv, I, QKV;
-    struct Layer { float *ln1, *ln2, *bqkv; void *wqkv, *wo, *wg, *wu, *wd; };
+    struct Layer { float *ln1, *ln2, *bqkv; void *wqkv, *wo, *wg, *wu, *wd; void *tqkv, *to, *tg, *tu, *td; };
     std::vector<Layer> layers;
     float *lm_norm = nullptr, *inv_freq = nullptr;
     int ws_rows = 0;
@@ -117,7 +118,8 @@
     float *pm = nullptr, *pl = nullptr, *po = nullptr;
     int HF = 0, MODW = 0;
     struct HLayer { float* norm; void *wg, *wu, *wd; int ig, iu, id; };
-    bool w13_on = false;
+    bool w13_on = false, w13_lm = false;
+    std::vector<W13Twin> twins;
     std::vector<HLayer> hl;
     void *h_in = nullptr, *h_cond = nullptr, *h_t0 = nullptr, *h_t2 = nullptr, *h_ada = nullptr, *h_out = nullptr;
     int n_steps = 0;
diff --git a/vibevoice_amd/csrc/engine_head.hip b/vibevoice_amd/csrc/engine_head.hip
--- a/vibevoice_amd/csrc/engine_head.hip
+++ b/vibevoice_amd/csrc/engine_head.hip
@@ -1,5 +1,6 @@
 #include "engine_ctx.h"
 #include "pass_plan.h"
+#include "vv_w13.h"
 
 static int set_schedule(vv_ctx* ctx, int n_steps, const float* t, const float* coef, int width, void* stream, bool stochastic = false) {
     VV_SHARED;
@@ -126,14 +127,17 @@
         float* cur = ctx->xh_parts + (size_t)(l & 1) * 2 * xps;
         float* nxt = ctx->xh_parts + (size_t)((l + 1) & 1) * 2 * xps;
         g1.xa = cur; g1.n_xa = xp; g1.part_stride = xps;
-        const Weight &mg = ctx->w[ctx->hl[l].ig], &mu = ctx->w[ctx->hl[l].iu], &md = ctx->w[ctx->hl[l].id];
-        if (p.w13 && mg.w13_ok && mu.w13_ok && vv_gemv_w13_form(&g1, c.xsplit) >= 0) { g1.w13 = mg.w13; g1.w13_2 = mu.w13; }
+        const int tg = ctx->w[ctx->hl[l].ig].twin, tu = ctx->w[ctx->hl[l].iu].twin, td = ctx->w[ctx->hl[l].id].twin;
+        if (p.w13 && tg >= 0 && tu >= 0 && vv_gemv_w13_form(&g1, c.xsplit) >= 0) {
+            g1.w13 = ctx->twins[tg].planes; g1.w13_2 = ctx->twins[tu].planes;
+            g1.w13_exact = ctx->twins[tg].exact == 1 && ctx->twins[tu].exact == 1;
+        }
         GEMM(g1);
         VVGemm g2 = mk_gemm(ctx->hl[l].wd, ctx->hact, xh, rows, H, HF, HF, H);
         g2.epi = VV_EPI_GATED_RESID; g2.gate = base + 2 * H; g2.ld_gate = MODW; g2.nt = 1;
         g2.ya = cur; g2.n_ya = xp; g2.part_stride = xps;
         xp = ksplit_parts(ctx, g2, nxt, xps);
-        if (p.w13 && md.w13_ok && vv_gemv_w13_form(&g2, c.xsplit) >= 0) g2.w13 = md.w13;
+        if (p.w13 && td >= 0 && vv_gemv_w13_form(&g2, c.xsplit) >= 0) { g2.w13 = ctx->twins[td].planes; g2.w13_exact = ctx->twins[td].exact == 1; }
         if (ctx->probe_on) { char nm[64]; snprintf(nm, 64, "layer %d hact (parts in %d)", l, g1.n_xa); nan_probe(ctx, st, nm, ctx->hact, (size_t)rows * HF); }
         GEMM(g2);
         if (ctx->probe_on) {
@@ -269,8 +273,24 @@
     return 0;
 }
 
+static int head_w13_resolve(vv_ctx* ctx, hipStream_t st) {
+    if (!ctx->w13_on) return 0;
+    bool changed = false, waited = false;
+    for (W13Twin& t : ctx->twins) {
+        if (t.lm || t.exact >= 0) continue;
+        if (!waited) { HIPCHK(ctx, hipStreamSynchronize(st)); waited = true; }
+        unsigned ok = 0;
+        HIPCHK(ctx, hipMemcpy(&ok, (const char*)t.planes + vv_w13_plane_bytes(t.N, t.K) + (size_t)2 * (t.N / 16) * 4, 4, hipMemcpyDeviceToHost));
+        t.exact = ok == 1;
+        if (t.used >= 0 && t.used != t.exact) changed = true;
+        t.used = t.exact;
+    }
+    return changed ? drop_graphs(ctx, {"samp:", "sde:", "rows:", "gen:"}) : 0;
+}
+
 static int run_sampler(vv_ctx* ctx, hipStream_t st, const char* key, const SampleReq& r) {
     ctx->launches = 0;
+    { VV_SHARED; VVTRY(head_w13_resolve(ctx, st)); }
     const int rc = graphed(ctx, key, st, [&]() { return sample_body(ctx, st, r); });
     nan_probe_report(ctx, st, key);
     return rc;
@@ -328,6 +348,7 @@
     if (n < 1 || n > 16) return fail(ctx, "vv_head_forward: n must be in [1,16]");
     const int H = ctx->H;
     for (int i = 1; i < n; ++i) if (t_host[i] != t_host[0]) return fail(ctx, "vv_head_forward: all rows must share one timestep");
+    VVTRY(head_w13_resolve(ctx, st));
     float* tdev = ctx->tmp2 + 63 * 256;
     HIPCHK(ctx, hipStreamSynchronize(st));
     HIPCHK(ctx, hipMemcpy(tdev + 128, t_host, 4, hipMemcpyHostToDevice));
diff --git a/vibevoice_amd/csrc/engine_lm.hip b/vibevoice_amd/csrc/engine_lm.hip
--- a/vibevoice_amd/csrc/engine_lm.hip
+++ b/vibevoice_amd/csrc/engine_lm.hip
@@ -127,6 +127,8 @@
     VVGemm g = mk_gemm(L.wqkv, ctx->h, ctx->qkv, R, QKV, H, H, QKV);
     g.pro = VV_PRO_RMS; g.nw = L.ln1; g.eps = c.lm_eps; g.epi = VV_EPI_BIAS; g.bias = L.bqkv; g.nt = 1;
     g.xa = ctx->h_parts; g.n_xa = hp; g.part_stride = hps;
+    const auto w13 = [&](const VVGemm& a, const void* t) { return p.w13 && t && vv_gemv_w13_form(&a, c.xsplit) >= 0; };
+    if (w13(g, L.tqkv)) g.w13 = L.tqkv;
     GEMM(g);
     if (p.attn == VV_ATTN_FUSED) {
         VVTRY(lm_decode_attn(ctx, st, R, l, p, nullptr));
@@ -153,10 +155,12 @@
     hp = 0;
     VVGemm gm = mk_gemm(L.wg, ctx->h, ctx->act, R, I, H, H, I);
     gm.W2 = (const u32x4*)L.wu; gm.pro = VV_PRO_RMS; gm.nw = L.ln2; gm.eps = c.lm_eps; gm.epi = VV_EPI_SWIGLU; gm.nt = 1;
+    if (L.tu && w13(gm, L.tg)) { gm.w13 = L.tg; gm.w13_2 = L.tu; }
     GEMM(gm);
     VVGemm gd = mk_gemm(L.wd, ctx->act, ctx->h, R, H, I, I, H);
     gd.epi = VV_EPI_RESID; gd.nt = 1;
     if (l + 1 < l1) hp = ksplit_parts(ctx, gd, ctx->h_parts, hps);
+    if (w13(gd, L.td)) gd.w13 = L.td;
     GEMM(gd);
     return 0;
 }
@@ -207,7 +211,7 @@
         ctx->rope_ready = true;
     }
     VVLmPlan plan;
-    if (vv_lm_pass_plan(pin, n_rows, {ctx->ws_rows, ctx->c.attn_splits, ctx->Hkv, ctx->tile3_ok, ctx->attn2_ok, ctx->p16_ok}, &plan))
+    if (vv_lm_pass_plan(pin, n_rows, {ctx->ws_rows, ctx->c.attn_splits, ctx->Hkv, ctx->tile3_ok, ctx->attn2_ok, ctx->p16_ok, ctx->w13_lm}, &plan))
         return fail(ctx, "a launch of %d rows must be consecutive positions of one cache (decode / ragged launches take <= %d rows)", n_rows, ctx->ws_rows);
     char key[160]; snprintf(key, 160, "lm:%d:%p:%p:%d:%d:%d:%d:%d", n_rows, (const void*)x_in_dev, (void*)hidden_out_dev, l0, l1, final_norm,
                             plan.key_mode, plan.key_split);
diff --git a/vibevoice_amd/csrc/gemv.hip b/vibevoice_amd/csrc/gemv.hip
--- a/vibevoice_amd/csrc/gemv.hip
+++ b/vibevoice_amd/csrc/gemv.hip
@@ -41,7 +41,7 @@
     if constexpr (EPI == VV_EPI_CFG_DPM) asm volatile("" ::"s"(a.sde_noise), "s"(a.cfg_rows));
     VV_STAMP(0);
     VV_BSTAMP(0);
-    const int lane = threadIdx.x & 63;
+    int lane = threadIdx.x & 63;
     const int wave = __builtin_amdgcn_readfirstlane((int)(threadIdx.x >> 6));
     const int t_base = (MR == 16) ? (int)blockIdx.y * 16 : 0;
     const int T = min(MR, pT - t_base);
@@ -55,13 +55,13 @@
     const unsigned kt0 = kb0 + wave * kper;
     const unsigned kt1 = min(kb1, kt0 + kper);
     const bool has_k = kt0 < kt1;
-    const int frow = lane & 15, fq = lane >> 4;
+    int frow = lane & 15, fq = lane >> 4;
     unsigned char* stg = stg_all + (size_t)wave * (NOP * XS * U * 4 * GSB);
-    const unsigned kk = lane * 4;
-    const unsigned st_off = ((kk >> 5) * 4 + ((kk & 31) >> 3)) * GSB + (kk & 7) * 2;
-
-    const u32x4* wbase = pW + (size_t)tile * k_tiles * 64 + lane;
-    const u32x4* wbase2 = DUAL ? pW2 + (size_t)tile * k_tiles * 64 + lane : nullptr;
+    unsigned kk = lane * 4;
+    unsigned st_off = ((kk >> 5) * 4 + ((kk & 31) >> 3)) * GSB + (kk & 7) * 2;
+
+    const u32x4* wbase = WF ? nullptr : pW + (size_t)tile * k_tiles * 64 + lane;
+    const u32x4* wbase2 = DUAL && !WF ? pW2 + (size_t)tile * k_tiles * 64 + lane : nullptr;
     const unsigned char* gbase = reinterpret_cast<const unsigned char*>(pW) + (size_t)tile * (k_tiles >> 2) * VV_W13_GROUP;
     const unsigned char* gbase2 = reinterpret_cast<const unsigned char*>(pW2) + (size_t)tile * (k_tiles >> 2) * VV_W13_GROUP;
     constexpr int RG = WF ? (DUAL ? 2 : 3) : 1;
@@ -133,7 +133,7 @@
         }
     };
     XR R;
-    u32x4 wA[WF ? 1 : U][NM], wB[WF ? 1 : U][NM];
+    u32x4 wA[U][NM], wB[U][NM];
     if constexpr (WF) {
         if (has_k) {
             x_load(kt0, R);
@@ -284,60 +284,122 @@
 
     if constexpr (WF) {
         float wscale[NM];
-        {
-            const size_t tail = (size_t)gridDim.x * (k_tiles >> 2) * VV_W13_GROUP;
-            wscale[0] = vv_w13_scale(reinterpret_cast<const unsigned*>(reinterpret_cast<const unsigned char*>(pW) + tail)[tile]);
-            if constexpr (DUAL) wscale[1] = vv_w13_scale(reinterpret_cast<const unsigned*>(reinterpret_cast<const unsigned char*>(pW2) + tail)[tile]);
-        }
-        if (has_k) {
-            x_stage(kt0, R);
+        auto w13_loop = [&](XR& Rx) {
+        const unsigned klen = kt1 - kt0;
+        auto mma1 = [&](const u32x4 (&f)[NM][4], int t, unsigned slot) {
+            u32x4 xf = u32x4{0u, 0u, 0u, 0u};
+            if (frow < MRS) xf = *reinterpret_cast<const u32x4*>(stg + (size_t)(slot * 4 + fq) * GSB + frow * 16);
+            const bf16x8 xb = __builtin_bit_cast(bf16x8, xf);
+#pragma unroll
+            for (int i = 0; i < NM; ++i)
+                acc[i] = __builtin_amdgcn_mfma_f32_16x16x32_bf16(__builtin_bit_cast(bf16x8, f[i][t]), xb, acc[i], 0, 0, 0);
+        };
+        auto wstep = [&](unsigned i, auto s0c, auto s1c) {
+            constexpr int sl[2] = {decltype(s0c)::value, decltype(s1c)::value};
+#pragma unroll
+            for (int gi = 0; gi < 2; ++gi) {
+                u32x4 f[NM][4];
+                if (gi == 0) {
+                    if (ph > 0 && i > 0) {
+#pragma unroll
+                        for (int m = 0; m < NM; ++m) vv_w13_unpack(raw[sl[0]][m], wscale[m], f[m]);
+#pragma unroll
+                        for (int t = 0; t < 3; ++t)
+                            if ((unsigned)t < ph && 8 * i + t - ph < klen) mma1(f, t, 8 + t - ph);
+                    }
+                    if (i > 0 && 8 * i < klen) x_stage(kt0 + 8 * i, Rx);
+                    if (8 * (i + 1) < klen) x_load(kt0 + 8 * (i + 1), Rx);
+                }
+#pragma unroll
+                for (int m = 0; m < NM; ++m) vv_w13_unpack(raw[sl[gi]][m], wscale[m], f[m]);
+                const unsigned gn = g_lo + 2 * i + gi + RG;
+                if (gn < g_hi) g_load(gn, raw[sl[gi]]);
+#pragma unroll
+                for (int t = 0; t < 4; ++t)
+                    if ((unsigned)t >= (gi == 0 ? ph : 0u) && 8 * i + 4 * gi + t - ph < klen) mma1(f, t, 4 * gi + t - ph);
+            }
+        };
+        const unsigned n_wb = (ph + klen + 7) >> 3;
+        using S0 = std::integral_constant<int, 0>; using S1 = std::integral_constant<int, 1>; using S2 = std::integral_constant<int, 2>;
+        if constexpr (RG == 2) {
+#pragma unroll 1
+            for (unsigned i = 0; i < n_wb; ++i) wstep(i, S0{}, S1{});
+        } else {
+#pragma unroll 1
+            for (unsigned i = 0; i < n_wb; i += 3) {
+                wstep(i, S0{}, S1{});
+                if (i + 1 < n_wb) wstep(i + 1, S2{}, S0{});
+                if (i + 2 < n_wb) wstep(i + 2, S1{}, S2{});
+            }
+        }
+        };
+        if constexpr (WF == 1) {
+            {
+                const size_t tail = (size_t)gridDim.x * (k_tiles >> 2) * VV_W13_GROUP;
+                wscale[0] = vv_w13_scale(reinterpret_cast<const unsigned*>(reinterpret_cast<const unsigned char*>(pW) + tail)[tile]);
+                if constexpr (DUAL) wscale[1] = vv_w13_scale(reinterpret_cast<const unsigned*>(reinterpret_cast<const unsigned char*>(pW2) + tail)[tile]);
+            }
+            if (has_k) {
+                x_stage(kt0, R);
+                VV_STAMP(2);
+                w13_loop(R);
+            }
+        } else {
+            unsigned w13_ok;
+            {
+                const unsigned n_tiles = (unsigned)pN >> 4;
+                const size_t tail = (size_t)n_tiles * (k_tiles >> 2) * VV_W13_GROUP;
+                const unsigned* t1 = reinterpret_cast<const unsigned*>(reinterpret_cast<const unsigned char*>(pW) + tail);
+                unsigned sw[NM];
+                sw[0] = t1[tile];
+                w13_ok = t1[n_tiles + tile];
+                if constexpr (DUAL) {
+                    const unsigned* t2 = reinterpret_cast<const unsigned*>(reinterpret_cast<const unsigned char*>(pW2) + tail);
+                    sw[1] = t2[tile];
+                    w13_ok &= t2[n_tiles + tile];
+                    asm volatile("" ::"s"(sw[1]));
+                }
+                asm volatile("" ::"s"(sw[0]), "s"(w13_ok));
+#pragma unroll
+                for (int m = 0; m < NM; ++m) wscale[m] = vv_w13_scale(sw[m]);
+            }
+            if (has_k) x_stage(kt0, R);
             VV_STAMP(2);
-            const unsigned klen = kt1 - kt0;
-            auto mma1 = [&](const u32x4 (&f)[NM][4], int t, unsigned slot) {
-                u32x4 xf = u32x4{0u, 0u, 0u, 0u};
-                if (frow < MRS) xf = *reinterpret_cast<const u32x4*>(stg + (size_t)(slot * 4 + fq) * GSB + frow * 16);
-                const bf16x8 xb = __builtin_bit_cast(bf16x8, xf);
-#pragma unroll
-                for (int i = 0; i < NM; ++i)
-                    acc[i] = __builtin_amdgcn_mfma_f32_16x16x32_bf16(__builtin_bit_cast(bf16x8, f[i][t]), xb, acc[i], 0, 0, 0);
+            auto w_stream = [&](XR& Rx) {
+                if constexpr (DUAL) {
+#pragma unroll 1
+                    for (unsigned ktb = kt0; ktb < kt1; ktb += U) {
+                        const bool n1 = ktb + U < kt1;
+                        if (n1) x_load(ktb + U, Rx);
+                        mma(ktb, wA);
+                        if (n1) { w_load(ktb + U, wA); x_stage(ktb + U, Rx); }
+                    }
+                } else
+#pragma unroll 1
+                for (unsigned ktb = kt0; ktb < kt1; ktb += 2 * U) {
+                    const bool n1 = ktb + U < kt1, n2 = ktb + 2 * U < kt1;
+                    if (n1) { x_load(ktb + U, Rx); w_load(ktb + U, wB); }
+                    mma(ktb, wA);
+                    if (n1) x_stage(ktb + U, Rx);
+                    if (n2) { x_load(ktb + 2 * U, Rx); w_load(ktb + 2 * U, wA); }
+                    if (n1) mma(ktb + U, wB);
+                    if (n2) x_stage(ktb + 2 * U, Rx);
+                }
             };
-            auto wstep = [&](unsigned i, auto s0c, auto s1c) {
-                constexpr int sl[2] = {decltype(s0c)::value, decltype(s1c)::value};
-#pragma unroll
-                for (int gi = 0; gi < 2; ++gi) {
-                    u32x4 f[NM][4];
-                    if (gi == 0) {
-                        if (ph > 0 && i > 0) {
-#pragma unroll
-                            for (int m = 0; m < NM; ++m) vv_w13_unpack(raw[sl[0]][m], wscale[m], f[m]);
-#pragma unroll
-                            for (int t = 0; t < 3; ++t)
-                                if ((unsigned)t < ph && 8 * i + t - ph < klen) mma1(f, t, 8 + t - ph);
-                        }
-                        if (i > 0 && 8 * i < klen) x_stage(kt0 + 8 * i, R);
-                        if (8 * (i + 1) < klen) x_load(kt0 + 8 * (i + 1), R);
-                    }
-#pragma unroll
-                    for (int m = 0; m < NM; ++m) vv_w13_unpack(raw[sl[gi]][m], wscale[m], f[m]);
-                    const unsigned gn = g_lo + 2 * i + gi + RG;
-                    if (gn < g_hi) g_load(gn, raw[sl[gi]]);
-#pragma unroll
-                    for (int t = 0; t < 4; ++t)
-                        if ((unsigned)t >= (gi == 0 ? ph : 0u) && 8 * i + 4 * gi + t - ph < klen) mma1(f, t, 4 * gi + t - ph);
-                }
-            };
-            const unsigned n_wb = (ph + klen + 7) >> 3;
-            using S0 = std::integral_constant<int, 0>; using S1 = std::integral_constant<int, 1>; using S2 = std::integral_constant<int, 2>;
-            if constexpr (RG == 2) {
-#pragma unroll 1
-                for (unsigned i = 0; i < n_wb; ++i) wstep(i, S0{}, S1{});
-            } else {
-#pragma unroll 1
-                for (unsigned i = 0; i < n_wb; i += 3) {
-                    wstep(i, S0{}, S1{});
-                    if (i + 1 < n_wb) wstep(i + 1, S2{}, S0{});
-                    if (i + 2 < n_wb) wstep(i + 2, S1{}, S2{});
-                }
+            if (__builtin_expect(w13_ok == 0, 0)) {
+                if (has_k) {
+                    asm volatile("" : "+v"(lane));
+                    frow = lane & 15; fq = lane >> 4; kk = lane * 4;
+                    st_off = ((kk >> 5) * 4 + ((kk & 31) >> 3)) * GSB + (kk & 7) * 2;
+                    wbase = a.W + (size_t)tile * k_tiles * 64 + lane;
+                    if constexpr (DUAL) wbase2 = a.W2 + (size_t)tile * k_tiles * 64 + lane;
+                    w_load(kt0, wA);
+                    XR Rf;
+                    w_stream(Rf);
+                }
+            } else if (has_k) {
+                XR Rw = R;
+                w13_loop(Rw);
             }
         }
     } else
@@ -476,9 +538,10 @@
 static const auto gemv_kernels = gemv_kernel_table(std::make_index_sequence<VV_GF_COUNT * VV_GEMV_MAX_PAIRS * VV_GEMV_MAX_XS>{});
 
 template <size_t... J>
-static constexpr std::array<std::array<GemvKernel, 2>, sizeof...(J)> gemv_w13_table(std::index_sequence<J...>) {
+static constexpr std::array<std::array<GemvKernel, 3>, sizeof...(J)> gemv_w13_table(std::index_sequence<J...>) {
     return {{{vv_gemv_kernel<1, vv_gemv_w13_forms[J].pro, vv_gemv_w13_forms[J].epi, vv_gemv_w13_forms[J].mr, vv_gemv_w13_forms[J].wpb, 0, 0, 0>,
-              vv_gemv_kernel<1, vv_gemv_w13_forms[J].pro, vv_gemv_w13_forms[J].epi, vv_gemv_w13_forms[J].mr, vv_gemv_w13_forms[J].wpb, 0, 0, 1>}...}};
+              vv_gemv_kernel<1, vv_gemv_w13_forms[J].pro, vv_gemv_w13_forms[J].epi, vv_gemv_w13_forms[J].mr, vv_gemv_w13_forms[J].wpb, 0, 0, 1>,
+              vv_gemv_kernel<1, vv_gemv_w13_forms[J].pro, vv_gemv_w13_forms[J].epi, vv_gemv_w13_forms[J].mr, vv_gemv_w13_forms[J].wpb, 0, 0, 2>}...}};
 }
 static const auto gemv_w13_kernels = gemv_w13_table(std::make_index_sequence<VV_GEMV_W13_FORMS>{});
 
@@ -500,11 +563,11 @@
     if (a.w13) {
         const int wi = vv_gemv_w13_form(&a, xs);
         if (wi < 0 || (a.epi == VV_EPI_SWIGLU && !a.w13_2)) return VV_RC_NO_FORM;
-        k = gemv_w13_kernels[wi][1];
-        a.W = (const u32x4*)a.w13; a.W2 = (const u32x4*)a.w13_2;
+        k = gemv_w13_kernels[wi][a.w13_exact ? 1 : 2];
     }
     if (form) { form[0] = p.form.xs; form[1] = p.form.mr; form[2] = p.form.wpb; form[3] = p.form.parts; form[4] = p.form.sl; }
-    hipLaunchKernelGGL(k, p.grid, dim3(p.form.wpb * 64), 0, s, a.W, a.W2, a.X, a.Y, a.nw, a.T, a.N, a.K, a.ldx, a.ldy, a);
+    hipLaunchKernelGGL(k, p.grid, dim3(p.form.wpb * 64), 0, s, a.w13 ? (const u32x4*)a.w13 : a.W, a.w13 ? (const u32x4*)a.w13_2 : a.W2, a.X, a.Y, a.nw,
+                       a.T, a.N, a.K, a.ldx, a.ldy, a);
     return vv_launch_rc(0);
 }
 
@@ -512,8 +575,8 @@
     if (a.epi == VV_EPI_SWIGLU && (!a.W2 || (a.w13 && !a.w13_2))) return -1;
     const int wi = vv_gemv_w13_find(a.pro, a.epi, mr, wpb);
     if (wi < 0 || !vv_gemv_eligible(&a) || !vv_gemv_w13_shape(&a, 1) || a.T > mr) return VV_RC_NO_FORM;
-    const GemvKernel k = gemv_w13_kernels[wi][a.w13 ? 1 : 0];
-    if (a.w13) { a.W = (const u32x4*)a.w13; a.W2 = (const u32x4*)a.w13_2; }
-    hipLaunchKernelGGL(k, dim3(a.N / 16, 1), dim3(wpb * 64), 0, s, a.W, a.W2, a.X, a.Y, a.nw, a.T, a.N, a.K, a.ldx, a.ldy, a);
+    const GemvKernel k = gemv_w13_kernels[wi][a.w13 ? (a.w13_exact ? 1 : 2) : 0];
+    hipLaunchKernelGGL(k, dim3(a.N / 16, 1), dim3(wpb * 64), 0, s, a.w13 ? (const u32x4*)a.w13 : a.W, a.w13 ? (const u32x4*)a.w13_2 : a.W2, a.X, a.Y, a.nw,
+                       a.T, a.N, a.K, a.ldx, a.ldy, a);
     return vv_launch_rc(0);
 }
diff --git a/vibevoice_amd/csrc/gemv_plan.h b/vibevoice_amd/csrc/gemv_plan.h
--- a/vibevoice_amd/csrc/gemv_plan.h
+++ b/vibevoice_amd/csrc/gemv_plan.h
@@ -129,7 +129,8 @@
 
 struct VVGemvW13Form { int pro, epi, mr, wpb; };
 inline constexpr VVGemvW13Form vv_gemv_w13_forms[] = {
-    {VV_PRO_RMS_MOD, VV_EPI_SWIGLU, 2, 4}, {VV_PRO_RMS_MOD, VV_EPI_SWIGLU, 4, 8}, {VV_PRO_NONE, VV_EPI_GATED_RESID, 4, 8}};
+    {VV_PRO_RMS_MOD, VV_EPI_SWIGLU, 2, 4}, {VV_PRO_RMS_MOD, VV_EPI_SWIGLU, 4, 8}, {VV_PRO_NONE, VV_EPI_GATED_RESID, 4, 8},
+    {VV_PRO_RMS, VV_EPI_BIAS, 2, 4}, {VV_PRO_RMS, VV_EPI_SWIGLU, 2, 4}, {VV_PRO_NONE, VV_EPI_RESID, 4, 8}};
 constexpr int VV_GEMV_W13_FORMS = sizeof(vv_gemv_w13_forms) / sizeof(vv_gemv_w13_forms[0]);
 inline int vv_gemv_w13_find(int pro, int epi, int mr, int wpb) {
     for (int i = 0; i < VV_GEMV_W13_FORMS; ++i) {
diff --git a/vibevoice_amd/csrc/pass_plan.h b/vibevoice_amd/csrc/pass_plan.h
--- a/vibevoice_amd/csrc/pass_plan.h
+++ b/vibevoice_amd/csrc/pass_plan.h
@@ -12,7 +12,7 @@
 enum { VV_LM_PREFILL, VV_LM_P16, VV_LM_GEMV };
 enum { VV_ATTN_FUSED, VV_ATTN_PREFILL4, VV_ATTN_SPLIT_MERGE };
 
-struct VVLmCaps { int ws_rows, attn_splits, Hkv; bool tile3_ok, attn2_ok, p16_ok; };
+struct VVLmCaps { int ws_rows, attn_splits, Hkv; bool tile3_ok, attn2_ok, p16_ok; bool w13 = false; };
 
 struct VVLmPlan {
     bool fused;
@@ -23,6 +23,7 @@
     bool zero_v_tail;
     int key_mode, key_split;
     int64_t kv_positions;
+    bool w13 = false;
 };
 
 inline int vv_lm_pass_plan(const VVRow* rows, int n_rows, const VVLmCaps& c, VVLmPlan* p) {
@@ -60,6 +61,7 @@
     p->zero_v_tail = p->route == VV_LM_PREFILL || chunk_attn;
     p->key_mode = fused ? 1 : (contiguous ? 2 : 0);
     p->key_split = chunk_attn ? 0 : S;
+    p->w13 = c.w13 && p->route == VV_LM_GEMV && n_rows <= 2;
     return 0;
 }
 
diff --git a/vibevoice_amd/csrc/vv_common.h b/vibevoice_amd/csrc/vv_common.h
--- a/vibevoice_amd/csrc/vv_common.h
+++ b/vibevoice_amd/csrc/vv_common.h
@@ -79,6 +79,7 @@
     float* dw_hnew;
     const void* w13;
     const void* w13_2;
+    int w13_exact;
 };
 
 struct VVGemv16p {
diff --git a/vibevoice_amd/csrc/vv_launch.h b/vibevoice_amd/csrc/vv_launch.h
--- a/vibevoice_amd/csrc/vv_launch.h
+++ b/vibevoice_amd/csrc/vv_launch.h
@@ -99,6 +99,7 @@
 int vv_gemv_launch(VVGemm a, int xs, hipStream_t s, int* form);
 int vv_gemv_w13_form_launch(VVGemm a, int mr, int wpb, hipStream_t s);
 int vv_w13_pack_launch(const void* packed, void* twin, int N, int K, hipStream_t s);
+int vv_w13_pack_rows_launch(const void* packed, void* twin, int N, int K, int tile0, int tiles, hipStream_t s);
 int vv_w13_unpack_launch(const void* twin, void* packed, int N, int K, hipStream_t s);
 int vv_tile_ok(const VVGemm* a, int xs);
 int vv_tile_launch(VVGemm a, int xs, hipStream_t s);
diff --git a/vibevoice_amd/csrc/w13.hip b/vibevoice_amd/csrc/w13.hip
--- a/vibevoice_amd/csrc/w13.hip
+++ b/vibevoice_amd/csrc/w13.hip
@@ -6,10 +6,10 @@
 
 constexpr int PACK_WAVES = 4;
 
-__global__ __launch_bounds__(PACK_WAVES * 64) void vv_w13_pack_kernel(const u32x4* __restrict__ W, unsigned char* __restrict__ out, int n_tiles, int k_tiles) {
+__global__ __launch_bounds__(PACK_WAVES * 64) void vv_w13_pack_kernel(const u32x4* __restrict__ W, unsigned char* __restrict__ out, int n_tiles, int k_tiles, int tile0) {
     __shared__ unsigned red[PACK_WAVES];
     const int lane = threadIdx.x & 63, wave = threadIdx.x >> 6;
-    const unsigned tile = blockIdx.x;
+    const unsigned tile = blockIdx.x + tile0;
     const int groups = k_tiles >> 2;
     const u32x4* src = W + (size_t)tile * k_tiles * 64;
     unsigned emax = 0;
@@ -106,12 +106,15 @@
 
 }
 
-extern "C" int vv_w13_pack_launch(const void* packed, void* twin, int N, int K, hipStream_t s) {
-    if (!vv_w13_shape_ok(N, K)) return VV_RC_NO_FORM;
+extern "C" int vv_w13_pack_rows_launch(const void* packed, void* twin, int N, int K, int tile0, int tiles, hipStream_t s) {
+    if (!vv_w13_shape_ok(N, K) || tile0 < 0 || tiles < 1 || tile0 + tiles > N / 16) return VV_RC_NO_FORM;
     const int n_tiles = N / 16, k_tiles = K / 32;
-    hipLaunchKernelGGL(vv_w13_pack_kernel, dim3(n_tiles), dim3(PACK_WAVES * 64), 0, s, (const u32x4*)packed, (unsigned char*)twin, n_tiles, k_tiles);
+    hipLaunchKernelGGL(vv_w13_pack_kernel, dim3(tiles), dim3(PACK_WAVES * 64), 0, s, (const u32x4*)packed, (unsigned char*)twin, n_tiles, k_tiles, tile0);
     hipLaunchKernelGGL(vv_w13_fold_kernel, dim3(1), dim3(256), 0, s, reinterpret_cast<unsigned*>((unsigned char*)twin + vv_w13_plane_bytes(N, K)), n_tiles);
     return vv_launch_rc(0);
+}
+extern "C" int vv_w13_pack_launch(const void* packed, void* twin, int N, int K, hipStream_t s) {
+    return vv_w13_pack_rows_launch(packed, twin, N, K, 0, N / 16, s);
 }
 extern "C" int vv_w13_unpack_launch(const void* twin, void* packed, int N, int K, hipStream_t s) {
     if (!vv_w13_shape_ok(N, K)) return VV_RC_NO_FORM;
```

Result: faster. 17.91 (median of 6 runs) (+3.7%).
